# hyperplane-lab/RGBManip

Hardware: AMD Instinct MI355X
Metric: adapose_poses_per_sec_batch256 (higher is better)
Workload: dtype bf16

## Files before the change

include/rgbm.h:

```cpp
#ifndef RGBM_H_
#define RGBM_H_
#include <stddef.h>
#include <stdint.h>

#ifdef __cplusplus
extern "C" {
#endif

#define RGBM_VERSION 100
#define RGBM_F32 0
#define RGBM_BF16 1
#define RGBM_F16 2
#define RGBM_BF16X3 3

int rgbm_version(void);
const char* rgbm_last_error(void);

typedef struct rgbm_weight_desc {
  const char* name;
  const float* data;
  int ndim;
  const int64_t* shape;
} rgbm_weight_desc;

// ... 72 lines not shown
int rgbm_cloud_gather_views(const float* maps, const int32_t* index, int n, int V, int S2, int C, int cap, float* out, void* stream);

int rgbm_adapose_postprocess(int B, int P, int img_size, const float* nocs1, const float* depth1, const float* r1,
                             const int32_t* choose1, const double* Kcrop, const double* E1, double* bbox_world, double* ts,
                             int32_t* valid, void* stream);
int rgbm_adapose_postprocess_scratch_bytes(int B, size_t* bytes);
int rgbm_adapose_postprocess_ws(int B, int P, int img_size, const float* nocs1, const float* depth1, const float* r1,
                                const int32_t* choose1, const double* Kcrop, const double* E1, double* bbox_world, double* ts,
                                int32_t* valid, void* scratch, size_t scratch_bytes, void* stream);

int rgbm_adapose_postprocess_regressed(int B, int P, const float* nocs1, const float* r1, const float* t1, const float* s1,
                                       const double* E1, double* bbox_world, double* ts, int32_t* valid, void* stream);

int rgbm_adapose_postprocess_ransac(int B, int P, int img_size, uint32_t seed, const float* nocs1, const float* depth1,
                                    const int32_t* choose1, const double* Kcrop, const double* E1, double* bbox_world, double* srt,
                                    int32_t* valid, void* stream);
int rgbm_adapose_postprocess_pnp(int B, int P, uint32_t seed, const float* nocs1, const float* pts2d1, const float* nocs2,
                                 const float* pts2d2, const double* K, const double* E1, const double* E2, double* bbox_out,
                                 double* srt_out, int32_t* info_out, int32_t* valid_out, void* stream);

int rgbm_prepare_inputs(const float* rgb_dev, const uint8_t* mask_dev, const double* K_dev, int N, int H, int W, int S, int P,
                        uint32_t seed, float* img_out, int32_t* choose_out, float* pts2d_out, double* Kcrop_out,
                        int32_t* window_out, int32_t* valid_out, uint8_t* scratch, void* stream);

int rgbm_prepare_inputs_indexed(const float* rgb_dev, const uint8_t* mask_dev, const double* K_dev, const int32_t* frame_map_dev,
                                int N, int H, int W, int S, int P, uint32_t seed, float* img_out, int32_t* choose_out,
                                float* pts2d_out, double* Kcrop_out, int32_t* window_out, int32_t* valid_out, uint8_t* scratch,
                                void* stream);
int rgbm_prepare_inputs_ex(const float* rgb_dev, const uint8_t* mask_dev, const double* K_dev, const int32_t* frame_map_dev,
                           int frame0, int N, int H, int W, int S, int P, uint32_t seed, float* img_out, int32_t* choose_out,
                           float* pts2d_out, double* Kcrop_out, int32_t* window_out, int32_t* valid_out, uint8_t* scratch,
                           void* stream);
int rgbm_prepare_inputs_u8(const uint8_t* rgb_dev, const uint8_t* mask_dev, const double* K_dev, const int32_t* frame_map_dev,
                           int frame0, int N, int H, int W, int S, int P, uint32_t seed, float* img_out, int32_t* choose_out,
                           float* pts2d_out, double* Kcrop_out, int32_t* window_out, int32_t* valid_out, uint8_t* scratch,
                           void* stream);
int rgbm_prepare_inputs_opt(const void* rgb_dev, int pixel_type, int normalize, const uint8_t* mask_dev, const double* K_dev,
                            const int32_t* frame_map_dev, int frame0, int N, int H, int W, int S, int P, uint32_t seed, float* img_out,
                            int32_t* choose_out, float* pts2d_out, double* Kcrop_out, int32_t* window_out, int32_t* valid_out,
                            uint8_t* scratch, void* stream);
int rgbm_prepare_inputs_windows(const void* pix_dev, int pixel_type, int normalize, const uint8_t* mask_pix_dev, const int64_t* offset_dev,
                                const int32_t* window_dev, const int32_t* valid_in_dev, const double* K_dev, int frame0, int N, int H, int W,
                                int S, int P, uint32_t seed, float* img_out, int32_t* choose_out, float* pts2d_out, double* Kcrop_out,
                                int32_t* valid_out, uint8_t* scratch, void* stream);
int rgbm_quantize_frames(const float* src_dev, uint8_t* dst_dev, size_t n, void* stream);

int rgbm_projection(const double* Kcrop_dev, const double* E_dev, float* P_dev, int N, void* stream);
int rgbm_mask_extent(const uint8_t* mask_dev, int N, int H, int W, int32_t* ext_out, int32_t* count_out, void* stream);

int rgbm_lookat_quat(const double* dir_dev, int N, int batch_zero, double* quat_dev, void* stream);
int rgbm_control_action_to_pose(const float* action_dev, int lda, const double* pose_mid, const double* pose_min,
                                const double* pose_max, int N, double* pose_dev, void* stream);
typedef struct rgbm_control_reward_args {
  const float* action;
  const double* cam_pose;
  const double* target;
  const float* move_success;
  const double* bbox;
  const double* avail;
  const double* gt_bbox;
  const double* pred_bbox;
  const double* pose_cur;
  const double* pose_prev;
  const double* robot_pose;
  const double* success;
  double* reward;
  double* terms;
  double coef[14];
  double proper_pos[3];
  double precision2;
  int N, T, lda, pots, first;
  int pad_;
} rgbm_control_reward_args;
int rgbm_control_reward(const rgbm_control_reward_args* args, void* stream);
int rgbm_control_grasp_frame(const double* est_dev, int N, double* center_dev, double* direction_dev, void* stream);

typedef struct rgbm_synth_scene {
  const double* cam_pose;
  const double* robot_pose;
  const double* box;
  double fx, fy, cx, cy;
  int N, H, W, env0;
} rgbm_synth_scene;
int rgbm_synth_camera(const rgbm_synth_scene* scene, double* K_dev, double* E_dev, double* rays_dev, void* stream);
int rgbm_synth_render(const rgbm_synth_scene* scene, const double* rays_dev, float* color_dev, uint8_t* mask_dev, void* stream);
int rgbm_synth_render_u8(const rgbm_synth_scene* scene, const double* rays_dev, uint8_t* color_dev, uint8_t* mask_dev,
                         int32_t* extent_dev, int32_t* count_dev, void* stream);

int rgbm_gae(int T, int N, const float* rewards, const uint8_t* dones, const float* values, const float* last_values,
             float gamma, float lam, float* returns, float* adv, double* sums, void* stream);
int rgbm_adv_normalise(int64_t n_local, float* adv, const double* sums, double count_total, void* stream);

typedef struct rgbm_policy_layout {
  int dims[5];
  int log_std;
  int w[2][4];
  int b[2][4];
  int total;
} rgbm_policy_layout;
int rgbm_policy_forward(const float* params, const rgbm_policy_layout* L, int n, int mode, const float* obs, const float* noise,
                        float* actions, float* logp, float* value, float* mu, void* stream);
int rgbm_ppo_partial_floats(const rgbm_policy_layout* L, int n, size_t* count);
int rgbm_ppo_minibatch_fwd_bwd(const float* params, const rgbm_policy_layout* L, int n, const float* obs, const float* actions,
                               const float* old_logp, const float* adv, const float* returns, const float* old_values,
                               const float* old_mu, const float* old_log_std, float clip, float vcoef, float ecoef,
                               float* partial_scratch, float* grads_flat, void* stream);
int rgbm_ppo_clip_adam(float* params, const float* grads_flat, float* exp_avg, float* exp_avg_sq, void* opt_state,
                       const rgbm_policy_layout* L, float inv_world, float max_norm, float desired_kl, float lr_min,
                       float lr_max, int adaptive, void* stream);

#define RGBM_POLICY_MAX_HIDDEN 6
#define RGBM_POLICY_MAX_WIDTH 512
#define RGBM_POLICY_MAX_ACT 32
#define RGBM_ACT_ELU 0
#define RGBM_ACT_SELU 1
#define RGBM_ACT_RELU 2
#define RGBM_ACT_LRELU 3
#define RGBM_ACT_TANH 4
#define RGBM_ACT_SIGMOID 5
typedef struct rgbm_policy_desc {
  int obs_dim, state_dim, act_dim;
  int activation;
  int asymmetric;
  int n_hidden[2];
  int hidden[2][RGBM_POLICY_MAX_HIDDEN];
  int w[2][RGBM_POLICY_MAX_HIDDEN + 1];
  int b[2][RGBM_POLICY_MAX_HIDDEN + 1];
  int log_std;
  int total;
} rgbm_policy_desc;
int rgbm_policy_forward_ex(const float* params, const rgbm_policy_desc* D, int n, int mode, const float* obs, const float* states,
                           const float* noise, float* actions, float* logp, float* value, float* mu, void* stream);
int rgbm_ppo_scratch_floats_ex(const rgbm_policy_desc* D, int n, int clipped_value_loss, size_t* count);
int rgbm_ppo_minibatch_fwd_bwd_ex(const float* params, const rgbm_policy_desc* D, int n, const float* obs, const float* states,
                                  const float* actions, const float* old_logp, const float* adv, const float* returns,
                                  const float* old_values, const float* old_mu, const float* old_log_std, float clip, float vcoef,
                                  float ecoef, int clipped_value_loss, float* scratch, float* grads_flat, void* stream);
int rgbm_ppo_clip_adam_ex(float* params, const float* grads_flat, float* exp_avg, float* exp_avg_sq, void* opt_state, int total,
                          float inv_world, float max_norm, float desired_kl, float lr_min, float lr_max, int adaptive, void* stream);

int rgbm_conv_nd(int dtype, const void* in_dev, int N, int D, int H, int W, int Cin, int Cin_pad, const float* w_host,
                 int Cout, int Cout_pad, int KD, int KH, int KW, int stride_d, int stride_hw, int pad_d, int pad_hw,
                 int dil_hw, int transposed, const float* bias_host, const float* bn_scale_host, const float* bn_shift_host,
                 const void* res_dev, int res_mode, int act, float slope, void* out_dev, void* stream);
#define RGBM_CONV_PLAN_INTS 9
int rgbm_conv_plan(int dtype, int N, int D, int H, int W, int Cin, int Cin_pad, int Cout, int Cout_pad, int KD, int KH, int KW,
                   int stride_d, int stride_hw, int pad_d, int pad_hw, int dil_hw, int transposed, int has_bias, int res_mode, int act,
                   int cls, int n_cu, int32_t* plan);
#define RGBM_BORDER_HEAD_INTS 10
int rgbm_conv_border_plan(int dtype, int N, int H, int W, int Cin, int Cout, int K, int stride, int pad, int dil, int res_mode, int n_cu,
                          int32_t* head, int32_t* classes, int cap_classes, int32_t* tiles, int32_t* order, int cap_tiles, int32_t* wg_off,
                          int cap_wg, int32_t* rows, int64_t cap_rows);
int rgbm_conv_border_launches(int64_t* count);
int rgbm_bn_per_sample_scratch_bytes(int V, size_t* bytes);
int rgbm_bn_per_sample(int dtype, void* y_dev, const void* res_dev, const float* gamma_dev, const float* beta_dev, void* scratch_dev,
                       int V, int64_t nvox, int C, int relu, void* stream);
int rgbm_conv3d_tile(int layer, int dtype, const void* in_dev, int N, int D, int H, int W, const float* w_host,
                     const float* bn_scale_host, const float* bn_shift_host, const void* res_dev, void* out_dev, void* stream);
int rgbm_upsample_conv3x3(int dtype, const void* in_dev, int V, int h, int w, int Cin, const float* w_host, int Cout,
                          const float* bias_host, int act, float slope, void* z_scratch_dev, void* out_dev, void* stream);
int rgbm_upsample_conv3x3_final(int dtype, const void* in_dev, int V, int h, int w, const float* w3_host, const float* b3_host,
                                float slope, const float* wf_host, const float* bf_host, void* out_dev, int out_f32, void* stream);
int rgbm_stem(int dtype, const float* img1_dev, const float* img2_dev, const float* w_host, void* out_dev, int B, int S, void* stream);
int rgbm_maxpool3x3s2(int dtype, const void* in_dev, void* out_dev, int V, int H, int W, int C, void* stream);
int rgbm_resize_bilinear_ac(int dtype, const void* in_dev, void* out_dev, int V, int Hs, int Ws, int C, int Ho, int Wo,
                            void* stream);
int rgbm_adaptive_avgpool(int dtype, const void* in_dev, void* out_dev, int V, int H, int W, int C, int S, void* stream);
int rgbm_build_volume(int dtype, const void* feat_dev, const float* P_views_dev, const float* depths_dev, float* homog_scratch,
                      void* vol_dev, int V, int B, int D, int H, int W, void* stream);
int rgbm_conv0_sweep(const void* feat_dev, const float* P_views_dev, const float* depths_dev, float* homog_scratch,
                     const float* w_host, const float* bn_scale_host, const float* bn_shift_host, void* out_dev,
                     int V, int B, int D, int H, int W, void* stream);
int rgbm_conv0_sweep_dt(int dtype, const void* feat_dev, const float* P_views_dev, const float* depths_dev, float* homog_scratch,
                        const float* w_host, const float* bn_scale_host, const float* bn_shift_host, void* out_dev,
                        int V, int B, int D, int H, int W, void* stream);
int rgbm_conv0_sweep_f16feat(const void* feat_f16_dev, const float* P_views_dev, const float* depths_dev, float* homog_scratch,
                             const float* w_host, const float* bn_scale_host, const float* bn_shift_host, void* out_bf16_dev,
                             int V, int B, int D, int H, int W, void* stream);
int rgbm_adapose_forward_ex(rgbm_adapose_t* h, int B, const float* img1, const float* img2, const int32_t* choose1,
                            const int32_t* choose2, const float* P1, const float* P2, const float* depths, void* workspace,
                            size_t workspace_bytes, const rgbm_adapose_out* out, int stop_after, void* stream);
int rgbm_adapose_forward_graph(rgbm_adapose_t* h, int B, const float* img1, const float* img2, const int32_t* choose1,
                               const int32_t* choose2, const float* P1, const float* P2, const float* depths, void* workspace,
                               size_t workspace_bytes, const rgbm_adapose_out* out, void* stream, int32_t* n_nodes, int32_t* captured);
int rgbm_adapose_graph_clear(rgbm_adapose_t* h);
int rgbm_adapose_feature_bytes(rgbm_adapose_t* h, size_t* bytes);
int rgbm_adapose_features_workspace_bytes(rgbm_adapose_t* h, int V, size_t* bytes);
int rgbm_adapose_features(rgbm_adapose_t* h, int V, const float* img, const int32_t* slots_dev, void* pool, int pool_records,
                          void* workspace, size_t workspace_bytes, void* stream);
int rgbm_adapose_forward_cached(rgbm_adapose_t* h, int B, const void* pool, int pool_records, const int32_t* slot1_dev,
                                const int32_t* slot2_dev, const int32_t* choose1, const int32_t* choose2, const float* P1, const float* P2,
                                const float* depths, void* workspace, size_t workspace_bytes, const rgbm_adapose_out* out, void* stream);
int rgbm_adapose_fetch(rgbm_adapose_t* h, int B, void* workspace, const char* name, float* out_dev, size_t capacity,
                       size_t* n_elems, void* stream);
int rgbm_crop_fingerprint(const float* img, int V, int n_words, uint64_t* keys_out, void* stream);

#define RGBM_PROF_ROWS 42
int rgbm_debug_flags(int flags);
int rgbm_set_tuning(const char* key, long long value);
int rgbm_microbench_mfma_scratch_floats(int* n);
int rgbm_microbench_mfma(float* scratch, int iters, int random_operands, double* flops, void* stream);
int rgbm_microbench_copy(const void* src, void* dst, size_t bytes, void* stream);
int rgbm_prof_rows(void);
int rgbm_prof_start(void);
int rgbm_prof_stop(double* stats);
int rgbm_prof_select(int row);

#ifdef __cplusplus
}
#endif
#endif
```

rgbmanip_amd/_lib.py:

```python
from __future__ import annotations

import ctypes as C
import os

_HERE = os.path.dirname(os.path.abspath(__file__))
LIB_PATH = os.environ.get("RGBM_HIP_LIB") or os.path.join(_HERE, "librgbm_hip.so")

F32, BF16, F16, BF16X3 = 0, 1, 2, 3
ACT_NONE, ACT_RELU, ACT_PRELU, ACT_TANH = 0, 1, 2, 3
RES_NONE, RES_PRE_ACT, RES_POST_ACT = 0, 1, 2


PROF_ROWS = 42
PROF_KERNELS = [
    ("conv_igemm_glds_kernel<float, 16, 256>", "fp32"), ("conv_igemm_glds_kernel<float, 32, 256>", "fp32"),
    ("conv_igemm_glds_kernel<float, 64, 256>", "fp32"), ("conv_igemm_glds_kernel<float, 128, 128>", "fp32"),
    ("conv_igemm_glds_kernel<unsigned short, 16, 256>", "bf16"), ("conv_igemm_glds_kernel<unsigned short, 32, 256>", "bf16"),
    ("conv_igemm_glds_kernel<unsigned short, 64, 256>", "bf16"), ("conv_igemm_glds_kernel<unsigned short, 128, 128>", "bf16"),
    ("conv3d_tile_kernel<float, ...> (conv1..conv11)", "fp32"), ("conv3d_tile_kernel<unsigned short, ...> (conv1..conv11)", "bf16"),
    ("conv3d_tile_kernel<float, 32, 16, 4, 8, 8, 1, false, true> (conv0 + fused plane sweep)", "fp32"),
    ("conv3d_tile_kernel<unsigned short, 32, 16, 4, 8, 8, 1, false, true> (conv0 + fused plane sweep)", "bf16"),
    ("conv_igemm_ws_kernel<float, ...>", "fp32"), ("conv_igemm_ws_kernel<unsigned short, false, false> (128 channels x 256 pixels)", "bf16"),
    ("conv0_sweep_persistent_kernel<unsigned short> (conv0 + fused plane sweep of bf16 nets; sweep_f16 = 0 / fp16 nets: conv0_sweep_kernel)", "bf16"), ("conv_igemm_ws64_kernel", "bf16"),
    ("conv3d_tile_kernel<unsigned short, 32, 16, 6, 8, 8, 1, false, false> (conv0 on a materialised volume)", "bf16"),
    ("conv3d_tile_kernel<unsigned short, 8, 16, 2, 8, 8, 2, false, false> (conv1)", "bf16"),
    ("conv3d_tile_kernel<unsigned short, 16, 16, 4, 8, 8, 1, false, false> (conv2)", "bf16"),
    ("conv3d_tile_kernel<unsigned short, 16, 32, 2, 8, 8, 2, false, false> (conv3)", "bf16"),
    ("conv3d_tile_kernel<unsigned short, 32, 32, 2, 8, 8, 1, false, false> (conv4)", "bf16"),
    ("conv3d_tile_kernel<unsigned short, 32, 64, 1, 8, 8, 2, false, false> (conv5)", "bf16"),
    ("conv3d_tile_kernel<unsigned short, 64, 64, 1, 8, 8, 1, false, false> (conv6)", "bf16"),
    ("conv3d_tile_kernel<unsigned short, 64, 32, 1, 8, 8, 1, true, false> (conv7)", "bf16"),
    ("conv3d_tile_kernel<unsigned short, 32, 16, 2, 8, 8, 1, true, false> (conv9)", "bf16"),
    ("conv3d_tile_kernel<unsigned short, 16, 16, 4, 8, 8, 1, true, false> (conv11)", "bf16"),
] + [("conv_igemm_glds_kernel<bx3_t, ...> (all channel tiles)", "bf16x3"), ("conv3d_tile_kernel<bx3_t, ...> (conv1..conv11)", "bf16x3"),
     ("conv0 + fused plane sweep <bx3_t>", "bf16x3"), ("conv_igemm_ws_kernel<rgbm::bx3_t, false, false> (128 channels x 256 pixels)", "bf16x3"),
     ("pose_mlp1_kernel (pose_mlp1.0 + pose_mlp1.2 of a bf16 net in one launch)", "bf16"),
     ("conv_igemm_m32_kernel<unsigned short, 256, 256> (256 channels x 256 pixels, 32x32x16 MFMAs; gemm_kernel = 0: conv_igemm_ws_kernel<unsigned short, true, false>, 256 x 128)", "bf16"),
     ("pose_mlp2_kernel (pose_mlp2.0 + pose_mlp2.2 + the sum over points of a bf16 net in one launch)", "bf16"),
     ("conv_igemm_m32_kernel<rgbm::bx3_t, 256, 256> (256 channels x 256 pixels, 32x32x16 MFMAs; gemm_kernel = 0: conv_igemm_ws_kernel<rgbm::bx3_t, true, false>, 256 x 128)", "bf16x3"),
     ("conv_igemm_ws_kernel<rgbm::bx3_t, false, false, true> (64 channels x 256 pixels, four multiply waves)", "bf16x3"),
     ("conv_igemm_ws_kernel<unsigned short, false, false, true> (64 channels x 256 pixels, four multiply waves)", "bf16"),
     ("conv_igemm_ws_kernel<float, false, false, true> (64 channels x 256 pixels, four multiply waves)", "fp32"),
     ("upconv_combine_kernel<16-bit> (PSPUpsample tap combination)", "bf16"), ("upconv_combine_kernel<4-byte> (PSPUpsample tap combination)", "bf16x3"),
     ("upconv_final_kernel (up_3 + final in one kernel; either storage width)", "bf16"),
     ("conv_igemm_m32_kernel<unsigned short, 128, 64 / 128 / 256> (128-pixel tiles: tail and small-batch launches of the 256-channel GEMM)", "bf16"),
     ("conv_igemm_m32_kernel<rgbm::bx3_t, 128, 64 / 128 / 256> (128-pixel tiles: tail and small-batch launches of the 256-channel GEMM)", "bf16x3")]
assert len(PROF_KERNELS) == PROF_ROWS


class RgbmError(RuntimeError):
    pass


class WeightDesc(C.Structure):
    _fields_ = [("name", C.c_char_p), ("data", C.c_void_p), ("ndim", C.c_int), ("shape", C.POINTER(C.c_int64))]


class PolicyLayout(C.Structure):
    _fields_ = [("dims", C.c_int * 5), ("log_std", C.c_int), ("w", (C.c_int * 4) * 2), ("b", (C.c_int * 4) * 2), ("total", C.c_int)]


POLICY_MAX_HIDDEN, POLICY_MAX_WIDTH, POLICY_MAX_ACT = 6, 512, 32
POLICY_ACTIVATIONS = {"elu": 0, "selu": 1, "relu": 2, "crelu": 2, "lrelu": 3, "tanh": 4, "sigmoid": 5}


class PolicyDesc(C.Structure):
    _fields_ = [("obs_dim", C.c_int), ("state_dim", C.c_int), ("act_dim", C.c_int), ("activation", C.c_int), ("asymmetric", C.c_int),
                ("n_hidden", C.c_int * 2), ("hidden", (C.c_int * POLICY_MAX_HIDDEN) * 2),
                ("w", (C.c_int * (POLICY_MAX_HIDDEN + 1)) * 2), ("b", (C.c_int * (POLICY_MAX_HIDDEN + 1)) * 2),
                ("log_std", C.c_int), ("total", C.c_int)]


class AdaposeOut(C.Structure):
    _fields_ = [(n, C.c_void_p) for n in ("view1_nocs", "view2_nocs", "view1_depth", "view2_depth", "view1_r", "view2_r",
                                           "view1_t", "view2_t", "view1_s", "view2_s")]


class ControlRewardArgs(C.Structure):
    _fields_ = [(n, C.c_void_p) for n in ("action", "cam_pose", "target", "move_success", "bbox", "avail", "gt_bbox", "pred_bbox",
                                           "pose_cur", "pose_prev", "robot_pose", "success", "reward", "terms")] + [
        ("coef", C.c_double * 14), ("proper_pos", C.c_double * 3), ("precision2", C.c_double),
        ("N", C.c_int), ("T", C.c_int), ("lda", C.c_int), ("pots", C.c_int), ("first", C.c_int), ("pad_", C.c_int)]


class SynthScene(C.Structure):
    _fields_ = [("cam_pose", C.c_void_p), ("robot_pose", C.c_void_p), ("box", C.c_void_p),
                ("fx", C.c_double), ("fy", C.c_double), ("cx", C.c_double), ("cy", C.c_double),
                ("N", C.c_int), ("H", C.c_int), ("W", C.c_int), ("env0", C.c_int)]


_vp, _i, _f, _d, _sz, _i64 = C.c_void_p, C.c_int, C.c_float, C.c_double, C.c_size_t, C.c_int64

SIGNATURES = {
    "rgbm_version": (_i, []),
    "rgbm_last_error": (C.c_char_p, []),
    "rgbm_adapose_create": (_i, [C.POINTER(_vp), _i, C.POINTER(WeightDesc), _i, _i, _i]),
    "rgbm_adapose_create_baseline": (_i, [C.POINTER(_vp), _i, C.POINTER(WeightDesc), _i, _i, _i]),
    "rgbm_view_fusion": (_i, [_vp, _vp, _vp, _i, _i, _vp, _vp, _vp, _sz, _vp]),
    "rgbm_view_fusion_scratch_bytes": (_i, [_i, _i, C.POINTER(_sz)]),
    "rgbm_depth_head": (_i, [_vp, _vp, _i64, _vp, _vp]),
    "rgbm_adapose_destroy": (_i, [_vp]),
    "rgbm_adapose_set_chunk": (_i, [_vp, _i]),
    "rgbm_adapose_set_option": (_i, [_vp, C.c_char_p, _i]),
    "rgbm_adapose_workspace_bytes": (_i, [_vp, _i, C.POINTER(_sz)]),
    "rgbm_adapose_set_dropout": (_i, [_vp, _f, C.c_uint64]),
    "rgbm_adapose_dropout_masks": (_i, [_vp, _i, _vp]),
    "rgbm_adapose_set_dropout_masks": (_i, [_vp, _i, _vp]),
    "rgbm_adapose_forward": (_i, [_vp, _i, _vp, _vp, _vp, _vp, _vp, _vp, _vp, _vp, _sz, C.POINTER(AdaposeOut), _vp]),
    "rgbm_adapose_forward_ex": (_i, [_vp, _i, _vp, _vp, _vp, _vp, _vp, _vp, _vp, _vp, _sz, C.POINTER(AdaposeOut), _i, _vp]),
    "rgbm_adapose_forward_graph": (_i, [_vp, _i, _vp, _vp, _vp, _vp, _vp, _vp, _vp, _vp, _sz, C.POINTER(AdaposeOut), _vp, C.POINTER(C.c_int32),
                                        C.POINTER(C.c_int32)]),
    "rgbm_adapose_samples_workspace_bytes": (_i, [_vp, _i, _i, C.POINTER(_sz)]),
    "rgbm_adapose_forward_samples": (_i, [_vp, _i, _i, _vp, _vp, _vp, _vp, _vp, _vp, _vp, _vp, _sz, C.POINTER(AdaposeOut), _vp]),
    "rgbm_sample_box_stats": (_i, [_vp, _vp, _i, _i, _vp, _vp, _vp, _vp, _vp, _vp, _vp, _vp, _vp]),
    "rgbm_sample_point_stats": (_i, [_vp, _i, _i, _i64, _vp, _vp, _vp]),
    "rgbm_box_agreement": (_i, [_vp, _vp, _vp, _vp, _i] + [_vp] * 14),
    "rgbm_box_iou_matrix": (_i, [_vp, _vp, _vp, _vp, _i, _i, _i, _vp, _vp]),
    "rgbm_adapose_dense_workspace_bytes": (_i, [_vp, _i, C.POINTER(_sz)]),
    "rgbm_adapose_forward_dense": (_i, [_vp, _i, _vp, _vp, _vp, _vp, _vp, _vp, _vp, _vp, _sz, C.POINTER(AdaposeOut), _vp, _vp, _vp]),
    "rgbm_adapose_forward_maps": (_i, [_vp, _i, _vp, _vp, _vp, _vp, _vp, _vp, _vp, _vp, _sz, C.POINTER(AdaposeOut), _vp, _vp, _vp, _vp]),
    "rgbm_nocs_map": (_i, [_vp, _vp, _i, _i, _vp, _vp]),
    "rgbm_cloud_gather": (_i, [_vp, _vp, _vp, _i, _i, _i, _i, _vp, _vp]),
    "rgbm_cloud_similarity_scratch_bytes": (_i, [_i, _i, C.POINTER(_sz)]),
    "rgbm_cloud_similarity": (_i, [_vp, _vp, _vp, _i, _i, C.c_uint32, _vp, _vp, _vp, _vp, _vp, _sz, _vp]),
    "rgbm_depth_to_points": (_i, [_vp, _vp, _vp, _i, _i, _vp, _vp]),
    "rgbm_depth_consistency": (_i, [_vp, _vp, _vp, _vp, _vp, _vp, _vp, _vp, _i, _i, _d, _d, _f, _vp, _vp, _vp, _vp, _vp]),
    "rgbm_cloud_pack": (_i, [_vp, _vp, _vp, _vp, _vp, _vp, _vp, _vp, _i, _i, _i, _vp, _vp, _vp, _vp]),
    "rgbm_depth_fusion": (_i, [_vp, _vp, _vp, _vp, _vp, _i, _i, _i, _d, _d, _f, _i, _vp, _vp, _vp, _vp, _vp]),
    "rgbm_cloud_pack_views": (_i, [_vp, _vp, _vp, _vp, _i, _i, _i, _i, _vp, _vp, _vp, _vp]),
    "rgbm_cloud_gather_views": (_i, [_vp, _vp, _i, _i, _i, _i, _i, _vp, _vp]),
    "rgbm_adapose_graph_clear": (_i, [_vp]),
    "rgbm_adapose_feature_bytes": (_i, [_vp, C.POINTER(_sz)]),
    "rgbm_adapose_features_workspace_bytes": (_i, [_vp, _i, C.POINTER(_sz)]),
    "rgbm_adapose_features": (_i, [_vp, _i, _vp, _vp, _vp, _i, _vp, _sz, _vp]),
    "rgbm_adapose_forward_cached": (_i, [_vp, _i, _vp, _i, _vp, _vp, _vp, _vp, _vp, _vp, _vp, _vp, _sz, C.POINTER(AdaposeOut), _vp]),
    "rgbm_crop_fingerprint": (_i, [_vp, _i, _i, _vp, _vp]),
    "rgbm_adapose_fetch": (_i, [_vp, _i, _vp, C.c_char_p, _vp, _sz, C.POINTER(_sz), _vp]),
    "rgbm_adapose_postprocess": (_i, [_i, _i, _i, _vp, _vp, _vp, _vp, _vp, _vp, _vp, _vp, _vp, _vp]),
    "rgbm_adapose_postprocess_scratch_bytes": (_i, [_i, C.POINTER(_sz)]),
    "rgbm_adapose_postprocess_ws": (_i, [_i, _i, _i, _vp, _vp, _vp, _vp, _vp, _vp, _vp, _vp, _vp, _vp, _sz, _vp]),
    "rgbm_adapose_postprocess_regressed": (_i, [_i, _i, _vp, _vp, _vp, _vp, _vp, _vp, _vp, _vp, _vp]),
    "rgbm_adapose_postprocess_ransac": (_i, [_i, _i, _i, C.c_uint32, _vp, _vp, _vp, _vp, _vp, _vp, _vp, _vp, _vp]),
    "rgbm_adapose_postprocess_pnp": (_i, [_i, _i, C.c_uint32, _vp, _vp, _vp, _vp, _vp, _vp, _vp, _vp, _vp, _vp, _vp, _vp]),
    "rgbm_gae": (_i, [_i, _i, _vp, _vp, _vp, _vp, _f, _f, _vp, _vp, _vp, _vp]),
    "rgbm_adv_normalise": (_i, [_i64, _vp, _vp, _d, _vp]),
    "rgbm_policy_forward": (_i, [_vp, _vp, _i, _i, _vp, _vp, _vp, _vp, _vp, _vp, _vp]),
    "rgbm_ppo_partial_floats": (_i, [_vp, _i, C.POINTER(_sz)]),
    "rgbm_ppo_minibatch_fwd_bwd": (_i, [_vp, _vp, _i, _vp, _vp, _vp, _vp, _vp, _vp, _vp, _vp, _f, _f, _f, _vp, _vp, _vp]),
    "rgbm_ppo_clip_adam": (_i, [_vp, _vp, _vp, _vp, _vp, _vp, _f, _f, _f, _f, _f, _i, _vp]),
    "rgbm_policy_forward_ex": (_i, [_vp, _vp, _i, _i, _vp, _vp, _vp, _vp, _vp, _vp, _vp, _vp]),
    "rgbm_ppo_scratch_floats_ex": (_i, [_vp, _i, _i, C.POINTER(_sz)]),
    "rgbm_ppo_minibatch_fwd_bwd_ex": (_i, [_vp, _vp, _i, _vp, _vp, _vp, _vp, _vp, _vp, _vp, _vp, _vp, _f, _f, _f, _i, _vp, _vp, _vp]),
    "rgbm_ppo_clip_adam_ex": (_i, [_vp, _vp, _vp, _vp, _vp, _i, _f, _f, _f, _f, _f, _i, _vp]),
    "rgbm_conv_nd": (_i, [_i, _vp, _i, _i, _i, _i, _i, _i, _vp, _i, _i, _i, _i, _i, _i, _i, _i, _i, _i, _i, _vp, _vp, _vp,
                          _vp, _i, _i, _f, _vp, _vp]),
    "rgbm_conv_plan": (_i, [_i] * 23 + [C.POINTER(C.c_int32)]),
    "rgbm_conv_border_plan": (_i, [_i] * 12 + [C.POINTER(C.c_int32)] * 2 + [_i] + [C.POINTER(C.c_int32)] * 2 + [_i, C.POINTER(C.c_int32), _i,
                                   C.POINTER(C.c_int32), _i64]),
    "rgbm_conv_border_launches": (_i, [C.POINTER(C.c_int64)]),
    "rgbm_bn_per_sample_scratch_bytes": (_i, [_i, C.POINTER(_sz)]),
    "rgbm_bn_per_sample": (_i, [_i, _vp, _vp, _vp, _vp, _vp, _i, _i64, _i, _i, _vp]),
    "rgbm_conv3d_tile": (_i, [_i, _i, _vp, _i, _i, _i, _i, _vp, _vp, _vp, _vp, _vp, _vp]),
    "rgbm_upsample_conv3x3": (_i, [_i, _vp, _i, _i, _i, _i, _vp, _i, _vp, _i, _f, _vp, _vp, _vp]),
    "rgbm_upsample_conv3x3_final": (_i, [_i, _vp, _i, _i, _i, _vp, _vp, _f, _vp, _vp, _vp, _i, _vp]),
    "rgbm_stem": (_i, [_i, _vp, _vp, _vp, _vp, _i, _i, _vp]),
    "rgbm_maxpool3x3s2": (_i, [_i, _vp, _vp, _i, _i, _i, _i, _vp]),
    "rgbm_resize_bilinear_ac": (_i, [_i, _vp, _vp, _i, _i, _i, _i, _i, _i, _vp]),
    "rgbm_adaptive_avgpool": (_i, [_i, _vp, _vp, _i, _i, _i, _i, _i, _vp]),
    "rgbm_build_volume": (_i, [_i, _vp, _vp, _vp, _vp, _vp, _i, _i, _i, _i, _i, _vp]),
    "rgbm_conv0_sweep": (_i, [_vp, _vp, _vp, _vp, _vp, _vp, _vp, _vp, _i, _i, _i, _i, _i, _vp]),
    "rgbm_conv0_sweep_dt": (_i, [_i, _vp, _vp, _vp, _vp, _vp, _vp, _vp, _vp, _i, _i, _i, _i, _i, _vp]),
    "rgbm_conv0_sweep_f16feat": (_i, [_vp, _vp, _vp, _vp, _vp, _vp, _vp, _vp, _i, _i, _i, _i, _i, _vp]),
    "rgbm_prepare_inputs": (_i, [_vp, _vp, _vp, _i, _i, _i, _i, _i, C.c_uint32, _vp, _vp, _vp, _vp, _vp, _vp, _vp, _vp]),
    "rgbm_prepare_inputs_indexed": (_i, [_vp, _vp, _vp, _vp, _i, _i, _i, _i, _i, C.c_uint32, _vp, _vp, _vp, _vp, _vp, _vp, _vp, _vp]),
    "rgbm_prepare_inputs_ex": (_i, [_vp, _vp, _vp, _vp, _i, _i, _i, _i, _i, _i, C.c_uint32, _vp, _vp, _vp, _vp, _vp, _vp, _vp, _vp]),
    "rgbm_prepare_inputs_u8": (_i, [_vp, _vp, _vp, _vp, _i, _i, _i, _i, _i, _i, C.c_uint32, _vp, _vp, _vp, _vp, _vp, _vp, _vp, _vp]),
    "rgbm_prepare_inputs_opt": (_i, [_vp, _i, _i, _vp, _vp, _vp, _i, _i, _i, _i, _i, _i, C.c_uint32, _vp, _vp, _vp, _vp, _vp, _vp, _vp, _vp]),
    "rgbm_prepare_inputs_windows": (_i, [_vp, _i, _i, _vp, _vp, _vp, _vp, _vp, _i, _i, _i, _i, _i, _i, C.c_uint32, _vp, _vp, _vp, _vp, _vp, _vp, _vp]),
    "rgbm_quantize_frames": (_i, [_vp, _vp, C.c_size_t, _vp]),
    "rgbm_projection": (_i, [_vp, _vp, _vp, _i, _vp]),
    "rgbm_mask_extent": (_i, [_vp, _i, _i, _i, _vp, _vp, _vp]),
    "rgbm_lookat_quat": (_i, [_vp, _i, _i, _vp, _vp]),
    "rgbm_control_action_to_pose": (_i, [_vp, _i, C.POINTER(C.c_double), C.POINTER(C.c_double), C.POINTER(C.c_double), _i, _vp, _vp]),
    "rgbm_control_reward": (_i, [C.POINTER(ControlRewardArgs), _vp]),
    "rgbm_control_grasp_frame": (_i, [_vp, _i, _vp, _vp, _vp]),
    "rgbm_synth_camera": (_i, [C.POINTER(SynthScene), _vp, _vp, _vp, _vp]),
    "rgbm_synth_render": (_i, [C.POINTER(SynthScene), _vp, _vp, _vp, _vp]),
    "rgbm_synth_render_u8": (_i, [C.POINTER(SynthScene), _vp, _vp, _vp, _vp, _vp, _vp]),
    "rgbm_debug_flags": (_i, [_i]),
    "rgbm_set_tuning": (_i, [C.c_char_p, _i64]),
    "rgbm_prof_rows": (_i, []),
    "rgbm_microbench_mfma_scratch_floats": (_i, [C.POINTER(C.c_int)]),
    "rgbm_microbench_mfma": (_i, [_vp, _i, _i, C.POINTER(C.c_double), _vp]),
    "rgbm_microbench_copy": (_i, [_vp, _vp, C.c_size_t, _vp]),
    "rgbm_prof_start": (_i, []),
    "rgbm_prof_select": (_i, [_i]),
    "rgbm_prof_stop": (_i, [C.POINTER(C.c_double)]),
}

_lib = None


def load():
    global _lib
    if _lib is not None:
        return _lib
    if not os.path.exists(LIB_PATH):
        raise RgbmError(f"{LIB_PATH} not found: build it with rgbmanip_amd/csrc/build.sh "
                        f"(or `python -c 'import __graft_entry__ as g; g.build()'`). There is no CPU fallback.")
    lib = C.CDLL(LIB_PATH)
    for name, (res, args) in SIGNATURES.items():
        fn = getattr(lib, name)
        fn.restype = res
        fn.argtypes = args
    if lib.rgbm_prof_rows() != PROF_ROWS:
        raise RgbmError(f"{LIB_PATH}: rgbm_prof_rows() = {lib.rgbm_prof_rows()}, this binding expects {PROF_ROWS} (stale build?)")
    _lib = lib
    return lib


def check(rc: int, what: str = ""):
    if rc != 0:
        msg = load().rgbm_last_error()
        raise RgbmError(f"{what} failed (code {rc}): {msg.decode() if msg else ''}")


def stream_ptr(stream=None):
    import torch
    s = stream if stream is not None else torch.cuda.current_stream()
    return C.c_void_p(s.cuda_stream)


def ptr(t):
    return C.c_void_p(t.data_ptr()) if t is not None else C.c_void_p(0)
```

rgbmanip_amd/csrc/capi.cpp:

```cpp
#include "../../include/rgbm.h"

#include <string.h>

#include <algorithm>
#include <initializer_list>
#include <memory>
#include <string>
#include <utility>
#include <vector>

#include "adapose.h"
#include "box_overlap.h"
#include "control.h"
#include "cost3d.h"
#include "conv_plan.h"
#include "prof.h"
#include "sample_stats.h"
#include "view_fusion.h"

using namespace rgbm;

struct ForwardGraph {
  int B = 0;
  hipStream_t stream = nullptr;
// ... 490 lines not shown
  else if (nm == "pf96") { src = bf.PF96; cnt = V * P * 96; dt = n.pose_dtype() == BF16X3 ? BF16X3 : F32; }
  else if (nm == "pf2") { src = bf.pf2; cnt = V * 256; dt = F32; }
  else if (nm == "r6") { src = bf.r6; cnt = V * 6; dt = F32; }
  else if (nm == "fused1" && bf.fused) { src = bf.fused; cnt = (size_t)B * P * 32; dt = F32; }
  else if (nm == "fused2" && bf.fused) { src = bf.fused + (size_t)B * P * 32; cnt = (size_t)B * P * 32; dt = F32; }
  static const struct { const char* name; int row; } taps3d[] = {{"c0", 0}, {"c2", 2}, {"c4", 4}, {"c6", 6}, {"u7", 7}, {"u9", 8}, {"u11", 9}};
  int row3d = -1;
  for (const auto& t : taps3d)
    if (nm == t.name) { row3d = t.row; src = bf.c3[row3d]; cnt = cost3d_out_elems(row3d, (int)Vc, (int)D, (int)S); }
  if (is_baseline(h))
    RGBM_REQUIRE(nm == "feat" || nm == "fused1" || nm == "fused2" || nm == "pf96" || nm == "pf2" || nm == "r6" || nm == "layer4" || nm == "cat" ||
                 nm == "u1" || nm == "u2", "tap '" + nm + "' does not exist in the baseline network");
  RGBM_REQUIRE(src != nullptr, "unknown intermediate name: " + nm);
  const bool tap3d = row3d >= 0 && row3d < 9;
  RGBM_REQUIRE(!(tap3d && n.sparse_active()), "tap '" + nm + "' needs a dense cost regularisation: set option sparse_dec = 0 before the forward "
               "(the default computes it only inside the chosen pixels' dependency cones)");
  *n_elems = cnt;
  RGBM_REQUIRE(cnt <= capacity, "fetch capacity too small");
  return launch_to_f32(dt, src, out_dev, (long long)cnt, (hipStream_t)stream);
}

int rgbm_adapose_postprocess(int B, int P, int img_size, const float* nocs1, const float* depth1, const float* r1,
                             const int32_t* choose1, const double* Kcrop, const double* E1, double* bbox_world, double* ts,
                             int32_t* valid, void* stream) {
  RGBM_REQUIRE(B > 0 && nocs1 && depth1 && r1 && choose1 && Kcrop && E1 && bbox_world && ts && valid, "postprocess arguments");
  return launch_postprocess(nocs1, depth1, r1, choose1, Kcrop, E1, bbox_world, ts, valid, B, P, img_size, (hipStream_t)stream);
}

int rgbm_adapose_postprocess_scratch_bytes(int B, size_t* bytes) {
  RGBM_REQUIRE(B > 0 && bytes, "postprocess_scratch_bytes arguments");
  *bytes = postprocess_slices(B) > 1 ? postprocess_scratch_bytes(B) : 0;
  return 0;
}

int rgbm_adapose_postprocess_ws(int B, int P, int img_size, const float* nocs1, const float* depth1, const float* r1,
                                const int32_t* choose1, const double* Kcrop, const double* E1, double* bbox_world, double* ts,
                                int32_t* valid, void* scratch, size_t scratch_bytes, void* stream) {
  RGBM_REQUIRE(B > 0 && nocs1 && depth1 && r1 && choose1 && Kcrop && E1 && bbox_world && ts && valid, "postprocess arguments");
  return launch_postprocess(nocs1, depth1, r1, choose1, Kcrop, E1, bbox_world, ts, valid, B, P, img_size, (hipStream_t)stream,
                            scratch, scratch_bytes);
}

int rgbm_adapose_postprocess_ransac(int B, int P, int img_size, uint32_t seed, const float* nocs1, const float* depth1,
                                    const int32_t* choose1, const double* Kcrop, const double* E1, double* bbox_world, double* srt,
                                    int32_t* valid, void* stream) {
  return launch_umeyama_ransac(nocs1, depth1, choose1, Kcrop, E1, bbox_world, srt, valid, B, P, img_size, seed, (hipStream_t)stream);
}

int rgbm_gae(int T, int N, const float* rewards, const uint8_t* dones, const float* values, const float* last_values,
             float gamma, float lam, float* returns, float* adv, double* sums, void* stream) {
  RGBM_REQUIRE(rewards && dones && values && last_values && returns && adv && sums, "gae arguments");
  return launch_gae(T, N, rewards, dones, values, last_values, gamma, lam, returns, adv, sums, (hipStream_t)stream);
}

int rgbm_adv_normalise(int64_t n_local, float* adv, const double* sums, double count_total, void* stream) {
  RGBM_REQUIRE(adv && sums && n_local > 0 && count_total > 1.0, "adv_normalise arguments");
  return launch_adv_normalise(n_local, adv, sums, count_total, (hipStream_t)stream);
}

static ConvGeom conv_nd_geom(int Cin, int Cout, int KD, int KH, int KW, int stride_d, int stride_hw, int pad_d, int pad_hw, int dil_hw,
                             int transposed, int act, float slope) {
  ConvGeom g;
  g.Cin = Cin; g.Cout = Cout; g.KD = KD; g.KH = KH; g.KW = KW;
  g.sd = stride_d; g.sh = g.sw = stride_hw; g.pd = pad_d; g.ph = g.pw = pad_hw;
  g.dild = 1; g.dilh = g.dilw = dil_hw; g.transposed = transposed != 0; g.act = act; g.slope = slope;
  return g;
}

int rgbm_conv_nd(int dtype, const void* in_dev, int N, int D, int H, int W, int Cin, int Cin_pad, const float* w_host,
                 int Cout, int Cout_pad, int KD, int KH, int KW, int stride_d, int stride_hw, int pad_d, int pad_hw,
                 int dil_hw, int transposed, const float* bias_host, const float* bn_scale_host, const float* bn_shift_host,
                 const void* res_dev, int res_mode, int act, float slope, void* out_dev, void* stream) {
  RGBM_REQUIRE(in_dev && w_host && out_dev, "conv arguments");
  const ConvGeom g = conv_nd_geom(Cin, Cout, KD, KH, KW, stride_d, stride_hw, pad_d, pad_hw, dil_hw, transposed, act, slope);
  ConvLayer L;
  if (int rc = L.init(dtype, g, w_host, bias_host, bn_scale_host, bn_shift_host, Cin_pad, Cout_pad)) return rc;
  return finish_one_shot(L.run(in_dev, out_dev, N, D, H, W, Cout_pad, res_dev, res_mode, nullptr, 0, (hipStream_t)stream), stream);
}

int rgbm_conv_plan(int dtype, int N, int D, int H, int W, int Cin, int Cin_pad, int Cout, int Cout_pad, int KD, int KH, int KW,
                   int stride_d, int stride_hw, int pad_d, int pad_hw, int dil_hw, int transposed, int has_bias, int res_mode, int act,
                   int cls, int n_cu, int32_t* plan) {
  RGBM_REQUIRE(plan && n_cu >= 0 && dtype >= F32 && dtype <= BF16X3 && N > 0 && D > 0 && H > 0 && W > 0, "conv_plan arguments");
  const ConvGeom g = conv_nd_geom(Cin, Cout, KD, KH, KW, stride_d, stride_hw, pad_d, pad_hw, dil_hw, transposed, act, 0.f);
  PackedConv pc;
  if (int rc = conv_pack_geom(g, dtype, Cin_pad, Cout_pad, cls, &pc)) return rc;
  ConvDesc d;
  conv_desc_geom(d, g, pc, Cin_pad, Cout_pad, N, D, H, W, Cout_pad, cls);
  alignas(16) static const float buffer[4] = {};
  d.in = d.wgt = buffer; d.out = const_cast<float*>(buffer);
  d.bias = has_bias ? buffer : nullptr;
  d.res = res_mode != RES_NONE ? buffer : nullptr;
  d.res_mode = res_mode;
  ConvTuning t;
  ConvPlan p;
  if (int rc = conv_tuning(n_cu, &t)) return rc;
  if (int rc = plan_conv(d, dtype, t, &p)) return rc;
  const int32_t v[RGBM_CONV_PLAN_INTS] = {p.kernel, p.bch, p.bpix, p.ksplit, (int32_t)p.main_rows, p.tail_bch, p.identity_residual, (int32_t)d.M, d.KT};
  memcpy(plan, v, sizeof(v));
  return 0;
}

int rgbm_conv_border_plan(int dtype, int N, int H, int W, int Cin, int Cout, int K, int stride, int pad, int dil, int res_mode, int n_cu,
                          int32_t* head, int32_t* classes, int cap_classes, int32_t* tiles, int32_t* order, int cap_tiles, int32_t* wg_off,
                          int cap_wg, int32_t* rows, int64_t cap_rows) {
  RGBM_REQUIRE(head && n_cu >= 0 && dtype >= F32 && dtype <= BF16X3 && N > 0 && H > 0 && W > 0 && K > 0, "conv_border_plan arguments");
  const ConvGeom g = conv_nd_geom(Cin, Cout, 1, K, K, 1, stride, 0, pad, dil, 0, ACT_RELU, 0.f);
  PackedConv pc;
  const int E = dtype_chunk(dtype);
  const int Cin_pad = (Cin + E - 1) / E * E, Cout_pad = (Cout + 3) / 4 * 4;
  if (int rc = conv_pack_geom(g, dtype, Cin_pad, Cout_pad, 0, &pc)) return rc;
  ConvDesc d;
  conv_desc_geom(d, g, pc, Cin_pad, Cout_pad, N, 1, H, W, Cout_pad, 0);
  alignas(16) static const float buffer[4] = {};
  d.in = d.wgt = buffer; d.out = const_cast<float*>(buffer);
  d.res = res_mode != RES_NONE ? buffer : nullptr;
  d.res_mode = res_mode;
  d.w_finite = 1;
  ConvTuning t;
  ConvPlan p;
  if (int rc = conv_tuning(n_cu, &t)) return rc;
  if (int rc = plan_conv(d, dtype, t, &p)) return rc;
  memset(head, 0, RGBM_BORDER_HEAD_INTS * sizeof(int32_t));
  BorderPlan bp;
  if (p.kernel != CONV_M32 || !p.border || !plan_border(d, dtype, t.flags, p.main_rows, t.n_cu, &bp)) return 0;
  const int32_t h[RGBM_BORDER_HEAD_INTS] = {1, (int32_t)bp.classes.size(), (int32_t)bp.tiles.size(), bp.n_wg, (int32_t)bp.rows.size(),
                                             (int32_t)bp.max_wg_steps, (int32_t)bp.total_steps, (int32_t)bp.parent_steps, bp.steps_per_tap, bp.kr};
  memcpy(head, h, sizeof(h));
  if (classes) {
    RGBM_REQUIRE((int)bp.classes.size() <= cap_classes, "conv_border_plan: cap_classes too small");
    for (size_t c = 0; c < bp.classes.size(); ++c) {
      classes[3 * c] = bp.classes[c].n_pix; classes[3 * c + 1] = bp.classes[c].mask; classes[3 * c + 2] = (int32_t)bp.classes[c].row0;
    }
  }
  if (tiles || order) RGBM_REQUIRE((int)bp.tiles.size() <= cap_tiles, "conv_border_plan: cap_tiles too small");
  if (tiles)
    for (size_t i = 0; i < bp.tiles.size(); ++i) {
      const BorderTile& bt = bp.tiles[i];
      const int32_t v[5] = {bt.cls, bt.ch, bt.mask, bt.steps, (int32_t)bt.row0};
      memcpy(tiles + 5 * i, v, sizeof(v));
    }
  if (order) memcpy(order, bp.order.data(), bp.order.size() * sizeof(int32_t));
  if (wg_off) {
    RGBM_REQUIRE(bp.n_wg + 1 <= cap_wg, "conv_border_plan: cap_wg too small");
    memcpy(wg_off, bp.wg_off.data(), bp.wg_off.size() * sizeof(int32_t));
  }
  if (rows) {
    RGBM_REQUIRE((int64_t)bp.rows.size() <= cap_rows, "conv_border_plan: cap_rows too small");
    memcpy(rows, bp.rows.data(), bp.rows.size() * sizeof(int32_t));
  }
  return 0;
}

int rgbm_conv_border_launches(int64_t* count) {
  RGBM_REQUIRE(count, "conv_border_launches arguments");
  *count = border_launch_count();
  return 0;
}

int rgbm_upsample_conv3x3(int dtype, const void* in_dev, int V, int h, int w, int Cin, const float* w_host, int Cout,
                          const float* bias_host, int act, float slope, void* z_scratch_dev, void* out_dev, void* stream) {
  RGBM_REQUIRE(in_dev && w_host && z_scratch_dev && out_dev, "upsample_conv3x3 arguments");
  UpConvLayer L;
  if (int rc = L.init(dtype, Cin, Cout, w_host, bias_host, act, slope)) return rc;
  return finish_one_shot(L.run(in_dev, z_scratch_dev, out_dev, V, h, w, Cout, (hipStream_t)stream), stream);
}

int rgbm_upsample_conv3x3_final(int dtype, const void* in_dev, int V, int h, int w, const float* w3_host, const float* b3_host,
                                float slope, const float* wf_host, const float* bf_host, void* out_dev, int out_f32, void* stream) {
  RGBM_REQUIRE(in_dev && w3_host && b3_host && wf_host && bf_host && out_dev, "upsample_conv3x3_final arguments");
  UpConvFinal L;
  if (int rc = L.init(dtype, w3_host, b3_host, slope, wf_host, bf_host)) return rc;
  return finish_one_shot(L.run(in_dev, out_dev, out_f32, V, h, w, (hipStream_t)stream), stream);
}

int rgbm_stem(int dtype, const float* img1_dev, const float* img2_dev, const float* w_host, void* out_dev, int B, int S, void* stream) {
  RGBM_REQUIRE(img1_dev && img2_dev && w_host && out_dev && B > 0, "stem arguments");
  std::vector<float> pk;
  stem_pack(w_host, pk);
  DevBuf wd;
  if (int rc = upload_packed(pk, dtype, wd)) return rc;
  return finish_one_shot(launch_stem(dtype, img1_dev, img2_dev, wd.get(), out_dev, B, 2 * B, S, (hipStream_t)stream), stream);
}

int rgbm_bn_per_sample_scratch_bytes(int V, size_t* bytes) {
  RGBM_REQUIRE(V > 0 && bytes, "bn_per_sample_scratch_bytes arguments");
  *bytes = bn_scratch_bytes(V);
  return 0;
}
int rgbm_bn_per_sample(int dtype, void* y_dev, const void* res_dev, const float* gamma_dev, const float* beta_dev, void* scratch_dev,
                       int V, int64_t nvox, int C, int relu, void* stream) {
  RGBM_REQUIRE(y_dev && gamma_dev && beta_dev && scratch_dev, "bn_per_sample arguments");
  return launch_bn_per_sample(dtype, y_dev, res_dev, gamma_dev, beta_dev, scratch_dev, V, (long long)nvox, C, relu, (hipStream_t)stream);
}
int rgbm_maxpool3x3s2(int dtype, const void* in_dev, void* out_dev, int V, int H, int W, int C, void* stream) {
  return launch_maxpool3x3s2(dtype, in_dev, out_dev, V, H, W, C, (hipStream_t)stream);
}
int rgbm_resize_bilinear_ac(int dtype, const void* in_dev, void* out_dev, int V, int Hs, int Ws, int C, int Ho, int Wo,
                            void* stream) {
  return launch_resize_bilinear_ac(dtype, in_dev, out_dev, V, Hs, Ws, C, Ho, Wo, C, 0, (hipStream_t)stream);
}
int rgbm_adaptive_avgpool(int dtype, const void* in_dev, void* out_dev, int V, int H, int W, int C, int S, void* stream) {
  return launch_adaptive_avgpool(dtype, in_dev, out_dev, V, H, W, C, S, (hipStream_t)stream);
}
int rgbm_build_volume(int dtype, const void* feat_dev, const float* P_views_dev, const float* depths_dev, float* homog_scratch,
                      void* vol_dev, int V, int B, int D, int H, int W, void* stream) {
  if (int rc = launch_homography(P_views_dev, homog_scratch, V, B, (hipStream_t)stream)) return rc;
  return launch_build_volume(dtype, feat_dev, homog_scratch, depths_dev, vol_dev, 0, V, V, B, D, H, W, (hipStream_t)stream);
}

}

#include "prof.h"
extern "C" {
int rgbm_prof_rows(void) { return rgbm::kProfVariants; }
int rgbm_microbench_mfma_scratch_floats(int* n) {
  RGBM_REQUIRE(n, "microbench_mfma_scratch_floats arguments");
  return rgbm::microbench_mfma_scratch_floats(n);
}
int rgbm_microbench_mfma(float* scratch, int iters, int random_operands, double* flops, void* stream) {
  return rgbm::launch_microbench_mfma(scratch, iters, random_operands, flops, (hipStream_t)stream);
}
int rgbm_microbench_copy(const void* src, void* dst, size_t bytes, void* stream) {
  return rgbm::launch_microbench_copy(src, dst, bytes, (hipStream_t)stream);
}
int rgbm_prof_start(void) { return rgbm::prof_start(); }
int rgbm_prof_select(int row) {
  RGBM_REQUIRE(row >= -1 && row < rgbm::kProfVariants, "prof_select: row out of range");
  return rgbm::prof_select(row);
}
int rgbm_prof_stop(double* stats) {
  RGBM_REQUIRE(stats != nullptr, "prof_stop arguments");
  return rgbm::prof_stop(stats, rgbm::kProfVariants);
}
}

extern "C" int rgbm_conv3d_tile(int layer, int dtype, const void* in_dev, int N, int D, int H, int W, const float* w_host,
                                const float* bn_scale_host, const float* bn_shift_host, const void* res_dev, void* out_dev,
                                void* stream) {
  RGBM_REQUIRE(layer >= 0 && layer < kCost3dLayers && in_dev && w_host && bn_scale_host && bn_shift_host && out_dev, "conv3d_tile arguments");
  const Cost3dLayer& L = kCost3d[layer];
  const int coutp = cost3d_coutp(layer);
  std::vector<float> packed;
  conv3d_tile_pack(w_host, bn_scale_host, L.cin, L.cout, coutp, L.transposed, dtype, packed);
  DevBuf wdev, bdev;
  if (upload_packed(packed, dtype, wdev)) return -2;
  std::vector<float> bpad(coutp, 0.f);
  for (int o = 0; o < L.cout; ++o) bpad[o] = bn_shift_host[o];
  if (upload_f32(bpad.data(), bpad.size(), bdev)) return -2;
  Conv3dTileDesc d;
  memset(&d, 0, sizeof(d));
  d.in = in_dev; d.wgt = wdev.get(); d.out = out_dev; d.bias = bdev.get<float>(); d.res = res_dev;
  d.N = N; d.Di = D; d.Hi = H; d.Wi = W;
  if (L.transposed) { d.Do = 2 * D; d.Ho = 2 * H; d.Wo = 2 * W; d.Dq = D; d.Hq = H; d.Wq = W; }
  else {
    const int s = L.stride;
    d.Do = (D + 2 - 3) / s + 1; d.Ho = (H + 2 - 3) / s + 1; d.Wo = (W + 2 - 3) / s + 1;
    d.Dq = d.Do; d.Hq = d.Ho; d.Wq = d.Wo;
  }
  d.Cout = L.cout; d.relu = 1; d.prof_variant = -1;
  return finish_one_shot(launch_conv3d_tile(layer, dtype, d, (hipStream_t)stream), stream);
}

static int conv0_sweep_entry(int dtype, int feat_f16, const void* feat_dev, const float* P_views_dev, const float* depths_dev,
                             float* homog_scratch, const float* w_host, const float* bn_scale_host, const float* bn_shift_host,
                             void* out_dev, int V, int B, int D, int H, int W, void* stream) {
  RGBM_REQUIRE(feat_dev && P_views_dev && depths_dev && homog_scratch && w_host && bn_scale_host && bn_shift_host && out_dev,
               "conv0_sweep arguments");
  RGBM_REQUIRE(dtype == BF16 || dtype == F16 || dtype == BF16X3, "conv0_sweep: 16-bit storage types or bf16x3 (fp32 features in, split-pair c0 out)");
  if (int rc = launch_homography(P_views_dev, homog_scratch, V, B, (hipStream_t)stream)) return rc;
  std::vector<float> packed;
  conv0_sweep_pack(w_host, bn_scale_host, packed);
  DevBuf wdev, bdev;
  if (dtype == BF16X3) { if (conv0_sweep_x3_upload(packed, wdev.out())) return -2; }
  else if (upload_packed(packed, feat_f16 ? (int)F16 : dtype, wdev)) return -2;
  std::vector<float> bpad(cost3d_coutp(0), 0.f);
  for (int o = 0; o < kCost3d[0].cout; ++o) bpad[o] = bn_shift_host[o];
  if (upload_f32(bpad.data(), bpad.size(), bdev)) return -2;
  Conv3dTileDesc d;
  memset(&d, 0, sizeof(d));
  d.wgt = wdev.get(); d.out = out_dev; d.bias = bdev.get<float>();
  d.N = V; d.Di = D; d.Hi = H; d.Wi = W; d.Do = D; d.Ho = H; d.Wo = W; d.Dq = D; d.Hq = H; d.Wq = W;
  d.Cout = kCost3d[0].cout; d.relu = 1; d.prof_variant = -1;
  d.feat = feat_dev; d.homog = homog_scratch; d.depths = depths_dev; d.v0 = 0; d.V = V; d.B = B;
  d.feat_f16 = feat_f16;
  return finish_one_shot(dtype == BF16X3 ? launch_conv0_sweep_x3(d, (hipStream_t)stream) : launch_conv0_sweep(d, dtype, (hipStream_t)stream), stream);
}

extern "C" int rgbm_conv0_sweep_dt(int dtype, const void* feat_dev, const float* P_views_dev, const float* depths_dev,
                                   float* homog_scratch, const float* w_host, const float* bn_scale_host, const float* bn_shift_host,
                                   void* out_dev, int V, int B, int D, int H, int W, void* stream) {
  return conv0_sweep_entry(dtype, 0, feat_dev, P_views_dev, depths_dev, homog_scratch, w_host, bn_scale_host, bn_shift_host, out_dev, V, B, D,
                           H, W, stream);
}

extern "C" int rgbm_conv0_sweep_f16feat(const void* feat_f16_dev, const float* P_views_dev, const float* depths_dev,
                                        float* homog_scratch, const float* w_host, const float* bn_scale_host,
                                        const float* bn_shift_host, void* out_bf16_dev, int V, int B, int D, int H, int W, void* stream) {
  return conv0_sweep_entry(BF16, 1, feat_f16_dev, P_views_dev, depths_dev, homog_scratch, w_host, bn_scale_host, bn_shift_host, out_bf16_dev,
                           V, B, D, H, W, stream);
}

extern "C" int rgbm_conv0_sweep(const void* feat_dev, const float* P_views_dev, const float* depths_dev, float* homog_scratch,
                                const float* w_host, const float* bn_scale_host, const float* bn_shift_host, void* out_dev,
                                int V, int B, int D, int H, int W, void* stream) {
  return rgbm_conv0_sweep_dt(BF16, feat_dev, P_views_dev, depths_dev, homog_scratch, w_host, bn_scale_host, bn_shift_host, out_dev,
// ... 191 lines not shown
```

rgbmanip_amd/csrc/common.h:

```cpp
#pragma once
#include <hip/hip_runtime.h>
#include <stdint.h>
#include <stdio.h>
#include <string>

namespace rgbm {

enum DType { F32 = 0, BF16 = 1, F16 = 2, BF16X3 = 3 };
enum Act { ACT_NONE = 0, ACT_RELU = 1, ACT_PRELU = 2, ACT_TANH = 3 };
enum ResMode { RES_NONE = 0, RES_PRE_ACT = 1, RES_POST_ACT = 2 };

typedef __attribute__((ext_vector_type(8))) __bf16 bf16x8;
typedef _Float16 f16_t;
typedef __attribute__((ext_vector_type(8))) _Float16 f16x8;
typedef __attribute__((ext_vector_type(4))) _Float16 f16x4;
typedef __attribute__((ext_vector_type(8))) float f32x8;
typedef __attribute__((ext_vector_type(4))) float f32x4;

void set_error(const std::string& s);
int fail(const char* what, const char* file, int line);

#define RGBM_CHECK_HIP(expr)                                                             \
  do {                                                                                   \
    hipError_t _e = (expr);                                                              \
// ... 63 lines not shown
  return o;
}
__device__ __forceinline__ void bx3_join4(const uint4& c, float* v) {
  v[0] = __uint_as_float(c.x << 16) + __uint_as_float(c.z << 16);
  v[1] = __uint_as_float(c.x & 0xffff0000u) + __uint_as_float(c.z & 0xffff0000u);
  v[2] = __uint_as_float(c.y << 16) + __uint_as_float(c.w << 16);
  v[3] = __uint_as_float(c.y & 0xffff0000u) + __uint_as_float(c.w & 0xffff0000u);
}
template <> struct Elem<bx3_t> {
  static constexpr int kPerChunk = 4;
  __device__ static __forceinline__ float ld(const bx3_t* p) {
    const unsigned long long a = (unsigned long long)p;
    const unsigned short* ch = reinterpret_cast<const unsigned short*>(a & ~15ull);
    const int e = (int)((a >> 2) & 3);
    return bf16_to_f32(ch[e]) + bf16_to_f32(ch[4 + e]);
  }
  __device__ static __forceinline__ void st(bx3_t* p, float v) {
    const unsigned long long a = (unsigned long long)p;
    unsigned short* ch = reinterpret_cast<unsigned short*>(a & ~15ull);
    const int e = (int)((a >> 2) & 3);
    const unsigned short h = f32_to_bf16(v);
    ch[e] = h;
    ch[4 + e] = f32_to_bf16(v - bf16_to_f32(h));
  }
};

__device__ __forceinline__ float sat_f16(float v) { return v != v ? v : fminf(fmaxf(v, -65504.f), 65504.f); }

__device__ __forceinline__ void load4(const float* p, float v[4]) {
  float4 t = *reinterpret_cast<const float4*>(p);
  v[0] = t.x; v[1] = t.y; v[2] = t.z; v[3] = t.w;
}
__device__ __forceinline__ void load4(const unsigned short* p, float v[4]) {
  uint2 t = *reinterpret_cast<const uint2*>(p);
  v[0] = __uint_as_float(t.x << 16); v[1] = __uint_as_float(t.x & 0xffff0000u);
  v[2] = __uint_as_float(t.y << 16); v[3] = __uint_as_float(t.y & 0xffff0000u);
}
__device__ __forceinline__ void load4(const f16_t* p, float v[4]) {
  const f16x4 t = *reinterpret_cast<const f16x4*>(p);
  v[0] = (float)t[0]; v[1] = (float)t[1]; v[2] = (float)t[2]; v[3] = (float)t[3];
}
__device__ __forceinline__ void store4(f16_t* p, const float v[4]) {
  f16x4 t;
  t[0] = (f16_t)sat_f16(v[0]); t[1] = (f16_t)sat_f16(v[1]); t[2] = (f16_t)sat_f16(v[2]); t[3] = (f16_t)sat_f16(v[3]);
  *reinterpret_cast<f16x4*>(p) = t;
}
__device__ __forceinline__ void store4(float* p, const float v[4]) {
  *reinterpret_cast<float4*>(p) = make_float4(v[0], v[1], v[2], v[3]);
}
__device__ __forceinline__ void store4(unsigned short* p, const float v[4]) {
  uint2 t;
  t.x = pack2_bf16(v[0], v[1]);
  t.y = pack2_bf16(v[2], v[3]);
  *reinterpret_cast<uint2*>(p) = t;
}
__device__ __forceinline__ void load4(const bx3_t* p, float v[4]) { bx3_join4(*reinterpret_cast<const uint4*>(p), v); }
__device__ __forceinline__ void store4(bx3_t* p, const float v[4]) { *reinterpret_cast<uint4*>(p) = bx3_split4(v[0], v[1], v[2], v[3]); }
__device__ __forceinline__ void unpack_chunk(const uint4& c, float* v, bx3_t ) { bx3_join4(c, v); }
__device__ __forceinline__ uint4 pack_chunk(const float* v, bx3_t ) { return bx3_split4(v[0], v[1], v[2], v[3]); }
__device__ __forceinline__ void unpack_chunk(const uint4& c, float* v, float ) {
  v[0] = __uint_as_float(c.x); v[1] = __uint_as_float(c.y); v[2] = __uint_as_float(c.z); v[3] = __uint_as_float(c.w);
}
__device__ __forceinline__ void unpack_chunk(const uint4& c, float* v, unsigned short ) {
  v[0] = __uint_as_float(c.x << 16); v[1] = __uint_as_float(c.x & 0xffff0000u);
  v[2] = __uint_as_float(c.y << 16); v[3] = __uint_as_float(c.y & 0xffff0000u);
  v[4] = __uint_as_float(c.z << 16); v[5] = __uint_as_float(c.z & 0xffff0000u);
  v[6] = __uint_as_float(c.w << 16); v[7] = __uint_as_float(c.w & 0xffff0000u);
}
__device__ __forceinline__ void unpack_chunk(const uint4& c, float* v, f16_t ) {
  const f16x8 h = __builtin_bit_cast(f16x8, c);
#pragma unroll
  for (int e = 0; e < 8; ++e) v[e] = (float)h[e];
}
__device__ __forceinline__ uint4 pack_chunk(const float* v, f16_t ) {
  f16x8 h;
#pragma unroll
  for (int e = 0; e < 8; ++e) h[e] = (f16_t)sat_f16(v[e]);
  return __builtin_bit_cast(uint4, h);
}
__device__ __forceinline__ uint4 pack_chunk(const float* v, float ) {
  return make_uint4(__float_as_uint(v[0]), __float_as_uint(v[1]), __float_as_uint(v[2]), __float_as_uint(v[3]));
}
__device__ __forceinline__ uint4 pack_chunk(const float* v, unsigned short ) {
  uint4 c;
  c.x = pack2_bf16(v[0], v[1]);
  c.y = pack2_bf16(v[2], v[3]);
  c.z = pack2_bf16(v[4], v[5]);
  c.w = pack2_bf16(v[6], v[7]);
  return c;
}

typedef __attribute__((ext_vector_type(4))) short rgbm_s16x4;
__device__ __forceinline__ f32x4 mma_bx3_k16(const uint4& a, const uint4& b, f32x4 c) {
  const rgbm_s16x4 ah = __builtin_bit_cast(rgbm_s16x4, make_uint2(a.x, a.y)), al = __builtin_bit_cast(rgbm_s16x4, make_uint2(a.z, a.w));
  const rgbm_s16x4 bh = __builtin_bit_cast(rgbm_s16x4, make_uint2(b.x, b.y)), bl = __builtin_bit_cast(rgbm_s16x4, make_uint2(b.z, b.w));
  c = __builtin_amdgcn_mfma_f32_16x16x16bf16_1k(al, bh, c, 0, 0, 0);
  c = __builtin_amdgcn_mfma_f32_16x16x16bf16_1k(ah, bl, c, 0, 0, 0);
  c = __builtin_amdgcn_mfma_f32_16x16x16bf16_1k(ah, bh, c, 0, 0, 0);
  return c;
}
__device__ __forceinline__ void bx3_pair(const uint4& c0, const uint4& c1, uint4& hi, uint4& lo) {
  hi = make_uint4(c0.x, c0.y, c1.x, c1.y);
  lo = make_uint4(c0.z, c0.w, c1.z, c1.w);
}

__host__ __device__ inline unsigned mix32(unsigned seed, unsigned frame, unsigned idx) {
  unsigned h = seed ^ (frame * 0x9E3779B9u) ^ (idx * 0x85EBCA6Bu);
  h ^= h >> 16; h *= 0x85EBCA6Bu; h ^= h >> 13; h *= 0xC2B2AE35u; h ^= h >> 16;
  return h;
}

template <int THREADS, class Op> __device__ inline double block_reduce(double v, double* red, Op op) {
  const int t = threadIdx.x;
  red[t] = v;
  __syncthreads();
  for (int s = THREADS / 2; s > 0; s >>= 1) {
    if (t < s) red[t] = op(red[t], red[t + s]);
    __syncthreads();
  }
  const double r = red[0];
  __syncthreads();
  return r;
}
template <int THREADS> __device__ inline double block_sum(double v, double* red) {
  return block_reduce<THREADS>(v, red, [](double a, double b) { return a + b; });
}
template <int THREADS> __device__ inline double block_max(double v, double* red) {
  return block_reduce<THREADS>(v, red, [](double a, double b) { return fmax(a, b); });
}

struct ConvDesc {
  const void* in; const void* wgt; void* out; const float* bias; const void* res;
  int N, Di, Hi, Wi, Cin, lcin;
  int Dq, Hq, Wq;
  int sd, sh, sw, pd, ph, pw;
  int KD, KH, KW, dild, dilh, dilw;
  int ntaps, KT, Kpad;
  int Cout, ldo;
  int Do, Ho, Wo;
  int osd, osh, osw, opd, oph, opw;
  int act; float slope; int res_mode; int bias_stride;
  long long M;
  int n_pix_tiles, n_ch_tiles;
  int n_tiles; unsigned fd_m[3]; int fd_s[3];
  int korder;
  int buf_ok;
  const void* ident;
  long long m0;
  const void* w2; const float* bias2; void* out2; int ldo2, cout2, kpad2, act2; float slope2;
  double algo_flops, algo_bytes;
  int out_f32;
  int ksplit; float* kscratch; unsigned* kcount;
  int w_finite; const int* btab; int b_nwg, b_ent, b_rows;
};

int launch_conv(const ConvDesc& d, int dtype, hipStream_t s);
bool conv_ws64_eligible(const ConvDesc& d, int dtype);
int conv_ch_tile(int Cout);
int conv_bk(int dtype);

}
```

rgbmanip_amd/csrc/conv_igemm_m32.inc:

```
#ifndef M32_SHIFT
#define M32_SHIFT 1
#endif
#ifndef M32_RACE_PROBE
#define M32_RACE_PROBE 0
#endif
typedef __attribute__((ext_vector_type(16))) float f32x16;

template <typename T> struct Mma32;
template <> struct Mma32<unsigned short> {
  __device__ static __forceinline__ void run(const uint4& a, const uint4& b, f32x16& c) {
    c = __builtin_amdgcn_mfma_f32_32x32x16_bf16(__builtin_bit_cast(bf16x8, a), __builtin_bit_cast(bf16x8, b), c, 0, 0, 0);
  }
};
template <> struct Mma32<f16_t> {
  __device__ static __forceinline__ void run(const uint4& a, const uint4& b, f32x16& c) {
    c = __builtin_amdgcn_mfma_f32_32x32x16_f16(__builtin_bit_cast(f16x8, a), __builtin_bit_cast(f16x8, b), c, 0, 0, 0);
  }
};

template <> struct Mma32<bx3_t> {
  __device__ static __forceinline__ void run(const uint4&, const uint4&, f32x16&) {}
};

__device__ __forceinline__ int m32_row_channel(int i) { return ((i >> 2) & 1) * 16 + (i & 3) + 4 * (i >> 3); }

template <typename T, int BPIX, int BCH = 256>
__global__ __launch_bounds__(BPIX == 256 ? 768 : 512) void conv_igemm_m32_kernel(const ConvDesc d) {
  constexpr bool BIG = BPIX == 256;
  constexpr bool STAGED = BIG && BCH == 256;
  constexpr bool X3 = std::is_same<T, bx3_t>::value;
  constexpr int NMW = BIG ? 8 : 4;
  constexpr int NTH = (NMW + 4) * 64;
  constexpr int NST = BIG ? 2 : 3;
  static_assert(BCH == 256 || BCH == 128 || BCH == 64, "channel tiles of 256 / 128 / 64");
  constexpr int E = 16 / sizeof(T);
  constexpr int BK = 8 * E;
  constexpr int XR = BPIX / 32;
  constexpr int WL = BCH / 32;
  constexpr int NP = XR + WL;
  constexpr int FA = BCH / 64, FB = 2;
  constexpr int WCHW = FA * 32;
  constexpr int STAGE = (BCH + BPIX) * 8;
  extern __shared__ __attribute__((aligned(16))) uint4 lds3[];

  const int tid = threadIdx.x;
  const int lane = tid & 63;
  const int wave = __builtin_amdgcn_readfirstlane(tid >> 6);
  constexpr bool KSPLIT = !BIG && BCH <= 128;
  int KT = d.KT, kt0 = 0, part = 0, nsp = 1, vtile = -1;
  if constexpr (KSPLIT) {
    if (d.ksplit > 1) {
      nsp = d.ksplit;
      part = (int)blockIdx.x % nsp;
      vtile = (int)blockIdx.x / nsp;
      kt0 = (int)((long long)part * d.KT / nsp);
      KT = (int)((long long)(part + 1) * d.KT / nsp) - kt0;
    }
  }
  const bool res_in_acc = d.ident != nullptr && d.res_mode == RES_PRE_ACT;
  const int KR = (res_in_acc && part == nsp - 1) ? BCH / BK : 0;
  const int KTT = KT + KR;
  const bool bm = STAGED && !X3 && d.btab != nullptr;
  const int* __restrict__ bent = d.btab;
  int n_my = vtile >= 0 ? 1 : ((int)d.n_tiles - (int)blockIdx.x + (int)gridDim.x - 1) / (int)gridDim.x;
  int total = n_my * KTT;
  if (bm) {
    const int be0 = d.btab[blockIdx.x];
    n_my = d.btab[blockIdx.x + 1] - be0;
    bent = d.btab + d.b_ent + 4 * be0;
    total = 0;
    for (int k = 0; k < n_my; ++k) total += bent[4 * k + 1] + KR;
  }
  auto bsteps = [&](int k) { return bm ? __builtin_amdgcn_readfirstlane(bent[4 * k + 1]) : KT; };
  auto tile_of = [&](int k, int& pix_tile, int& ch_tile) {
    if (bm) { pix_tile = 0; ch_tile = __builtin_amdgcn_readfirstlane(bent[4 * k + 2]) >> 16; return; }
    const int v = vtile >= 0 ? vtile : (int)blockIdx.x + k * (int)gridDim.x;
    const int nblk = d.n_tiles, bq = nblk >> 3, br = nblk & 7, xcd = v & 7, bidx = v >> 3;
    const int lid = (xcd < br ? xcd * (bq + 1) : br * (bq + 1) + (xcd - br) * bq) + bidx;
    pix_tile = lid / d.n_ch_tiles;
    ch_tile = lid - pix_tile * d.n_ch_tiles;
  };

  float* lbias = reinterpret_cast<float*>(lds3 + NST * STAGE);
  const bool bias_lds = d.bias != nullptr && d.bias_stride == 0 && d.Cout <= 2560;
  if (bias_lds)
    for (int i = tid; i < d.Cout; i += NTH) lbias[i] = d.bias[i];
  __syncthreads();

  if (wave >= NMW) {
    const int pw = wave - NMW;
    const int tp = tid - NMW * 64;
    const int j = tp & 7;
    const int r0 = tp >> 3;
    const int js = j ^ ((r0 >> 1) & 7);
    unsigned rmask[XR], xoff[XR], woff[WL], roff[XR];
    int tkd = 0, tkh = 0, tkw = 0, tc = 0;
    unsigned wko = 0;
    const unsigned lds0 = __builtin_amdgcn_readfirstlane(lds_addr(lds3 + pw * 64));
    const long long xbias = ((long long)(d.pd * d.Hi + d.ph) * d.Wi + d.pw) * d.Cin * (long long)sizeof(T);
    const __amdgpu_buffer_rsrc_t rsrc_x = __builtin_amdgcn_make_buffer_rsrc(
        const_cast<char*>(reinterpret_cast<const char*>(d.in)) - xbias, 0,
        (int)(unsigned)((long long)d.N * d.Di * d.Hi * d.Wi * d.Cin * (long long)sizeof(T) + xbias), 0x00020000);
    const __amdgpu_buffer_rsrc_t rsrc_w = __builtin_amdgcn_make_buffer_rsrc(
        const_cast<char*>(reinterpret_cast<const char*>(d.wgt)), 0, (int)(unsigned)((long long)d.n_ch_tiles * BCH * d.Kpad * (long long)sizeof(T)), 0x00020000);

    const __amdgpu_buffer_rsrc_t rsrc_r = __builtin_amdgcn_make_buffer_rsrc(
        const_cast<char*>(reinterpret_cast<const char*>(d.res)), 0, (int)(unsigned)(d.M * d.ldo * (long long)sizeof(T)), 0x00020000);
    const __amdgpu_buffer_rsrc_t rsrc_i = __builtin_amdgcn_make_buffer_rsrc(
        const_cast<char*>(reinterpret_cast<const char*>(d.ident)), 0, (int)(unsigned)(256 * 256 * sizeof(T)), 0x00020000);
    long long mybase = 0;
    unsigned mymask = 0;
    int my_ch_tile = 0, my_pix_tile = 0;
    int ikt = 0, itile = 0;
    int KTc = KT, KTTc = KTT, bkh0 = 0, bkh1 = 0, bkw0 = 0, bkw1 = 0, mym = -1;
    int* lrow = reinterpret_cast<int*>(lbias + 2560);
    auto decode_my = [&](long long m) {
      mybase = 0;
      mymask = 0;
      if (j < XR) {
        int xn = 0, xd0 = -(1 << 20), xh0 = 0, xw0 = 0;
        if (m >= 0 && m < d.M) {
          unsigned n, qd, qh, qw;
          decode_row(d, (unsigned)m, n, qd, qh, qw);
          xn = (int)n * d.Di;
          xd0 = (int)qd * d.sd - d.pd;
          xh0 = (int)qh * d.sh - d.ph;
          xw0 = (int)qw * d.sw - d.pw;
        }
        for (int kk = 0; kk < d.KD; ++kk) mymask |= (unsigned)((unsigned)(xd0 + kk * d.dild) < (unsigned)d.Di) << kk;
        for (int kk = 0; kk < d.KH; ++kk) mymask |= (unsigned)((unsigned)(xh0 + kk * d.dilh) < (unsigned)d.Hi) << (8 + kk);
        for (int kk = 0; kk < d.KW; ++kk) mymask |= (unsigned)((unsigned)(xw0 + kk * d.dilw) < (unsigned)d.Wi) << (16 + kk);
        if (bm) mymask = m >= 0 ? 0x00ffffffu : 0u;
        const long long pix0 = ((long long)(xn + xd0) * d.Hi + xh0) * d.Wi + xw0;
        mybase = pix0 * d.Cin * (long long)sizeof(T);
      }
    };
    auto prepare_tile = [&](int k) {
      int pix_tile, ch_tile;
      tile_of(k, pix_tile, ch_tile);
      my_ch_tile = ch_tile;
      my_pix_tile = pix_tile;
      if (bm) {
        const int tr = __builtin_amdgcn_readfirstlane(bent[4 * k + 2]);
        KTc = bsteps(k);
        KTTc = KTc + KR;
        bkh0 = tr & 15; bkh1 = (tr >> 4) & 15; bkw0 = (tr >> 8) & 15; bkw1 = (tr >> 12) & 15;
        mym = j < XR ? d.btab[d.b_rows + __builtin_amdgcn_readfirstlane(bent[4 * k]) + r0 + 32 * j] : -1;
        return;
      }
      decode_my(d.m0 + (long long)pix_tile * BPIX + r0 + 32 * j);
    };
    auto enter_tile = [&]() {
      const int grp = (tp & 63) & 56;
      if (bm) {
        decode_my(mym);
        if (j < XR) lrow[(itile & 1) * 256 + r0 + 32 * j] = mym;
        asm volatile("s_waitcnt lgkmcnt(0)" ::: "memory");
      }
#pragma unroll
      for (int i = 0; i < XR; ++i) {
        const long long b = __shfl(mybase, grp | i, 64);
        rmask[i] = (unsigned)__shfl((int)mymask, grp | i, 64);
        xoff[i] = (unsigned)(b + xbias + (long long)(js * E) * (long long)sizeof(T));
        if (KR) {
          long long m = d.m0 + (long long)my_pix_tile * BPIX + r0 + 32 * i;
          if (bm) { m = __shfl(mym, grp | i, 64); if (m < 0) m = d.M; }
          roff[i] = m < d.M ? (unsigned)((m * d.ldo + my_ch_tile * BCH + js * E) * (long long)sizeof(T)) : 0xffffffffu;
        }
      }
#pragma unroll
      for (int i = 0; i < WL; ++i) {
        const int row = r0 + 32 * i;
        woff[i] = (unsigned)(((long long)(my_ch_tile * BCH + row) * d.Kpad + js * E) * (long long)sizeof(T));
      }
      tkd = tkh = tkw = tc = 0;
      wko = 0;
      if (bm) {
        tkh = bkh0; tkw = bkw0;
        wko = (unsigned)((tkh * d.KW + tkw) * d.Cin) * (unsigned)sizeof(T);
      }
      if (kt0 > 0) {
        if (d.korder && d.lcin >= 0) {
          const int tap = kt0 % d.ntaps, cb = kt0 / d.ntaps;
          tkw = tap % d.KW; tkh = (tap / d.KW) % d.KH; tkd = tap / (d.KW * d.KH);
          tc = cb * BK;
          wko = (unsigned)(((long long)tap * d.Cin + tc) * (long long)sizeof(T));
        } else {
          wko = (unsigned)kt0 * (unsigned)(BK * sizeof(T));
          if (d.lcin >= 0) {
            const int cpt = d.Cin / BK, tap = kt0 / cpt;
            tc = (kt0 - tap * cpt) * BK;
            tkw = tap % d.KW; tkh = (tap / d.KW) % d.KH; tkd = tap / (d.KW * d.KH);
          } else {
            tc = kt0 * BK;
          }
        }
      }
    };

    auto issue = [&](int stage) {
      if (ikt == 0) enter_tile();
      const unsigned sbase = lds0 + (unsigned)stage * (STAGE * 16);
      const unsigned sel = (1u << tkd) | (256u << tkh) | (65536u << tkw);
      const unsigned soff = (unsigned)(((long long)((tkd * d.dild * d.Hi + tkh * d.dilh) * d.Wi + tkw * d.dilw) * d.Cin + tc) * (long long)sizeof(T));
      const bool cok = tkd < d.KD && tc + js * E < d.Cin;
      if (ikt >= KTc) {
        const unsigned ro = (unsigned)(ikt - KTc) * (unsigned)(BK * sizeof(T));
#pragma unroll
        for (int i = 0; i < XR; ++i) blds16(roff[i], rsrc_r, ro, sbase + (BCH * 8 + i * 256) * 16);
        if (!BIG) {
#pragma unroll
          for (int i = 0; i < WL; ++i) blds16((unsigned)(((r0 + 32 * i) * 256 + js * E) * (int)sizeof(T)), rsrc_i, ro, sbase + (i * 256) * 16);
        }
      } else {
#pragma unroll
        for (int i = 0; i < XR; ++i) {
          const bool ok = cok && (rmask[i] & sel) == sel;
          blds16(ok ? xoff[i] : 0xffffffffu, rsrc_x, soff, sbase + (BCH * 8 + i * 256) * 16);
        }
#pragma unroll
        for (int i = 0; i < WL; ++i) blds16(woff[i], rsrc_w, wko, sbase + (i * 256) * 16);
      }
      if (ikt >= KTc) {
      } else if (bm) {
        if (++tkw == bkw1) { tkw = bkw0; if (++tkh == bkh1) { tkh = bkh0; tc += BK; } }
        wko = (unsigned)((tkh * d.KW + tkw) * d.Cin + tc) * (unsigned)sizeof(T);
      } else if (d.korder && d.lcin >= 0) {
        wko += (unsigned)d.Cin * (unsigned)sizeof(T);
        if (++tkw == d.KW) { tkw = 0; if (++tkh == d.KH) { tkh = 0; if (++tkd == d.KD) { tkd = 0; tc += BK; wko = (unsigned)tc * (unsigned)sizeof(T); } } }
      } else {
        wko += BK * (unsigned)sizeof(T);
        tc += BK;
        if (d.lcin >= 0 && tc >= d.Cin) {
          tc = 0;
          if (++tkw == d.KW) { tkw = 0; if (++tkh == d.KH) { tkh = 0; ++tkd; } }
        }
      }
      if (++ikt == KTTc) { ikt = 0; ++itile; if (itile < n_my) prepare_tile(itile); }
    };

    if (total > 0) prepare_tile(0);
    if (total > 0) issue(0);
    if (NST == 3 && total > 1) issue(1);
    int st = 0, gk = 0, gtile = 0;
    int gKTT = total > 0 ? bsteps(0) + KR : KTT;
    for (int g = 0; g < total; ++g) {
      if (NST == 2 || g + 1 >= total) asm volatile("s_waitcnt vmcnt(0)" ::: "memory");
      else asm volatile("s_waitcnt vmcnt(%0)" :: "n"(NP) : "memory");
      RGBM_BARRIER();
      if (NST == 3) { if (g + 2 < total) issue(st == 0 ? 2 : st - 1); }
      else { if (g + 1 < total) issue(st ^ 1); }
      st = st == NST - 1 ? 0 : st + 1;
      if (STAGED) { if (++gk == gKTT) { gk = 0; RGBM_BARRIER(); if (++gtile < n_my) gKTT = bsteps(gtile) + KR; } }
    }
    return;
  }

  const int wch = BIG ? (wave >> 2) * WCHW : (wave >> 1) * WCHW;
  const int wpix = BIG ? (wave & 3) * 64 : (wave & 1) * 64;
  const int li = lane & 31, lh = lane >> 5;
  const int rowA = wch + m32_row_channel(li), rowB = wpix + li;
  const unsigned offA = (unsigned)(rowA * 8 + (lh ^ ((rowA >> 1) & 7))) * 16u;
  const unsigned offB = (unsigned)(BCH * 8 + rowB * 8 + (lh ^ ((rowB >> 1) & 7))) * 16u;
  const char* ldsc = reinterpret_cast<const char*>(lds3);
  f32x16 acc[FA][FB];
  auto ident_frag = [&](int sub) {
    int lq = lane;
    asm volatile("" : "+v"(lq));
    const int qi = lq & 31, qh = lq >> 5;
    const int id_s = (qi >> 2) & 1, id_c = (qi & 3) + 4 * (qi >> 3);
    const int lh = qh;
    const unsigned one = std::is_same<T, f16_t>::value ? 0x3c00u : 0x3f80u;
    const bool mine = sub == id_s && lh == (id_c >> 3);
    const unsigned w = mine ? one << (16 * (id_c & 1)) : 0u;
    const int q = (id_c & 7) >> 1;
    return make_uint4(q == 0 ? w : 0u, q == 1 ? w : 0u, q == 2 ? w : 0u, q == 3 ? w : 0u);
  };
  auto load_step = [&](int st, int s, uint4 (&af)[FA], uint4 (&bf)[FB]) {
    const char* base = ldsc + st * (STAGE * 16);
    const unsigned oa = offA ^ ((unsigned)s << 5), ob = offB ^ ((unsigned)s << 5);
#pragma unroll
    for (int b = 0; b < FB; ++b) bf[b] = *reinterpret_cast<const uint4*>(base + ob + b * 4096);
#pragma unroll
    for (int a = 0; a < FA; ++a) af[a] = *reinterpret_cast<const uint4*>(base + oa + a * 4096);
  };
  auto mma_step = [&](const uint4 (&af)[FA], const uint4 (&bf)[FB]) {
#pragma unroll
    for (int a = 0; a < FA; ++a)
#pragma unroll
      for (int b = 0; b < FB; ++b) {
        Mma32<T>::run(af[a], bf[b], acc[a][b]);
      }
  };
  T* __restrict__ out = reinterpret_cast<T*>(d.out);
  const T* __restrict__ res = reinterpret_cast<const T*>(d.res);
  auto tile_interior = [&](int pix_tile, int ch_tile) {
    if (bm) return true;
    return (d.bias == nullptr || bias_lds) && d.m0 + (long long)(pix_tile + 1) * BPIX <= d.M && (ch_tile + 1) * BCH <= d.Cout && d.act != ACT_TANH;
  };
  int st = 0;
  for (int k = 0; k < n_my; ++k) {
    const int KTk = BIG ? bsteps(k) : KT;
    {
      int pt, ct;
      tile_of(k, pt, ct);
      if (tile_interior(pt, ct) && d.bias && part == 0) {
        const float* bp = lbias + ct * BCH + wch + lh * 16;
#pragma unroll
        for (int a = 0; a < FA; ++a) {
          f32x16 b16;
#pragma unroll
          for (int q = 0; q < 4; ++q) {
            const f32x4 b4 = *reinterpret_cast<const f32x4*>(bp + a * 32 + q * 4);
            b16[q * 4 + 0] = b4[0]; b16[q * 4 + 1] = b4[1]; b16[q * 4 + 2] = b4[2]; b16[q * 4 + 3] = b4[3];
          }
#pragma unroll
          for (int b = 0; b < FB; ++b) acc[a][b] = b16;
        }
      } else {
#pragma unroll
        for (int a = 0; a < FA; ++a)
#pragma unroll
          for (int b = 0; b < FB; ++b)
#pragma unroll
            for (int e = 0; e < 16; ++e) acc[a][b][e] = 0.f;
      }
    }
    if constexpr (X3) {
      const int zA = (rowA >> 1) & 7, zB = (rowB >> 1) & 7;
      unsigned oA3 = (unsigned)(rowA * 128) + (unsigned)(((2 * lh) ^ zA) << 4);
      unsigned oB3 = (unsigned)(BCH * 128 + rowB * 128) + (unsigned)(((2 * lh) ^ zB) << 4);
      const char* sb = ldsc;
      auto rdp = [&](unsigned off, uint4& hi, uint4& lo) {
        const uint4 c0 = *reinterpret_cast<const uint4*>(sb + off), c1 = *reinterpret_cast<const uint4*>(sb + (off ^ 16u));
        hi = make_uint4(c0.x, c0.y, c1.x, c1.y);
        lo = make_uint4(c0.z, c0.w, c1.z, c1.w);
      };
      const int KTM = BIG ? KTk : KTT;
      for (int kt = 0; kt < KTM; ++kt) {
        asm volatile("s_waitcnt lgkmcnt(0)" ::: "memory");
        RGBM_BARRIER();
        asm volatile("" : "+v"(oA3), "+v"(oB3));
        sb = ldsc + st * (STAGE * 16);
#pragma unroll
        for (int s = 0; s < 2; ++s) {
          uint4 Bh[FB], Bl[FB], Al, Ah, Aln, Ahn;
          const unsigned ob = oB3 ^ ((unsigned)s << 6), oa = oA3 ^ ((unsigned)s << 6);
#pragma unroll
          for (int b = 0; b < FB; ++b) rdp(ob + b * 4096, Bh[b], Bl[b]);
          rdp(oa, Ah, Al);
          __builtin_amdgcn_sched_barrier(0);
#pragma unroll
          for (int a = 0; a < FA; ++a) {
            if (a + 1 < FA) rdp(oa + (a + 1) * 4096, Ahn, Aln);
            __builtin_amdgcn_sched_barrier(0);
#pragma unroll
            for (int b = 0; b < FB; ++b) Mma32<unsigned short>::run(Al, Bh[b], acc[a][b]);
#pragma unroll
            for (int b = 0; b < FB; ++b) Mma32<unsigned short>::run(Ah, Bl[b], acc[a][b]);
#pragma unroll
            for (int b = 0; b < FB; ++b) Mma32<unsigned short>::run(Ah, Bh[b], acc[a][b]);
            __builtin_amdgcn_sched_barrier(0);
            if (a + 1 < FA) { Al = Aln; Ah = Ahn; }
          }
        }
        st = st == NST - 1 ? 0 : st + 1;
      }
      if constexpr (BIG) {
        if (KR) {
#pragma unroll
          for (int r = 0; r < BCH / BK; ++r) {
            asm volatile("s_waitcnt lgkmcnt(0)" ::: "memory");
            RGBM_BARRIER();
            if (wch == ((32 * r) / WCHW) * WCHW) {
              asm volatile("" : "+v"(oB3));
              sb = ldsc + st * (STAGE * 16);
#pragma unroll
              for (int s2 = 0; s2 < 2; ++s2) {
                uint4 Bh[FB], Bl[FB];
                const unsigned ob = oB3 ^ ((unsigned)s2 << 6);
#pragma unroll
                for (int b = 0; b < FB; ++b) rdp(ob + b * 4096, Bh[b], Bl[b]);
                const uint4 Aid = ident_frag(s2);
#pragma unroll
                for (int b = 0; b < FB; ++b) Mma32<unsigned short>::run(Aid, Bl[b], acc[((32 * r) % WCHW) / 32][b]);
#pragma unroll
                for (int b = 0; b < FB; ++b) Mma32<unsigned short>::run(Aid, Bh[b], acc[((32 * r) % WCHW) / 32][b]);
              }
            }
            st ^= 1;
          }
        }
      }
    } else if constexpr (BIG) {
      uint4 A[FA], B[FB], Bn[FB];
      unsigned oA = offA, oB = offB;
      auto ldA = [&](int s, int a) { A[a] = *reinterpret_cast<const uint4*>(ldsc + st * (STAGE * 16) + (oA ^ ((unsigned)s << 5)) + a * 4096); };
      auto ldB = [&](int s, uint4 (&bf)[FB]) {
#pragma unroll
        for (int b = 0; b < FB; ++b) bf[b] = *reinterpret_cast<const uint4*>(ldsc + st * (STAGE * 16) + (oB ^ ((unsigned)s << 5)) + b * 4096);
      };
      auto ldAs = [&](int stg, int s, int a) { A[a] = *reinterpret_cast<const uint4*>(ldsc + stg * (STAGE * 16) + (oA ^ ((unsigned)s << 5)) + a * 4096); };
      auto ldBs = [&](int stg, int s, uint4 (&bf)[FB]) {
#pragma unroll
        for (int b = 0; b < FB; ++b) bf[b] = *reinterpret_cast<const uint4*>(ldsc + stg * (STAGE * 16) + (oB ^ ((unsigned)s << 5)) + b * 4096);
      };
// ... 176 lines not shown
      pok[b] = m < d.M;
      if (dense_out && (interior || d.bias_stride == 0)) {
        nn[b] = 0;
        obase[b] = (pok[b] ? m : 0ll) * d.ldo;
        continue;
      }
      unsigned n, qd, qh, qw;
      decode_row(d, pok[b] ? (unsigned)m : 0u, n, qd, qh, qw);
      nn[b] = (int)n;
      obase[b] = ((((long long)n * d.Do + (qd * d.osd + d.opd)) * d.Ho + (qh * d.osh + d.oph)) * d.Wo + (qw * d.osw + d.opw)) * d.ldo;
    }
    constexpr int CHK = 16 / (int)sizeof(T);
    constexpr int NQ = 16 / CHK;
    if (interior) {
      const float nslope = d.act == ACT_RELU ? 0.f : d.act == ACT_PRELU ? d.slope : 1.f;
      auto fast = [&](auto resc) {
        constexpr int RES = decltype(resc)::value;
        constexpr int NF = FA * FB;
        constexpr int AR = FA < (X3 ? 2 : 4) ? FA : (X3 ? 2 : 4);
        static_assert(FA % AR == 0, "whole store rounds");
        uint4 pk[AR][NQ];
        uint4 rr[4][NQ];
        const long long mrow = d.m0 + (long long)pix_tile * BPIX + wpix;
        const int ch0 = ch_tile * BCH + wch;
        unsigned lofs_c = (unsigned)((li * d.ldo + lh * 16) * (int)sizeof(T));
        asm volatile("" : "+v"(lofs_c));
        auto rd = [&](int i) {
          const int b = i / FA, a = i % FA;
          const char* ub = reinterpret_cast<const char*>(res + (mrow + b * 32) * d.ldo + ch0 + a * 32);
#pragma unroll
          for (int q = 0; q < NQ; ++q) rr[i & 3][q] = *reinterpret_cast<const uint4*>(ub + lofs_c + q * 16);
        };
        auto make = [&](int i) {
          const int b = i / FA, a = i % FA;
#pragma unroll
          for (int q = 0; q < NQ; ++q) {
            float v[CHK], rv[CHK];
#pragma unroll
            for (int e = 0; e < CHK; ++e) v[e] = acc[a][b][q * CHK + e];
            if (RES != RES_NONE) unpack_chunk(rr[i & 3][q], rv, T());
            if (RES == RES_PRE_ACT) {
#pragma unroll
              for (int e = 0; e < CHK; ++e) v[e] += rv[e];
            }
#pragma unroll
            for (int e = 0; e < CHK; ++e) v[e] = v[e] < 0.f ? __builtin_fmaxf(v[e], -3.402823466e38f) * nslope : v[e];
            if (RES == RES_POST_ACT) {
#pragma unroll
              for (int e = 0; e < CHK; ++e) v[e] += rv[e];
            }
            pk[a % AR][q] = pack_chunk(v, T());
          }
        };
        auto store_round = [&](int b, int ar) {
          if constexpr (STAGED) {
            char* stg = const_cast<char*>(ldsc) + (st ^ 1) * (STAGE * 16) + wave * 8192;
            unsigned wofs = (unsigned)(li * 256 + (((lh * NQ) ^ (li & 15)) << 4));
            unsigned rofs = (unsigned)((lane >> 4) * 256 + (((lane & 15) ^ (lane >> 4)) << 4));
            unsigned gofs = (unsigned)(((lane >> 4) * d.ldo + (lane & 15) * CHK) * (int)sizeof(T));
            asm volatile("" : "+v"(wofs), "+v"(rofs), "+v"(gofs));
#pragma unroll
            for (int a = 0; a < AR; ++a)
#pragma unroll
              for (int q = 0; q < NQ; ++q)
                *reinterpret_cast<uint4*>(stg + (wofs ^ (unsigned)((a * 2 * NQ + q) << 4))) = pk[a][q];
            if (bm) {
              const int* lrow = reinterpret_cast<const int*>(lbias + 2560) + (k & 1) * 256 + wpix + b * 32 + (lane >> 4);
              char* oc = reinterpret_cast<char*>(out + ch0 + ar * AR * 32) + (lane & 15) * 16;
#pragma unroll
              for (int t = 0; t < 8; ++t) {
                const int m = lrow[4 * t];
                const uint4 v = *reinterpret_cast<const uint4*>(stg + t * 1024 + (rofs ^ (unsigned)(((4 * t) & 15) << 4)));
                if (m >= 0) *reinterpret_cast<uint4*>(oc + (long long)m * d.ldo * (long long)sizeof(T)) = v;
              }
              return;
            }
            char* ob = reinterpret_cast<char*>(out + (mrow + b * 32) * d.ldo + ch0 + ar * AR * 32);
#pragma unroll
            for (int t = 0; t < 8; ++t) {
              const uint4 v = *reinterpret_cast<const uint4*>(stg + t * 1024 + (rofs ^ (unsigned)(((4 * t) & 15) << 4)));
              *reinterpret_cast<uint4*>(ob + (long long)(4 * t) * d.ldo * (long long)sizeof(T) + gofs) = v;
            }
          } else {
#pragma unroll
            for (int a = 0; a < AR; ++a)
#pragma unroll
              for (int q = 0; q < NQ; ++q)
                *reinterpret_cast<uint4*>(reinterpret_cast<char*>(out + (mrow + b * 32) * d.ldo + ch0 + (ar * AR + a) * 32) + lofs_c + q * 16) = pk[a][q];
          }
        };
        if (RES != RES_NONE) { rd(0); rd(1); __builtin_amdgcn_sched_barrier(0); }
#pragma unroll
        for (int i = 0; i < NF; ++i) {
          make(i);
          __builtin_amdgcn_sched_barrier(0);
          if (RES != RES_NONE) {
            if (i < FA - 1) rd(i + 2);
            else if (i == FA - 1) {
#pragma unroll
              for (int k = FA + 1; k < NF; ++k) rd(k);
            }
            __builtin_amdgcn_sched_barrier(0);
          }
          if (i % AR == AR - 1) { store_round(i / FA, (i % FA) / AR); __builtin_amdgcn_sched_barrier(0); }
        }
      };
      if (BIG || res_in_acc) fast(IC<RES_NONE>{});
      else if (d.res_mode == RES_NONE) fast(IC<RES_NONE>{});
      else if (d.res_mode == RES_PRE_ACT) fast(IC<RES_PRE_ACT>{});
      else fast(IC<RES_POST_ACT>{});
      continue;
    }
    if constexpr (BIG) continue;
#pragma unroll
    for (int a = 0; a < FA; ++a) {
      const int chL = ch_tile * BCH + wch + a * 32 + lh * 16;
#pragma unroll
      for (int b = 0; b < FB; ++b) {
#pragma unroll
        for (int q = 0; q < NQ; ++q) {
          const int c = chL + q * CHK;
          if (!pok[b] || c >= d.Cout) continue;
          const bool whole = c + CHK <= d.Cout;
          float v[CHK], rv[CHK];
#pragma unroll
          for (int e = 0; e < CHK; ++e) v[e] = acc[a][b][q * CHK + e];
          if (d.bias) {
            const float* bp = d.bias + (long long)nn[b] * d.bias_stride + c;
#pragma unroll
            for (int e = 0; e < CHK; ++e) if (e < 4 || whole) v[e] += bp[e];
          }
#pragma unroll
          for (int e = 0; e < CHK; ++e) rv[e] = 0.f;
          if (d.res_mode != RES_NONE && !res_in_acc) {
            if (whole) unpack_chunk(*reinterpret_cast<const uint4*>(res + obase[b] + c), rv, T());
            else load4(res + obase[b] + c, rv);
          }
          if (d.res_mode == RES_PRE_ACT && !res_in_acc) {
#pragma unroll
            for (int e = 0; e < CHK; ++e) v[e] += rv[e];
          }
#pragma unroll
          for (int e = 0; e < CHK; ++e) v[e] = apply_act_g(v[e], d.act, d.slope);
          if (d.res_mode == RES_POST_ACT) {
#pragma unroll
            for (int e = 0; e < CHK; ++e) v[e] += rv[e];
          }
          if (whole) *reinterpret_cast<uint4*>(out + obase[b] + c) = pack_chunk(v, T());
          else store4(out + obase[b] + c, v);
        }
      }
    }
  }
}

static std::atomic<long long> g_border_launches{0};
long long border_launch_count() { return g_border_launches.load(std::memory_order_relaxed); }

template <typename T, int BPIX, int BCH = 256>
static int launch_m32_range(ConvDesc d, hipStream_t s) {
  constexpr int NST = BPIX == 256 ? 2 : 3;
  constexpr size_t LDS = ((size_t)NST * (BCH + BPIX) * 8) * sizeof(uint4) + 2560 * sizeof(float) + (BPIX == 256 && BCH == 256 ? 2 * 256 * sizeof(int) : 0);
  d.n_pix_tiles = (int)((d.M - d.m0 + BPIX - 1) / BPIX);
  d.n_ch_tiles = (d.Cout + BCH - 1) / BCH;
  const long long ntiles = (long long)d.n_pix_tiles * d.n_ch_tiles;
  RGBM_REQUIRE(ntiles > 0 && ntiles < (1ll << 31) && d.M < (1ll << 31), "conv grid out of range");
  d.n_tiles = (int)ntiles;
  make_fastdiv(d.Wq, d.fd_m[0], d.fd_s[0]);
  make_fastdiv(d.Hq, d.fd_m[1], d.fd_s[1]);
  make_fastdiv(d.Dq, d.fd_m[2], d.fd_s[2]);
  if (int rc = ensure_dynamic_lds(reinterpret_cast<const void*>(conv_igemm_m32_kernel<T, BPIX, BCH>), (int)LDS)) return rc;
  int n_cu = 0;
  if (int rc = persistent_grid_cus(&n_cu)) return rc;
  RGBM_REQUIRE(d.ksplit <= 1 || (BPIX == 128 && BCH <= 128 && ntiles * d.ksplit <= 4096 && d.kscratch && d.kcount), "K split: 64 / 128-channel x 128-pixel tiles, one workgroup per (tile, part)");
  const int grid = d.ksplit > 1 ? (int)(ntiles * d.ksplit) : ntiles < n_cu ? (int)ntiles : n_cu;
  RGBM_REQUIRE(d.btab == nullptr || (BPIX == 256 && BCH == 256 && d.m0 == 0 && grid == d.b_nwg), "border-class table: made for another grid");
  if (d.btab) g_border_launches.fetch_add(1, std::memory_order_relaxed);
  prof_begin_launch(s, BPIX == 256 && BCH == 256 ? (std::is_same<T, bx3_t>::value ? 33 : 31) : (std::is_same<T, bx3_t>::value ? 41 : 40), d.algo_flops, d.algo_bytes);
  hipLaunchKernelGGL((conv_igemm_m32_kernel<T, BPIX, BCH>), dim3((unsigned)grid), dim3(BPIX == 256 ? 768 : 512), LDS, s, d);
  prof_end_launch(s);
  RGBM_CHECK_HIP(hipGetLastError());
  return 0;
}

template <typename T>
static int m32_identity(const void** out) {
  static std::mutex mu;
  static std::map<int, void*> per_dev;
  int dev = 0;
  RGBM_CHECK_HIP(hipGetDevice(&dev));
  std::lock_guard<std::mutex> lock(mu);
  void*& p = per_dev[dev];
  if (!p) {
    if (std::is_same<T, bx3_t>::value) {
      std::vector<unsigned short> h(256 * 256 * 2, 0);
      for (int i = 0; i < 256; ++i) h[(i * 256 + (i & ~3)) * 2 + (i & 3)] = 0x3f80;
      RGBM_CHECK_HIP(hipMalloc(&p, h.size() * 2));
      RGBM_CHECK_HIP(hipMemcpy(p, h.data(), h.size() * 2, hipMemcpyHostToDevice));
    } else {
      std::vector<unsigned short> h(256 * 256, 0);
      const unsigned short one = std::is_same<T, f16_t>::value ? 0x3c00 : 0x3f80;
      for (int i = 0; i < 256; ++i) h[i * 256 + i] = one;
      RGBM_CHECK_HIP(hipMalloc(&p, h.size() * 2));
      RGBM_CHECK_HIP(hipMemcpy(p, h.data(), h.size() * 2, hipMemcpyHostToDevice));
    }
  }
  *out = p;
  return 0;
}

static int m32_ksplit_buffers(hipStream_t s, float** scratch, unsigned** count) {
  static std::mutex mu;
  static std::map<std::pair<int, hipStream_t>, std::pair<float*, unsigned*>> per_stream;
  int dev = 0;
  RGBM_CHECK_HIP(hipGetDevice(&dev));
  std::lock_guard<std::mutex> lock(mu);
  auto& e = per_stream[std::make_pair(dev, s)];
  if (!e.first) {
    hipStreamCaptureStatus cs = hipStreamCaptureStatusNone;
    if (hipStreamIsCapturing(s, &cs) == hipSuccess && cs != hipStreamCaptureStatusNone) { *scratch = nullptr; *count = nullptr; return 0; }
    float* sc = nullptr; unsigned* cn = nullptr;
    RGBM_CHECK_HIP(hipMalloc(&sc, kM32SplitFloats * sizeof(float)));
    RGBM_CHECK_HIP(hipMalloc(&cn, kM32SplitCounters * sizeof(unsigned)));
    RGBM_CHECK_HIP(hipMemsetAsync(cn, 0, kM32SplitCounters * sizeof(unsigned), s));
    e.first = sc; e.second = cn;
  }
  *scratch = e.first; *count = e.second;
  return 0;
}

template <typename T>
static int m32_setup(ConvDesc& d, const ConvPlan& p, hipStream_t s) {
  d.m0 = 0;
  d.ident = nullptr;
  d.korder = p.korder;
  d.ksplit = 1; d.kscratch = nullptr; d.kcount = nullptr;
  if (p.ksplit > 1) {
    if (int rc = m32_ksplit_buffers(s, &d.kscratch, &d.kcount)) return rc;
    if (d.kscratch) d.ksplit = p.ksplit;
  }
  return p.identity_residual ? m32_identity<T>(&d.ident) : 0;
}

template <typename T>
static int launch_m32_tiles128(const ConvDesc& d, int bch, hipStream_t s) {
  return bch == 64 ? launch_m32_range<T, 128, 64>(d, s) : bch == 128 ? launch_m32_range<T, 128, 128>(d, s) : launch_m32_range<T, 128, 256>(d, s);
}

template <typename T>
static int launch_m32_small(ConvDesc d, const ConvPlan& p, hipStream_t s) {
  if (int rc = m32_setup<T>(d, p, s)) return rc;
  d.btab = nullptr;
  return launch_m32_tiles128<T>(d, p.bch, s);
}

template <typename T>
static int launch_m32(ConvDesc d, const ConvPlan& p, hipStream_t s) {
  if (int rc = m32_setup<T>(d, p, s)) return rc;
  if (!p.border) d.btab = nullptr;
  if (p.main_rows > 0) {
    ConvDesc m = d;
    m.M = p.main_rows;
    const double frac = (double)m.M / (double)d.M;
    m.algo_flops = d.algo_flops * frac; m.algo_bytes = d.algo_bytes * frac;
    if (int rc = launch_m32_range<T, 256, 256>(m, s)) return rc;
    d.m0 = m.M;
    d.btab = nullptr;
    d.algo_flops *= 1.0 - frac; d.algo_bytes *= 1.0 - frac;
  }
  return p.tail_bch ? launch_m32_tiles128<T>(d, p.tail_bch, s) : 0;
}
```

rgbmanip_amd/csrc/conv_plan.cpp:

```cpp
#include "conv_plan.h"

#include <algorithm>
#include <functional>
#include <queue>
#include <utility>

#include "kernels.h"

namespace rgbm {

#ifndef M32_KSPLIT_MAX
#define M32_KSPLIT_MAX 4
#endif
#ifndef M32_KSPLIT_MINSTEPS
#define M32_KSPLIT_MINSTEPS 8
#endif

namespace {

bool uniform_taps(const ConvDesc& d, int bk) {
  if (d.KD > 8 || d.KH > 8 || d.KW > 8) return false;
  if (d.lcin < 0) return d.ntaps == 1;
  return d.Cin % bk == 0;
}
// ... 37 lines not shown
void tap_range(int q, int pad, int dil, int K, int n, int& k0, int& k1) {
  k0 = K; k1 = 0;
  for (int k = 0; k < K; ++k) {
    const int x = q - pad + k * dil;
    if (x >= 0 && x < n) { if (k < k0) k0 = k; k1 = k + 1; }
  }
  if (k0 > k1) k0 = k1 = 0;
}

struct AxisClasses {
  std::vector<int> k0, k1, count, cls;
};
bool axis_classes(int nq, int pad, int dil, int K, int n, AxisClasses* a) {
  a->cls.resize(nq);
  for (int q = 0; q < nq; ++q) {
    int k0, k1;
    tap_range(q, pad, dil, K, n, k0, k1);
    if (k1 == k0) return false;
    for (int k = k0; k < k1; ++k) {
      const int x = q - pad + k * dil;
      if (x < 0 || x >= n) return false;
    }
    size_t c = 0;
    while (c < a->k0.size() && !(a->k0[c] == k0 && a->k1[c] == k1)) ++c;
    if (c == a->k0.size()) { a->k0.push_back(k0); a->k1.push_back(k1); a->count.push_back(0); }
    a->count[c] += 1;
    a->cls[q] = (int)c;
  }
  return true;
}

bool border_shape_ok(const ConvDesc& d, int dtype) {
  return (dtype == BF16 || dtype == F16) && d.w_finite && d.KD == 1 && d.Di == 1 && d.Dq == 1 && d.pd == 0 && d.sd == 1 && d.sh == 1 && d.sw == 1 &&
         d.KH * d.KW > 1 && d.KH <= 4 && d.KW <= 4 && d.lcin >= 0 && d.Cin % conv_bk(dtype) == 0 && d.Cout % 256 == 0 && d.ph >= 0 && d.pw >= 0 &&
         d.dilh >= 1 && d.dilw >= 1 && d.N > 0 && d.M == (long long)d.N * d.Hq * d.Wq;
}

int popcount_int(int v) { int n = 0; for (; v; v &= v - 1) ++n; return n; }

}

static long long class_live_rows(const ConvDesc& d, const AxisClasses& ah, const AxisClasses& aw, long long main_rows, int i, int j) {
  const long long hw = (long long)d.Hq * d.Wq, whole = main_rows / hw, rem = main_rows % hw;
  const int hr = (int)(rem / d.Wq), wr = (int)(rem % d.Wq);
  long long h_below = 0, w_below = 0;
  for (int h = 0; h < hr; ++h) h_below += ah.cls[h] == i;
  for (int w = 0; w < wr; ++w) w_below += aw.cls[w] == j;
  return whole * ah.count[i] * aw.count[j] + h_below * aw.count[j] + (ah.cls[hr < d.Hq ? hr : 0] == i && hr < d.Hq ? w_below : 0);
}

bool border_applies(const ConvDesc& d, int dtype, int flags, long long main_rows) {
  if ((flags & (DBG_NO_BORDER_TILES | DBG_KORDER_TAPS_OUTER)) || !border_shape_ok(d, dtype)) return false;
  if (main_rows <= 0 || main_rows > d.M || main_rows % 256) return false;
  AxisClasses ah, aw;
  if (!axis_classes(d.Hq, d.ph, d.dilh, d.KH, d.Hi, &ah) || !axis_classes(d.Wq, d.pw, d.dilw, d.KW, d.Wi, &aw)) return false;
  long long tiles = 0, taps = 0;
  for (size_t i = 0; i < ah.k0.size(); ++i)
    for (size_t j = 0; j < aw.k0.size(); ++j) {
      const long long t = (class_live_rows(d, ah, aw, main_rows, (int)i, (int)j) + 255) / 256;
      tiles += t;
      taps += t * (ah.k1[i] - ah.k0[i]) * (aw.k1[j] - aw.k0[j]);
    }
  return taps < (main_rows / 256) * (long long)d.ntaps && tiles < (1ll << 20);
}

bool plan_border(const ConvDesc& d, int dtype, int flags, long long main_rows, int n_wg, BorderPlan* out) {
  if (n_wg <= 0 || !border_applies(d, dtype, flags, main_rows)) return false;
  AxisClasses ah, aw;
  axis_classes(d.Hq, d.ph, d.dilh, d.KH, d.Hi, &ah);
  axis_classes(d.Wq, d.pw, d.dilw, d.KW, d.Wi, &aw);
  BorderPlan p;
  p.n_wg = n_wg;
  p.n_ch = d.Cout / 256;
  p.steps_per_tap = d.Cin / conv_bk(dtype);
  const bool dense_out = d.osd == 1 && d.osh == 1 && d.osw == 1 && d.opd == 0 && d.oph == 0 && d.opw == 0 && d.Dq == d.Do && d.Hq == d.Ho && d.Wq == d.Wo;
  p.kr = (dense_out && d.res_mode == RES_PRE_ACT && d.res != nullptr) ? 256 / conv_bk(dtype) : 0;
  const int nw = (int)aw.k0.size();
  std::vector<int> of_class(ah.k0.size() * nw, -1);
  for (int h = 0; h < d.Hq; ++h)
    for (int w = 0; w < d.Wq; ++w) {
      int& c = of_class[ah.cls[h] * nw + aw.cls[w]];
      if (c < 0) {
        c = (int)p.classes.size();
        BorderClass bc = {};
        bc.kh0 = ah.k0[ah.cls[h]]; bc.kh1 = ah.k1[ah.cls[h]]; bc.kw0 = aw.k0[aw.cls[w]]; bc.kw1 = aw.k1[aw.cls[w]];
        for (int kh = bc.kh0; kh < bc.kh1; ++kh)
          for (int kw = bc.kw0; kw < bc.kw1; ++kw) bc.mask |= 1 << (kh * d.KW + kw);
        bc.n_pix = ah.count[ah.cls[h]] * aw.count[aw.cls[w]];
        p.classes.push_back(bc);
      }
    }
  int pix0 = 0;
  for (BorderClass& bc : p.classes) { bc.pix0 = pix0; pix0 += bc.n_pix; }
  p.pix.assign((size_t)d.Hq * d.Wq, 0);
  {
    std::vector<int> fill(p.classes.size(), 0);
    for (int h = 0; h < d.Hq; ++h)
      for (int w = 0; w < d.Wq; ++w) {
        const int c = of_class[ah.cls[h] * nw + aw.cls[w]];
        p.pix[p.classes[c].pix0 + fill[c]++] = h * d.Wq + w;
      }
  }
  const long long hw = (long long)d.Hq * d.Wq;
  p.total_steps = 0;
  for (size_t c = 0; c < p.classes.size(); ++c) {
    BorderClass& bc = p.classes[c];
    bc.row0 = (long long)p.rows.size();
    for (long long v = 0; v * hw < main_rows; ++v)
      for (int i = 0; i < bc.n_pix; ++i) {
        const long long m = v * hw + p.pix[bc.pix0 + i];
        if (m < main_rows) p.rows.push_back((int)m);
      }
    const long long live = (long long)p.rows.size() - bc.row0;
    p.rows.resize((size_t)(bc.row0 + (live + 255) / 256 * 256), -1);
    if (p.rows.size() >= (1u << 30)) return false;
    const int steps = popcount_int(bc.mask) * p.steps_per_tap + p.kr;
    for (long long t = 0; t < (live + 255) / 256; ++t)
      for (int ch = 0; ch < p.n_ch; ++ch) {
        p.tiles.push_back(BorderTile{(int)c, ch, bc.mask, steps, bc.row0 + t * 256});
        p.total_steps += steps;
      }
  }
  p.parent_steps = (main_rows / 256) * p.n_ch * (long long)(d.ntaps * p.steps_per_tap + p.kr);
  std::vector<int> by_steps(p.tiles.size());
  for (size_t i = 0; i < by_steps.size(); ++i) by_steps[i] = (int)i;
  auto mid_view = [&](int i) { const BorderClass& bc = p.classes[p.tiles[i].cls]; return (double)(p.tiles[i].row0 - bc.row0 + 128) / bc.n_pix; };
  std::stable_sort(by_steps.begin(), by_steps.end(), [&](int a, int b) { return mid_view(a) < mid_view(b); });
  if ((int)by_steps.size() > n_wg)
    std::stable_sort(by_steps.end() - n_wg, by_steps.end(), [&](int a, int b) { return p.tiles[a].steps > p.tiles[b].steps; });
  typedef std::pair<long long, std::pair<int, int>> Load;
  std::priority_queue<Load, std::vector<Load>, std::greater<Load>> q;
  const int per_xcd = (n_wg + 7) / 8;
  for (int b = 0; b < n_wg; ++b) q.push(Load(0, std::make_pair((b & 7) * per_xcd + (b >> 3), b)));
  std::vector<std::vector<int>> mine(n_wg);
  for (int i : by_steps) {
    Load l = q.top();
    q.pop();
    mine[l.second.second].push_back(i);
    l.first += p.tiles[i].steps;
    q.push(l);
  }
  p.max_wg_steps = 0;
  p.wg_off.assign(1, 0);
  for (int b = 0; b < n_wg; ++b) {
    long long s = 0;
    for (int i : mine[b]) { p.order.push_back(i); s += p.tiles[i].steps; }
    p.wg_off.push_back((int)p.order.size());
    if (s > p.max_wg_steps) p.max_wg_steps = s;
  }
  *out = std::move(p);
  return true;
}

int plan_conv(const ConvDesc& d, int dtype, const ConvTuning& t, ConvPlan* out) {
  RGBM_REQUIRE(d.M > 0 && d.M < (1ll << 31), "conv M out of range");
  RGBM_REQUIRE(d.Cout % 4 == 0 && d.ldo % 4 == 0, "conv Cout/ldo must be multiples of 4");
  RGBM_REQUIRE(d.KT > 0 && d.Kpad == d.KT * conv_bk(dtype), "conv K padding mismatch");
  RGBM_REQUIRE(d.Cin % dtype_chunk(dtype) == 0, "conv Cin must be a multiple of the 16-byte chunk");
  if (d.lcin >= 0) {
    RGBM_REQUIRE((1 << d.lcin) == d.Cin, "conv lcin mismatch");
  } else {
    RGBM_REQUIRE(d.ntaps == 1, "linear-K mode needs a single tap");
  }
  const int f = t.flags, n_cu = t.n_cu;
  const long long esz = (long long)dtype_size(dtype);
  const bool bits16 = esz == 2, mfma32 = dtype != F32;
  const int ch_tile = conv_ch_tile(d.Cout);
  const bool uni = uniform_taps(d, conv_bk(dtype)) && !(f & DBG_NONUNIFORM_TAPS);
  const bool out16 = (((unsigned long long)d.out | (unsigned long long)(d.ldo * esz)) & 15ull) == 0ull;
  const bool rows16 = out16 && ((unsigned long long)d.res & 15ull) == 0ull;
  const bool dense_out = d.osd == 1 && d.osh == 1 && d.osw == 1 && d.opd == 0 && d.oph == 0 && d.opw == 0 && d.Dq == d.Do && d.Hq == d.Ho && d.Wq == d.Wo;
  const bool ident_ok = dense_out && d.res_mode == RES_PRE_ACT && d.res != nullptr && d.M * d.ldo * esz < (1ll << 32) - 65536;
  const bool ws_rows = d.M >= (t.ws_min_rows > 0 ? t.ws_min_rows : 1024);

  ConvPlan p = {};
  p.uniform_taps = uni;
  p.ksplit = 1;
  p.korder = (f & DBG_KORDER_TAPS_OUTER) ? 0 : 1;
  auto pick = [&](int kernel, int bch, int bpix) {
    p.kernel = kernel; p.bch = bch; p.bpix = bpix;
    p.buf_ok = buffer_offsets_ok(d, bch, esz) && !(f & DBG_GLOBAL_ADDR);
    *out = p;
    return 0;
  };
  auto generic = [&]() { return pick(CONV_GENERIC, ch_tile, ch_tile == 128 ? 128 : 256); };
  auto small = [&](int bch) {
    p.ksplit = m32_ksplit_choice(d, f, ((d.M + 127) / 128) * ((d.Cout + bch - 1) / bch), n_cu, bch, 4);
    p.identity_residual = ident_ok && d.Cout % 256 == 0;
    return pick(CONV_M32_SMALL, bch, 128);
  };

  if (d.out_f32) {
    RGBM_REQUIRE(dtype == BF16X3 && d.w2 == nullptr, "out_f32 is a bf16x3 option of the generic kernel");
    return generic();
  }
  if (ch_tile == 128 && !(f & DBG_NO_WS) && ws_rows) {
    if (!uni || (f & DBG_V3_FOR_WS) || !rows16) return pick(CONV_V3, 128, 256);
    if (!(f & DBG_NO_SLIM_SMALL) && d.Cout % 64 == 0) {
      const long long slim_tiles = ((d.M + 255) / 256) * (d.Cout / 64);
      if (mfma32) {
        if (d.Cout % 256 == 0 && ((d.M + 255) / 256) * (d.Cout / 256) < n_cu && t.gemm_kernel >= 1 && !(f & (DBG_M32_TAILS_R5 | DBG_WS_128x256)) &&
            buffer_offsets_ok(d, 256, esz)) {
          const int bch = t.gemm_kernel == 1 ? 256 : m32_small_choice(d, n_cu, slim_tiles <= n_cu);
          if (bch) return small(bch);
        }
        if (d.Cout == 128 && ((d.M + 127) / 128) * 2 * 2 <= n_cu && t.gemm_kernel == 2 &&
            !(f & (DBG_M32_TAILS_R5 | DBG_WS_128x256 | DBG_NO_KSPLIT | DBG_L2_SLIM_TILE)) && d.w2 == nullptr && buffer_offsets_ok(d, 64, esz))
          return small(64);
      }
      if (slim_tiles <= n_cu) return pick(CONV_WS_SLIM, 64, 256);
    }
    if (d.Cout % 256 == 0 && !(f & DBG_WS_128x256)) {
      if (!(mfma32 && buffer_offsets_ok(d, 256, esz) && t.gemm_kernel >= 1)) return pick(CONV_WS_WIDE, 256, 128);
      const bool big_ok = dense_out && (d.bias == nullptr || (d.bias_stride == 0 && d.Cout <= 2560)) && d.act != ACT_TANH &&
                          (d.res_mode == RES_NONE || (d.res_mode == RES_PRE_ACT && d.res != nullptr)) && d.M * d.ldo * esz < (1ll << 32) - 65536;
      const long long P = d.M / 256, n_ch = d.Cout / 256, tiles = P * n_ch;
      long long Pm = 0;
      if (t.gemm_kernel != 1 && big_ok && tiles >= n_cu) {
        const long long rem = tiles % n_cu;
        Pm = (rem == 0 || rem * 10 >= (long long)n_cu * 6) ? P : (tiles - rem) / n_ch;
      }
      p.main_rows = Pm * 256;
      p.identity_residual = ident_ok;
      p.border = p.main_rows > 0 && p.korder == 1 && uni && border_applies(d, dtype, f, p.main_rows);
      p.tail_bch = p.main_rows == d.M ? 0 : 256;
      const long long pt = (d.M - p.main_rows + 127) / 128;
      if (p.tail_bch && t.gemm_kernel != 1 && !(f & DBG_M32_TAILS_R5)) {
        if (pt * (d.Cout / 64) <= n_cu) p.tail_bch = 64;
        else if (pt * (d.Cout / 128) <= n_cu) p.tail_bch = 128;
      }
      return pick(CONV_M32, 256, 256);
    }
    return pick(CONV_WS, 128, 256);
  }
  if (bits16 && uni && !(f & DBG_NO_WS64) && ch_tile == 64 && d.res_mode == RES_NONE && d.KT >= 2 && ws_rows &&
      (d.w2 ? d.Cout == 64 && d.kpad2 == 64 && (d.cout2 == 16 || d.cout2 == 32) && d.ldo2 % 4 == 0 : out16))
    return rowhalo_ok(d) && !(f & DBG_NO_ROWHALO) ? pick(CONV_WS64_ROWHALO, 64, 256) : pick(CONV_WS64, 64, 256);
  RGBM_REQUIRE(d.w2 == nullptr, "a fused 1x1 needs the ws64 kernel (check conv_ws64_eligible first)");
  if (ch_tile == 64 && uni && ws_rows && !(f & (DBG_NO_WS | DBG_V3_FOR_WS | DBG_NO_SLIM64)) && rows16) return pick(CONV_WS_SLIM, 64, 256);
  return generic();
}

}
```

rgbmanip_amd/csrc/conv_plan.h:

```cpp
#pragma once
#include <vector>

#include "common.h"

namespace rgbm {

struct ConvTuning {
  int flags;
  int gemm_kernel;
  long long ws_min_rows;
  int n_cu;
};

enum ConvKernel {
  CONV_GENERIC = 0,
  CONV_V3 = 1,
  CONV_WS = 2,
  CONV_WS_WIDE = 3,
  CONV_WS_SLIM = 4,
  CONV_WS64 = 5,
  CONV_WS64_ROWHALO = 6,
  CONV_M32 = 7,
  CONV_M32_SMALL = 8,
};

struct ConvPlan {
  int kernel;
  int bch, bpix;
  bool uniform_taps;
  long long main_rows;
  int tail_bch;
  int ksplit;
  bool identity_residual;
  int korder, buf_ok;
  bool border;
};

struct BorderClass {
  int kh0, kh1, kw0, kw1;
  int mask;
  int n_pix;
  int pix0;
  long long row0;
};
struct BorderTile {
  int cls, ch;
  int mask;
  int steps;
  long long row0;
};
struct BorderPlan {
  int n_wg, n_ch, kr, steps_per_tap;
  std::vector<BorderClass> classes;
  std::vector<int> pix;
  std::vector<BorderTile> tiles;
  std::vector<int> order;
  std::vector<int> wg_off;
  std::vector<int> rows;
  long long total_steps, parent_steps, max_wg_steps;
};
bool border_applies(const ConvDesc& d, int dtype, int flags, long long main_rows);
bool plan_border(const ConvDesc& d, int dtype, int flags, long long main_rows, int n_wg, BorderPlan* out);

constexpr size_t kM32SplitFloats = 8u << 20, kM32SplitCounters = 16384;

int plan_conv(const ConvDesc& d, int dtype, const ConvTuning& t, ConvPlan* out);
int conv_tuning(int n_cu, ConvTuning* t);

}
```

rgbmanip_amd/csrc/kernels.h:

```cpp
#pragma once
#include <vector>

#include "common.h"

namespace rgbm {

int launch_nchw_to_nhwc_pad(int dtype, const float* in, void* out, int V, int C, int H, int W, int Cp, hipStream_t s);
int launch_maxpool3x3s2(int dtype, const void* in, void* out, int V, int H, int W, int C, hipStream_t s);
int launch_resize_bilinear_ac(int dtype, const void* in, void* out, int V, int Hs, int Ws, int C, int Ho, int Wo, int ldo,
                              int ch_off, hipStream_t s);
int launch_copy_channels(int dtype, const void* in, void* out, long long npix, int C, int ldo, int ch_off, hipStream_t s);
int launch_adaptive_avgpool(int dtype, const void* in, void* out, int V, int H, int W, int C, int S, hipStream_t s);
int launch_adaptive_avgpool_multi(int dtype, const void* in, void* const* outs, const int* bins, int nb, int V, int H, int W, int C,
                                  hipStream_t s);
int launch_psp_pool_conv(int dtype, const void* in, int ldi, const void* const* w, void* const* outs, const int* bins, int V, int H, int W,
                         int act, float slope, hipStream_t s);
int launch_psp_resize_cat(int dtype, const void* f, const void* const* stages, const int* bins, void* out, int V, int Ho, int Wo, hipStream_t s);
int launch_homography(const float* P_views, float* out, int V, int B, hipStream_t s);
int launch_build_volume(int dtype, const void* feat, const float* homog, const float* depths, void* vol, int v0, int Vc, int V,
                        int B, int D, int H, int W, hipStream_t s);

int launch_upconv_combine(int dtype, const void* z, const float* bias, void* out, int V, int h, int w, int Co, int ldo, int act,
                          float slope, hipStream_t s, const float* drop = nullptr);
int launch_upconv_final(int dtype, const void* x, const void* wz, const float* bias, float slope, const void* wf, const float* biasf,
                        void* out, int out_f32, int V, int h, int w, hipStream_t s, const void* wf_f16 = nullptr);

constexpr int kDropoutPerView = 256 + 64;
unsigned dropout_threshold(float p);
float dropout_scale(float p);
int launch_dropout_masks(float* masks, unsigned long long* state, int B, float p, unsigned long long seed, int advance, hipStream_t s);

size_t bn_scratch_bytes(int V);
int launch_bn_per_sample(int dtype, void* y, const void* res, const float* gamma, const float* beta, void* scratch, int V,
                         long long nvox, int C, int relu, hipStream_t s);

int launch_to_f32(int dtype, const void* in, float* out, long long n, hipStream_t s);

int launch_gather_points(int dtype, const void* feat, const int* choose, float* out, int V, int P, int HW, int C, hipStream_t s);
int launch_prob_softmax_depth(int dtype, const void* u11, const float* wprob, const int* choose, const float* depths,
                              float* prob, float* depth_out, int v0, int Vc, int B, int P, int D, int H, int W, int classmajor,
                              hipStream_t s);
int launch_dense_depth(int dtype, const void* u11, const float* wprob, const float* depths, float* depth_map, float* conf_map,
                       int v0, int Vc, int B, int D, int H, int W, int classmajor, hipStream_t s);
int launch_depth_to_points(const float* depth, const double* Kc, const double* E, int n, int S, float* points, hipStream_t s);
int launch_depth_consistency(const float* depth_a, const float* conf_a, const unsigned char* mask_a, const double* Ka, const double* Ea,
                             const float* depth_b, const double* Kb, const double* Eb, int n, int S, double px_max, double rel_max,
                             float conf_min, float* fused, float* reproj, float* rel, unsigned char* keep, hipStream_t s);
int launch_cloud_pack(const float* fused1, const unsigned char* keep1, const double* K1, const double* E1, const float* fused2,
                      const unsigned char* keep2, const double* K2, const double* E2, int n, int S, int cap, float* cloud, int* index,
                      int* count, hipStream_t s);
int launch_depth_fusion(const float* depth, const float* conf, const unsigned char* mask, const double* Kc, const double* E, int n, int V,
                        int S, double px_max, double rel_max, float conf_min, int n_min, float* fused, unsigned char* keep,
                        unsigned char* nviews, unsigned short* agree, hipStream_t s);
int launch_cloud_pack_views(const float* fused, const unsigned char* keep, const double* Kc, const double* E, int n, int V, int S, int cap,
                            float* cloud, int* index, int* count, hipStream_t s);
int launch_cloud_gather_views(const float* maps, const int* index, int n, int V, int S2, int C, int cap, float* out, hipStream_t s);
int launch_fuse_points(int dtype, const void* feat, const float* homog, const float* depths, const int* choose,
                       const float* prob, float* out, int V, int B, int P, int D, int H, int W, int ldo, int ch_off,
                       hipStream_t s, int Vn = -1);
int launch_mean_points(int dtype, const void* in, float* out, float* scratch, int V, int P, int C, hipStream_t s);
int launch_f32_to_f16(const float* in, void* out, long long n, hipStream_t s);
void stem_pack(const float* w, std::vector<float>& packed);
int launch_stem(int dtype, const float* img1, const float* img2, const void* wpk, void* out, int B, int V, int S, hipStream_t s);
int launch_stem_views(int dtype, const float* img, const void* wpk, void* out, int V, int S, hipStream_t s);
int launch_feature_store(const void* src, void* pool, const int* slots, int V, int pool_records, size_t part_off, size_t part_bytes,
                         size_t record_bytes, hipStream_t s);
int launch_feature_gather(const void* pool, void* dst, const int* slot1, const int* slot2, int B, int pool_records, size_t part_off,
                          size_t part_bytes, size_t record_bytes, hipStream_t s);
int launch_feature_bad_slot_nan(const int* slot1, const int* slot2, int B, int pool_records, float* const out[10], const int per_pose[10],
                                hipStream_t s);
int launch_crop_fingerprint(const float* img, int V, int n_words, unsigned long long* keys_out, hipStream_t s);
int launch_f32_to_bx3(const float* in, void* out, long long n, hipStream_t s);
int launch_view_linear(const float* x, const float* W, const float* bias, float* out, int V, int I, int O, int ldw, int i0,
                       int relu, hipStream_t s);
struct PointMlpDesc {
  const float* table;
  const void* feat;
  const int* choose;
  float* nocs4;
  float* pf;
  int ldpf, P, HW;
  long long N;
};
int point_mlp_table_floats();
void point_mlp_pack(const float* const w[6], const float* const b[6], float* table);
int launch_point_mlp(int feat_dtype, const PointMlpDesc& d, hipStream_t s);
int launch_dense_nocs(int feat_dtype, const float* table, const void* feat, float* out, long long N, hipStream_t s);
int launch_ortho6d(const float* r6, float* R, int V, hipStream_t s);
int launch_mean_points_partial(int dtype, const void* in, float* scratch, int V, int P, int C, hipStream_t s);
int launch_view_linear_mean(const float* partial, int P, float* mean_out, const float* W, const float* bias, float* out, int V, int I, int O,
                            int ldw, int i0, int relu, hipStream_t s);
int launch_pose_heads_mean(const float* partial, int P, float* mean_out, float* R, float* const w[3][3], float* const b[3][3],
                           float* const out[3], const int odim[3], int V, hipStream_t s);
constexpr int kMeanSplit = 8;
constexpr int kPoseMlpSlab = 128;
struct PoseMlpDesc {
  const float* pf96;
  const void* w[4];
  int ldw[4];
  const float* bias[4];
  const float* vbias;
  void* q128;
  float* part128;
  float* part256;
  int V, P;
};
bool pose_mlp_fits(int P);
int launch_pose_mlp1(const PoseMlpDesc& d, hipStream_t s);
int launch_pose_mlp2(const PoseMlpDesc& d, hipStream_t s);
int launch_pose_heads(const float* pf2, float* const w[3][3], float* const b[3][3], float* const out[3], const int odim[3], int V,
                      hipStream_t s);
int launch_stage_in(const float* P1, const float* P2, const int* c1, const int* c2, float* Pviews, int* choose, int B, int P, hipStream_t s);
int launch_stage_out(const float* nocs4, const float* depth, const float* R, const float* tv, const float* sv, float* const nocs[2],
                     float* const dep[2], float* const r[2], float* const t[2], float* const sz[2], int B, int P, int view2, hipStream_t s);
int launch_copy_cols(const float* in, float* out, long long rows, int ldi, int ldo, int n, hipStream_t s);

struct Conv3dTileDesc {
  const void* in; const void* wgt; void* out; const float* bias; const void* res;
  int N, Di, Hi, Wi;
  int Do, Ho, Wo;
  int Dq, Hq, Wq;
  int ntd, nth, ntw;
  int Cout, relu;
  const void* feat; const float* homog; const float* depths; int v0, V, B;
  int prof_variant; double algo_flops, algo_bytes;
  int out_classmajor;
  int feat_f16;
  const int* tile_list; const int* tile_count;
  int tile_mask_stride;
  const unsigned char* tile_mask;
};
enum DebugFlag {
  DBG_NO_WS = 8, DBG_NONUNIFORM_TAPS = 16, DBG_V3_FOR_WS = 64, DBG_NO_WS64 = 128, DBG_NO_ROWHALO = 256, DBG_GENERIC_RESIZE = 512,
  DBG_PSP_STAGE_R5 = 1024, DBG_POINT_MLP_R5 = 2048, DBG_TILE_CONV0 = 4096, DBG_NO_KSPLIT = 16384, DBG_L2_SLIM_TILE = 32768,
  DBG_WS_128x256 = 65536, DBG_NO_SLIM64 = 262144, DBG_KORDER_TAPS_OUTER = 1 << 20, DBG_SWEEP_ALT_BLEND = 1 << 21, DBG_SWEEP_DOT2 = 1 << 22,
  DBG_PP_ONE_KERNEL = 1 << 23, DBG_NO_SLIM_SMALL = 1 << 24, DBG_PP_GENERIC_SELECT = 1 << 25, DBG_PP_GUARD = 1 << 26, DBG_GLOBAL_ADDR = 1 << 27,
  DBG_SWEEP_PER_TILE = 1 << 28, DBG_SPARSE_TAIL_R5 = 1 << 29, DBG_M32_TAILS_R5 = 1 << 30, DBG_POSE_MLP_R6 = 1 << 19, DBG_NO_BORDER_TILES = 32,
};
extern int g_debug_flags;
long long border_launch_count();
extern long long g_ws_min_rows;
extern int g_tuning_version;
extern int g_gemm_kernel;
void conv3d_tile_pack(const float* w, const float* scale, int Cin, int Cout, int coutp, bool transposed, int dtype,
                      std::vector<float>& packed);
int launch_conv3d_tile(int layer, int dtype, const Conv3dTileDesc& d, hipStream_t s);
int sparse_mask_bytes_per_view(int S);
int sparse_mask_offset(int S, int layer);
int launch_sparse_masks(const int* choose, int v0, int Vc, int P, int S, unsigned char* masks, int* sweep_list, int* sweep_count,
                        hipStream_t s);
int conv3d_tile_dims(int layer, int dtype, int* TD, int* TH, int* TW);

void conv0_sweep_pack(const float* w, const float* scale, std::vector<float>& packed);
int launch_conv0_sweep(const Conv3dTileDesc& d, int dtype, hipStream_t s);

int conv0_sweep_x3_upload(const std::vector<float>& packed, void** dev);
int launch_conv0_sweep_x3(const Conv3dTileDesc& d, hipStream_t s);
int launch_bx3_to_f32(const void* in, float* out, long long n, hipStream_t s);

int launch_prob_sparse(const void* u9, const void* c0, const void* w11_packed, const float* bias11, const float* wprob,
                       const int* choose, const float* depths, float* prob, float* depth_out, int v0, int Vc, int B, int P,
                       int D, int H, int W, int dtype, hipStream_t s, const void* w11_taps = nullptr);
void prob_sparse_pack(const float* w, const float* scale, std::vector<float>& packed);

int launch_prepare_inputs(const float* rgb, const unsigned char* mask, const double* K, const int* frame_map, int N, int H, int W, int S, int P,
                          unsigned seed, float* img, int* choose, float* pts2d, double* Kcrop, int* window, int* valid,
                          unsigned char* small_scratch, hipStream_t s, int frame0 = 0);
int launch_prepare_inputs_u8(const unsigned char* rgb, const unsigned char* mask, const double* K, const int* frame_map, int N, int H, int W,
                             int S, int P, unsigned seed, float* img, int* choose, float* pts2d, double* Kcrop, int* window, int* valid,
                             unsigned char* small_scratch, hipStream_t s, int frame0 = 0);
int launch_prepare_inputs_opt(const void* rgb, int pixel_type, int normalize, const unsigned char* mask, const double* K, const int* frame_map,
                              int N, int H, int W, int S, int P, unsigned seed, float* img, int* choose, float* pts2d, double* Kcrop,
                              int* window, int* valid, unsigned char* small_scratch, hipStream_t s, int frame0 = 0);
int launch_prepare_inputs_windows(const void* pix, int pixel_type, int normalize, const unsigned char* mask_pix, const long long* offset,
                                  const int* window, const int* valid_in, const double* K, int frame0, int N, int H, int W, int S, int P,
                                  unsigned seed, float* img, int* choose, float* pts2d, double* Kcrop, int* valid, unsigned char* small_scratch,
                                  hipStream_t s);
int launch_quantize_frames(const float* src, unsigned char* dst, size_t n, hipStream_t s);

int launch_umeyama_ransac(const float* nocs, const float* depth, const int* choose, const double* Kc, const double* E1,
                          double* bbox, double* srt, int* valid, int B, int P, int img, unsigned seed, hipStream_t s);

int launch_cloud_gather(const float* map1, const float* map2, const int* index, int n, int S2, int C, int cap, float* out, hipStream_t s);
size_t cloud_similarity_scratch_bytes(int n, int cap);
int launch_cloud_similarity(const float* nocs, const float* cloud, const int* count, int n, int cap, unsigned seed, double* bbox, double* srt,
                            int* info, int* valid, void* scratch, size_t scratch_bytes, hipStream_t s);

int launch_projection(const double* Kc, const double* E, float* P, int n, hipStream_t s);
int launch_pnp_ransac(const float* nocs1, const float* pts1, const float* nocs2, const float* pts2, const double* K, const double* E1,
                      const double* E2, double* bbox, double* srt, int* info, int* valid, int B, int P, unsigned seed, hipStream_t s);

int launch_mask_extent(const unsigned char* mask, int N, int H, int W, int* ext, int* count, hipStream_t s);

int launch_postprocess(const float* nocs, const float* depth, const float* rot, const int* choose, const double* Kc,
                       const double* E1, double* bbox, double* ts_out, int* valid, int B, int P, int img, hipStream_t s,
                       void* scratch = nullptr, size_t scratch_bytes = 0);
int launch_postprocess_regressed(const float* nocs, const float* rot, const float* tr, const float* sv, const double* E1, double* bbox,
                                 double* ts_out, int* valid, int B, int P, hipStream_t s);
int launch_microbench_mfma(float* scratch, int iters, int random_operands, double* flops, hipStream_t s);
int microbench_mfma_scratch_floats(int* n);
int launch_microbench_copy(const void* src, void* dst, size_t bytes, hipStream_t s);
size_t postprocess_scratch_bytes(int B);
int postprocess_slices(int B);

int launch_gae(int T, int N, const float* rewards, const unsigned char* dones, const float* values, const float* last_values,
               float gamma, float lam, float* returns, float* adv, double* sums, hipStream_t s);
int launch_adv_normalise(long long n_local, float* adv, const double* sums, double count_total, hipStream_t s);

struct PolicyLayout { int dims[5]; int log_std; int w[2][4]; int b[2][4]; int total; };
struct PolicyOptState { int t; int n_updates; float lr; float last_kl; float last_norm; float pad_; double sum_surr; double sum_vloss; };
int launch_policy_forward(const float* params, const PolicyLayout& L, int n, int mode, const float* obs, const float* noise,
                          float* actions, float* logp, float* value, float* mu, hipStream_t s);
int policy_partial_floats(const PolicyLayout& L, int n);
int launch_ppo_minibatch(const float* params, const PolicyLayout& L, int n, const float* obs, const float* actions,
                         const float* old_logp, const float* adv, const float* returns, const float* old_values,
                         const float* old_mu, const float* old_sigma, float clip, float vcoef, float ecoef, float* partial,
                         float* grads, hipStream_t s);
constexpr int POLICY_MAX_HIDDEN = 6, POLICY_MAX_WIDTH = 512, POLICY_MAX_ACT = 32;
enum { PACT_ELU = 0, PACT_SELU = 1, PACT_RELU = 2, PACT_LRELU = 3, PACT_TANH = 4, PACT_SIGMOID = 5 };
struct PolicyDesc {
  int obs_dim, state_dim, act_dim, activation, asymmetric;
  int n_hidden[2];
  int hidden[2][POLICY_MAX_HIDDEN];
  int w[2][POLICY_MAX_HIDDEN + 1];
  int b[2][POLICY_MAX_HIDDEN + 1];
  int log_std, total;
};
int launch_policy_forward_ex(const float* params, const PolicyDesc& D, int n, int mode, const float* obs, const float* states,
                             const float* noise, float* actions, float* logp, float* value, float* mu, hipStream_t s);
int ppo_scratch_floats_ex(const PolicyDesc& D, int n, int clipped_vloss, size_t* count);
int launch_ppo_minibatch_ex(const float* params, const PolicyDesc& D, int n, const float* obs, const float* states,
                            const float* actions, const float* old_logp, const float* adv, const float* returns,
                            const float* old_values, const float* old_mu, const float* old_sigma, float clip, float vcoef, float ecoef,
                            int clipped_vloss, float* scratch, float* grads, hipStream_t s);
int launch_ppo_adam(float* params, const float* grads, float* m, float* v, PolicyOptState* st, int total, float inv_world,
                    float max_norm, float desired_kl, float lr_min, float lr_max, int adaptive, hipStream_t s);

}
```

rgbmanip_amd/csrc/layers.cpp:

```cpp
#include "layers.h"
#include "conv_plan.h"
#include "kernels.h"

#include <string.h>

#include <array>
#include <map>
#include <mutex>
#include <utility>
#include <vector>

namespace rgbm {

static thread_local std::string g_err;
void set_error(const std::string& s) { g_err = s; }
const char* last_error_cstr() { return g_err.c_str(); }

static inline unsigned short host_f32_to_bf16(float f) {
  unsigned u;
  memcpy(&u, &f, 4);
  if ((u & 0x7fffffffu) > 0x7f800000u) return (unsigned short)((u >> 16) | 0x40);
  u += 0x7fffu + ((u >> 16) & 1u);
  return (unsigned short)(u >> 16);
}

int ensure_dynamic_lds(const void* fn, int bytes) {
  static std::mutex mu;
  static std::map<std::pair<int, const void*>, int> set_for;
  int dev = 0;
  RGBM_CHECK_HIP(hipGetDevice(&dev));
  std::lock_guard<std::mutex> lock(mu);
  int& have = set_for[std::make_pair(dev, fn)];
  if (bytes > have) {
    RGBM_CHECK_HIP(hipFuncSetAttribute(fn, hipFuncAttributeMaxDynamicSharedMemorySize, bytes));
    have = bytes;
  }
  return 0;
}

int persistent_grid_cus(int* n_cu) {
  static std::mutex mu;
  static std::map<int, int> per_dev;
  int dev = 0;
  RGBM_CHECK_HIP(hipGetDevice(&dev));
  std::lock_guard<std::mutex> lock(mu);
  int& n = per_dev[dev];
  if (n == 0) {
    RGBM_CHECK_HIP(hipDeviceGetAttribute(&n, hipDeviceAttributeMultiprocessorCount, dev));
    n = n / 8 * 8;
    if (n < 8) n = 8;
  }
  *n_cu = n;
  return 0;
}

static int upload_bytes(const void* host, size_t bytes, DevBuf& dev) {
  RGBM_CHECK_HIP(hipMalloc(dev.out(), bytes));
  RGBM_CHECK_HIP(hipMemcpy(dev.get(), host, bytes, hipMemcpyHostToDevice));
  return 0;
}

int upload_f32(const float* host, size_t n, DevBuf& dev) { return upload_bytes(host, n * sizeof(float), dev); }

static inline unsigned short host_f32_to_f16(float f) {
  const _Float16 h = (_Float16)(f > 65504.f ? 65504.f : (f < -65504.f ? -65504.f : f));
  unsigned short u;
  memcpy(&u, &h, 2);
  return u;
}

bool weights_fit_f16(const std::vector<float>& w) {
  double total = 0.0, small = 0.0;
  for (float v : w) {
    const float a = v < 0.f ? -v : v;
    if (!(a < 65504.f)) return false;
    total += a;
    if (a != 0.f && a < 6.103515625e-05f) small += a;
  }
  return small <= 1e-3 * total;
}

int upload_packed(const std::vector<float>& w, int dtype, DevBuf& dev) {
  if (dtype == BF16 || dtype == F16) {
    std::vector<unsigned short> h(w.size());
    for (size_t i = 0; i < w.size(); ++i) h[i] = dtype == BF16 ? host_f32_to_bf16(w[i]) : host_f32_to_f16(w[i]);
    return upload_bytes(h.data(), h.size() * 2, dev);
  }
  if (dtype == BF16X3) {
    RGBM_REQUIRE(w.size() % 4 == 0, "bf16x3 weights: element count must be a multiple of 4");
    std::vector<unsigned> h(w.size());
    for (size_t i = 0; i < w.size(); i += 4) {
      unsigned short hi[4], lo[4];
      for (int e = 0; e < 4; ++e) {
        hi[e] = host_f32_to_bf16(w[i + e]);
        unsigned u = (unsigned)hi[e] << 16;
        float hf;
        memcpy(&hf, &u, 4);
        lo[e] = host_f32_to_bf16(w[i + e] - hf);
      }
      h[i] = hi[0] | ((unsigned)hi[1] << 16); h[i + 1] = hi[2] | ((unsigned)hi[3] << 16);
      h[i + 2] = lo[0] | ((unsigned)lo[1] << 16); h[i + 3] = lo[2] | ((unsigned)lo[3] << 16);
    }
    return upload_bytes(h.data(), h.size() * 4, dev);
  }
  return upload_bytes(w.data(), w.size() * 4, dev);
}

int conv_pack_geom(const ConvGeom& g, int dtype, int Cin_pad, int Cout_pad, int cls, PackedConv* pc) {
  const int BK = conv_bk(dtype);
  RGBM_REQUIRE(Cin_pad % dtype_chunk(dtype) == 0 && Cin_pad >= g.Cin, "Cin_pad");
  RGBM_REQUIRE(Cout_pad % 4 == 0 && Cout_pad >= g.Cout, "Cout_pad");
  *pc = PackedConv();
  if (!g.transposed) {
    pc->KD = g.KD; pc->KH = g.KH; pc->KW = g.KW;
  } else {
    RGBM_REQUIRE(g.KD == 3 && g.KH == 3 && g.KW == 3 && g.sd == 2 && g.sh == 2 && g.sw == 2, "transposed conv geometry");
    RGBM_REQUIRE(cls >= 0 && cls < 8, "sub-pixel class");
    pc->KD = 1 + ((cls >> 2) & 1); pc->KH = 1 + ((cls >> 1) & 1); pc->KW = 1 + (cls & 1);
  }
  pc->ntaps = pc->KD * pc->KH * pc->KW;
  if (pc->ntaps > 1 || g.transposed) RGBM_REQUIRE(is_pow2(Cin_pad), "multi-tap / transposed conv needs power-of-two Cin_pad");
  const int K = pc->ntaps * Cin_pad;
  pc->Kpad = (K + BK - 1) / BK * BK;
  pc->KT = pc->Kpad / BK;
  return 0;
}

struct BorderTables {
  struct Entry { DevBuf buf; int n_wg = 0, b_ent = 0, b_rows = 0; };
  std::mutex mu;
  std::map<std::array<long long, 7>, Entry> per_shape;
};

int ConvLayer::init(int dtype_, const ConvGeom& g_, const float* w, const float* bias_h, const float* bn_scale,
                    const float* bn_shift, int Cin_pad_, int Cout_pad_) {
  g = g_;
  dtype = dtype_;
  Cin_pad = Cin_pad_;
  Cout_pad = Cout_pad_;
  PackedConv pc;
  if (int rc = conv_pack_geom(g, dtype, Cin_pad, Cout_pad, 0, &pc)) return rc;
  const int bch = conv_ch_tile(Cout_pad);
  const int rows = (Cout_pad + bch - 1) / bch * bch;

  if (bias_h || bn_shift) {
    std::vector<float> b(Cout_pad, 0.f);
    for (int o = 0; o < g.Cout; ++o) {
      float v = bias_h ? bias_h[o] : 0.f;
      if (bn_scale) v *= bn_scale[o];
      if (bn_shift) v += bn_shift[o];
      b[o] = v;
    }
    if (upload_f32(b.data(), b.size(), bias)) return -2;
  }

  auto finish = [&](PackedConv& pc, std::vector<float>& packed) -> int {
    if (upload_packed(packed, dtype, pc.w)) return -2;
    packs.push_back(std::move(pc));
    return 0;
  };

  if (!g.transposed) {
    std::vector<float> packed((size_t)rows * pc.Kpad, 0.f);
    const long long kvol = (long long)g.KD * g.KH * g.KW;
    for (int o = 0; o < g.Cout; ++o) {
      const float sc = bn_scale ? bn_scale[o] : 1.f;
      for (int c = 0; c < g.Cin; ++c)
        for (int t = 0; t < pc.ntaps; ++t)
          packed[(size_t)o * pc.Kpad + (size_t)t * Cin_pad + c] = w[((long long)o * g.Cin + c) * kvol + t] * sc;
    }
    w_finite = true;
    for (float v : packed)
      if (!((v < 0.f ? -v : v) <= 3.3895313892515355e38f)) { w_finite = false; break; }
    border = std::make_shared<BorderTables>();
    return finish(pc, packed);
  }

  for (int cls = 0; cls < 8; ++cls) {
    const int pd_ = (cls >> 2) & 1, ph_ = (cls >> 1) & 1, pw_ = cls & 1;
    if (int rc = conv_pack_geom(g, dtype, Cin_pad, Cout_pad, cls, &pc)) return rc;
    std::vector<float> packed((size_t)rows * pc.Kpad, 0.f);
    auto kidx = [](int p, int delta) { return p == 0 ? 1 : (delta == 0 ? 2 : 0); };
    for (int o = 0; o < g.Cout; ++o) {
      const float sc = bn_scale ? bn_scale[o] : 1.f;
      for (int c = 0; c < g.Cin; ++c)
        for (int dd = 0; dd < pc.KD; ++dd)
          for (int dh = 0; dh < pc.KH; ++dh)
            for (int dw = 0; dw < pc.KW; ++dw) {
              const int t = (dd * pc.KH + dh) * pc.KW + dw;
              const int kd = kidx(pd_, dd), kh = kidx(ph_, dh), kw = kidx(pw_, dw);
              packed[(size_t)o * pc.Kpad + (size_t)t * Cin_pad + c] =
                  w[(((long long)c * g.Cout + o) * 3 + kd) * 9 + kh * 3 + kw] * sc;
            }
    }
    if (finish(pc, packed)) return -2;
  }
  return 0;
}

void conv_out_dims(const ConvGeom& g, int Di, int Hi, int Wi, int& Do, int& Ho, int& Wo) {
  if (g.transposed) { Do = 2 * Di; Ho = 2 * Hi; Wo = 2 * Wi; return; }
  Do = (Di + 2 * g.pd - g.dild * (g.KD - 1) - 1) / g.sd + 1;
  Ho = (Hi + 2 * g.ph - g.dilh * (g.KH - 1) - 1) / g.sh + 1;
  Wo = (Wi + 2 * g.pw - g.dilw * (g.KW - 1) - 1) / g.sw + 1;
}

void ConvLayer::out_dims(int Di, int Hi, int Wi, int& Do, int& Ho, int& Wo) const { conv_out_dims(g, Di, Hi, Wi, Do, Ho, Wo); }

void conv_desc_geom(ConvDesc& d, const ConvGeom& g, const PackedConv& pc, int Cin_pad, int Cout_pad, int N, int Di, int Hi, int Wi,
                    int ldo, int cls) {
  memset(&d, 0, sizeof(d));
  conv_out_dims(g, Di, Hi, Wi, d.Do, d.Ho, d.Wo);
  d.N = N; d.Di = Di; d.Hi = Hi; d.Wi = Wi;
  d.Cin = Cin_pad;
  d.Cout = Cout_pad; d.ldo = ldo;
  d.act = g.act; d.slope = g.slope;
  d.KD = pc.KD; d.KH = pc.KH; d.KW = pc.KW;
  d.ntaps = pc.ntaps; d.KT = pc.KT; d.Kpad = pc.Kpad;
  d.lcin = (pc.ntaps > 1 || is_pow2(Cin_pad)) ? ilog2(Cin_pad) : -1;
  if (g.transposed) {
    d.Dq = Di; d.Hq = Hi; d.Wq = Wi;
    d.sd = d.sh = d.sw = 1; d.pd = d.ph = d.pw = 0;
    d.dild = d.dilh = d.dilw = 1;
    d.osd = d.osh = d.osw = 2;
    d.opd = (cls >> 2) & 1; d.oph = (cls >> 1) & 1; d.opw = cls & 1;
  } else {
    d.Dq = d.Do; d.Hq = d.Ho; d.Wq = d.Wo;
    d.sd = g.sd; d.sh = g.sh; d.sw = g.sw; d.pd = g.pd; d.ph = g.ph; d.pw = g.pw;
    d.dild = g.dild; d.dilh = g.dilh; d.dilw = g.dilw;
    d.osd = d.osh = d.osw = 1;
    d.opd = d.oph = d.opw = 0;
  }
  d.M = (long long)N * d.Dq * d.Hq * d.Wq;
}

int ConvLayer::build_desc(ConvDesc& d, const void* in, void* out, int N, int Di, int Hi, int Wi, int ldo, const void* res,
                          int res_mode, const float* bias_override, int bias_stride, int cls, bool out_plain_f32) const {
  RGBM_REQUIRE(!packs.empty(), "conv layer not initialised");
  const PackedConv& pc = packs[cls];
  conv_desc_geom(d, g, pc, Cin_pad, Cout_pad, N, Di, Hi, Wi, ldo, cls);
  d.in = in; d.out = out; d.res = res; d.wgt = pc.w.get();
  d.bias = bias_override ? bias_override : bias.get<float>();
  d.bias_stride = bias_override ? bias_stride : 0;
  d.res_mode = res ? res_mode : RES_NONE;
  d.out_f32 = (out_plain_f32 && dtype == BF16X3) ? 1 : 0;
  d.w_finite = w_finite ? 1 : 0;
  d.algo_flops = 2.0 * (double)d.M * g.Cout * (double)pc.ntaps * g.Cin;
  d.algo_bytes = ((double)d.M * g.Cout + (cls == 0 ? (double)N * Di * Hi * Wi * g.Cin : 0.0) +
                  (res ? (double)d.M * g.Cout : 0.0)) * (double)dtype_size(dtype) +
                 (double)g.Cout * pc.ntaps * g.Cin * (double)dtype_size(dtype);
  return 0;
}

int ConvLayer::attach_border(ConvDesc& d, hipStream_t s) const {
  if (!border || !w_finite || g.transposed || dtype == F32 || g.KH * g.KW == 1) return 0;
  ConvTuning t;
  ConvPlan p;
  if (int rc = conv_tuning(0, &t)) return rc;
  if (int rc = plan_conv(d, dtype, t, &p)) return rc;
  if (p.kernel != CONV_M32 || !p.border) return 0;
  int dev = 0;
  RGBM_CHECK_HIP(hipGetDevice(&dev));
  const std::array<long long, 7> key = {dev, d.N, d.Hi, d.Wi, t.n_cu, p.identity_residual ? 1 : 0, p.main_rows};
  std::lock_guard<std::mutex> lock(border->mu);
  auto it = border->per_shape.find(key);
  if (it == border->per_shape.end()) {
    hipStreamCaptureStatus cs = hipStreamCaptureStatusNone;
    if (hipStreamIsCapturing(s, &cs) == hipSuccess && cs != hipStreamCaptureStatusNone) return 0;
    BorderPlan bp;
    if (!plan_border(d, dtype, t.flags, p.main_rows, t.n_cu, &bp)) return 0;
    std::vector<int> tab(bp.wg_off);
    BorderTables::Entry e;
    e.n_wg = bp.n_wg;
    e.b_ent = (int)tab.size();
    for (int i : bp.order) {
      const BorderTile& bt = bp.tiles[i];
      const BorderClass& bc = bp.classes[bt.cls];
      tab.push_back((int)bt.row0);
      tab.push_back(bt.steps - bp.kr);
      tab.push_back(bc.kh0 | bc.kh1 << 4 | bc.kw0 << 8 | bc.kw1 << 12 | bt.ch << 16);
      tab.push_back(0);
    }
    e.b_rows = (int)tab.size();
    tab.insert(tab.end(), bp.rows.begin(), bp.rows.end());
    RGBM_CHECK_HIP(hipMalloc(e.buf.out(), tab.size() * sizeof(int)));
    RGBM_CHECK_HIP(hipMemcpy(e.buf.get(), tab.data(), tab.size() * sizeof(int), hipMemcpyHostToDevice));
    it = border->per_shape.emplace(key, std::move(e)).first;
  }
  d.btab = it->second.buf.get<int>();
  d.b_nwg = it->second.n_wg; d.b_ent = it->second.b_ent; d.b_rows = it->second.b_rows;
  return 0;
}

int ConvLayer::run(const void* in, void* out, int N, int Di, int Hi, int Wi, int ldo, const void* res, int res_mode,
                   const float* bias_override, int bias_stride, hipStream_t s, bool out_plain_f32) const {
  const int nclass = g.transposed ? 8 : 1;
  for (int cls = 0; cls < nclass; ++cls) {
    ConvDesc d;
    if (int rc = build_desc(d, in, out, N, Di, Hi, Wi, ldo, res, res_mode, bias_override, bias_stride, cls, out_plain_f32)) return rc;
    if (int rc = attach_border(d, s)) return rc;
    if (int rc = launch_conv(d, dtype, s)) return rc;
  }
  return 0;
}

int ConvLayer::run_then_1x1(const ConvLayer& next, const void* in, void* mid, int ldmid, void* out2, int ldo2, int N, int Di, int Hi,
                            int Wi, bool allow_fuse, bool* fused, hipStream_t s, bool out2_plain_f32) const {
  if (fused) *fused = false;
  const ConvGeom& ng = next.g;
  const bool is1x1 = !ng.transposed && ng.KD == 1 && ng.KH == 1 && ng.KW == 1 && ng.sd == 1 && ng.sh == 1 && ng.sw == 1 &&
                     ng.pd == 0 && ng.ph == 0 && ng.pw == 0 && next.packs.size() == 1;
  if (allow_fuse && is1x1 && !g.transposed && dtype_size(dtype) == 2 && next.dtype == dtype && next.Cin_pad == Cout_pad) {
    ConvDesc d;
    if (int rc = build_desc(d, in, mid, N, Di, Hi, Wi, ldmid, nullptr, RES_NONE, nullptr, 0, 0)) return rc;
    d.w2 = next.packs[0].w.get(); d.bias2 = next.bias.get<float>(); d.out2 = out2; d.ldo2 = ldo2; d.cout2 = next.Cout_pad;
    d.kpad2 = next.packs[0].Kpad; d.act2 = ng.act; d.slope2 = ng.slope;
    if (conv_ws64_eligible(d, dtype)) {
      d.algo_flops += 2.0 * (double)d.M * ng.Cout * ng.Cin;
      d.algo_bytes += ((double)d.M * ng.Cout - (double)d.M * g.Cout) * 2.0;
      if (int rc = launch_conv(d, dtype, s)) return rc;
      if (fused) *fused = true;
      return 0;
    }
  }
  if (int rc = run(in, mid, N, Di, Hi, Wi, ldmid, nullptr, RES_NONE, nullptr, 0, s)) return rc;
  int Do, Ho, Wo;
  out_dims(Di, Hi, Wi, Do, Ho, Wo);
  return next.run(mid, out2, N, Do, Ho, Wo, ldo2, nullptr, RES_NONE, nullptr, 0, s, out2_plain_f32);
}

int UpConvLayer::init(int dtype, int Cin, int Cout_, const float* w, const float* bias_h, int act_, float slope_) {
  Cout = Cout_; act = act_; slope = slope_;
  RGBM_REQUIRE(Cout % dtype_chunk(dtype) == 0, "upconv Cout must be a multiple of the 16-byte chunk");
  std::vector<float> wz((size_t)9 * Cout * Cin);
  for (int t = 0; t < 9; ++t)
    for (int o = 0; o < Cout; ++o)
      for (int c = 0; c < Cin; ++c) wz[((size_t)t * Cout + o) * Cin + c] = w[((size_t)o * Cin + c) * 9 + t];
  ConvGeom g;
  g.Cin = Cin; g.Cout = 9 * Cout; g.act = ACT_NONE;
  split = (dtype != F32 && 9 * Cout > 256 && (9 * Cout) % 256 != 0 && (9 * Cout) % 256 <= 64 && Cin % 64 == 0) ? (9 * Cout) / 256 * 256 : 0;
  if (split) {
    ConvGeom g1 = g, g2 = g;
    g1.Cout = split; g2.Cout = 9 * Cout - split;
    if (int rc = gemm.init(dtype, g1, wz.data(), nullptr, nullptr, nullptr, Cin, g1.Cout)) return rc;
    if (int rc = gemm2.init(dtype, g2, wz.data() + (size_t)split * Cin, nullptr, nullptr, nullptr, Cin, g2.Cout)) return rc;
  } else {
    if (int rc = gemm.init(dtype, g, wz.data(), nullptr, nullptr, nullptr, Cin, 9 * Cout)) return rc;
  }
  if (bias_h) { if (upload_f32(bias_h, Cout, bias)) return -2; }
  return 0;
}

int UpConvLayer::run_gemm(const void* in, void* z, int V, int h, int w, hipStream_t s) const {
  if (int rc = gemm.run(in, z, V, 1, h, w, 9 * Cout, nullptr, RES_NONE, nullptr, 0, s)) return rc;
  if (split)
    if (int rc = gemm2.run(in, reinterpret_cast<char*>(z) + (size_t)split * dtype_size(gemm.dtype), V, 1, h, w, 9 * Cout, nullptr, RES_NONE, nullptr, 0, s)) return rc;
  return 0;
}

int UpConvLayer::combine(const void* z, void* out, int V, int h, int w, int ldo, hipStream_t s, const float* drop) const {
  return launch_upconv_combine(gemm.dtype, z, bias.get<float>(), out, V, h, w, Cout, ldo, act, slope, s, drop);
}

int UpConvLayer::run(const void* in, void* z, void* out, int V, int h, int w, int ldo, hipStream_t s, const float* drop) const {
  if (int rc = run_gemm(in, z, V, h, w, s)) return rc;
  return combine(z, out, V, h, w, ldo, s, drop);
}

int UpConvFinal::init(int dtype_, const float* w3, const float* b3, float slope_, const float* wfin, const float* bfin) {
  RGBM_REQUIRE(dtype_ == BF16 || dtype_ == F16 || dtype_ == BF16X3, "upconv + final: 16-bit or split-pair storage");
  dtype = dtype_; slope = slope_;
  std::vector<float> z((size_t)9 * 64 * 64), f(wfin, wfin + 32 * 64);
  for (int t = 0; t < 9; ++t)
    for (int o = 0; o < 64; ++o)
      for (int c = 0; c < 64; ++c) z[((size_t)t * 64 + o) * 64 + c] = w3[((size_t)o * 64 + c) * 9 + t];
  if (int rc = upload_packed(z, dtype, wz)) return rc;
  if (int rc = upload_packed(f, dtype, wf)) return rc;
  if (dtype == BF16 && weights_fit_f16(f)) if (int rc = upload_packed(f, F16, wf_h)) return rc;
  if (upload_f32(b3, 64, bias) || upload_f32(bfin, 32, biasf)) return -2;
  return 0;
}

int UpConvFinal::run(const void* in, void* out, int out_kind, int V, int h, int w, hipStream_t s) const {
  return launch_upconv_final(dtype, in, wz.get(), bias.get<float>(), slope, wf.get(), biasf.get<float>(), out, out_kind, V, h, w, s, wf_h.get());
}

}
```

Before: 6030.

## Fold M32 conv tail tiles into the border-table main launch

Adds a 'fold' mode to the M32 implicit-GEMM conv kernel. The leftover pixel rows after the main range, normally run in a separate tail launch, are instead split into 128-pixel tiles and handed to the persistent workgroups of the main launch via a greedy least-loaded assignment stored in the border table. This removes a kernel launch and the tail's poor occupancy. In exchange it enlarges the LDS ring, adds a second producer/consumer pipeline inside the kernel, and relies on a heuristic cost model (step weight, tail launch cost) to decide when folding is used.

```diff
diff --git a/include/rgbm.h b/include/rgbm.h
--- a/include/rgbm.h
+++ b/include/rgbm.h
@@ -248,6 +248,11 @@
                           int32_t* head, int32_t* classes, int cap_classes, int32_t* tiles, int32_t* order, int cap_tiles, int32_t* wg_off,
                           int cap_wg, int32_t* rows, int64_t cap_rows);
 int rgbm_conv_border_launches(int64_t* count);
+#define RGBM_FOLD_HEAD_INTS 8
+int rgbm_conv_fold_plan(int dtype, int N, int H, int W, int Cin, int Cout, int K, int stride, int pad, int dil, int res_mode, int n_cu,
+                        int32_t* head, double* costs, int32_t* tiles, int32_t* order, int cap_tiles, int32_t* wg_off, int32_t* barriers,
+                        int cap_wg);
+int rgbm_conv_fold_launches(int64_t* count);
 int rgbm_bn_per_sample_scratch_bytes(int V, size_t* bytes);
 int rgbm_bn_per_sample(int dtype, void* y_dev, const void* res_dev, const float* gamma_dev, const float* beta_dev, void* scratch_dev,
                        int V, int64_t nvox, int C, int relu, void* stream);
diff --git a/rgbmanip_amd/_lib.py b/rgbmanip_amd/_lib.py
--- a/rgbmanip_amd/_lib.py
+++ b/rgbmanip_amd/_lib.py
@@ -158,6 +158,9 @@
     "rgbm_conv_border_plan": (_i, [_i] * 12 + [C.POINTER(C.c_int32)] * 2 + [_i] + [C.POINTER(C.c_int32)] * 2 + [_i, C.POINTER(C.c_int32), _i,
                                    C.POINTER(C.c_int32), _i64]),
     "rgbm_conv_border_launches": (_i, [C.POINTER(C.c_int64)]),
+    "rgbm_conv_fold_plan": (_i, [_i] * 12 + [C.POINTER(C.c_int32), C.POINTER(C.c_double)] + [C.POINTER(C.c_int32)] * 2 + [_i] +
+                                 [C.POINTER(C.c_int32)] * 2 + [_i]),
+    "rgbm_conv_fold_launches": (_i, [C.POINTER(C.c_int64)]),
     "rgbm_bn_per_sample_scratch_bytes": (_i, [_i, C.POINTER(_sz)]),
     "rgbm_bn_per_sample": (_i, [_i, _vp, _vp, _vp, _vp, _vp, _i, _i64, _i, _i, _vp]),
     "rgbm_conv3d_tile": (_i, [_i, _i, _vp, _i, _i, _i, _i, _vp, _vp, _vp, _vp, _vp, _vp]),
diff --git a/rgbmanip_amd/csrc/capi.cpp b/rgbmanip_amd/csrc/capi.cpp
--- a/rgbmanip_amd/csrc/capi.cpp
+++ b/rgbmanip_amd/csrc/capi.cpp
@@ -666,6 +666,69 @@
   return 0;
 }
 
+int rgbm_conv_fold_plan(int dtype, int N, int H, int W, int Cin, int Cout, int K, int stride, int pad, int dil, int res_mode, int n_cu,
+                        int32_t* head, double* costs, int32_t* tiles, int32_t* order, int cap_tiles, int32_t* wg_off, int32_t* barriers,
+                        int cap_wg) {
+  RGBM_REQUIRE(head && n_cu >= 0 && dtype >= F32 && dtype <= BF16X3 && N > 0 && H > 0 && W > 0 && K > 0, "conv_fold_plan arguments");
+  const ConvGeom g = conv_nd_geom(Cin, Cout, 1, K, K, 1, stride, 0, pad, dil, 0, ACT_RELU, 0.f);
+  PackedConv pc;
+  const int E = dtype_chunk(dtype);
+  const int Cin_pad = (Cin + E - 1) / E * E, Cout_pad = (Cout + 3) / 4 * 4;
+  if (int rc = conv_pack_geom(g, dtype, Cin_pad, Cout_pad, 0, &pc)) return rc;
+  ConvDesc d;
+  conv_desc_geom(d, g, pc, Cin_pad, Cout_pad, N, 1, H, W, Cout_pad, 0);
+  alignas(16) static const float buffer[4] = {};
+  d.in = d.wgt = buffer; d.out = const_cast<float*>(buffer);
+  d.res = res_mode != RES_NONE ? buffer : nullptr;
+  d.res_mode = res_mode;
+  d.w_finite = 1;
+  ConvTuning t;
+  ConvPlan p;
+  if (int rc = conv_tuning(n_cu, &t)) return rc;
+  if (int rc = plan_conv(d, dtype, t, &p)) return rc;
+  memset(head, 0, RGBM_FOLD_HEAD_INTS * sizeof(int32_t));
+  if (costs) costs[0] = costs[1] = costs[2] = costs[3] = 0.0;
+  BorderPlan bp;
+  FoldPlan fp;
+  if (p.kernel != CONV_M32 || !p.border || !plan_border(d, dtype, t.flags, p.main_rows, t.n_cu, &bp)) return 0;
+  if (!fold_eligible(d, dtype, t.flags, p)) return 0;
+  const bool taken = plan_fold(d, dtype, t.flags, p, bp, &fp);
+  const int steps = d.KT + fp.kr;
+  const int32_t h[RGBM_FOLD_HEAD_INTS] = {taken ? 1 : 0, (int32_t)fp.tiles.size(), fp.n_wg, fp.n_pix, fp.n_ch, steps, fp.kr, 1};
+  memcpy(head, h, sizeof(h));
+  if (costs) { costs[0] = fp.max_cost_folded; costs[1] = (double)fp.max_cost_main; costs[2] = fp.weight; costs[3] = fp.tail_launch; }
+  if (tiles || order) RGBM_REQUIRE((int)fp.tiles.size() <= cap_tiles, "conv_fold_plan: cap_tiles too small");
+  if (tiles)
+    for (size_t i = 0; i < fp.tiles.size(); ++i) {
+      const int32_t v[3] = {fp.tiles[i].pix, fp.tiles[i].ch, fp.tiles[i].steps};
+      memcpy(tiles + 3 * i, v, sizeof(v));
+    }
+  if (order) memcpy(order, fp.order.data(), fp.order.size() * sizeof(int32_t));
+  if (wg_off || barriers) RGBM_REQUIRE(fp.n_wg + 1 <= cap_wg, "conv_fold_plan: cap_wg too small");
+  if (wg_off) memcpy(wg_off, fp.wg_off.data(), fp.wg_off.size() * sizeof(int32_t));
+  if (barriers)
+    for (int b = 0; b < fp.n_wg; ++b) {
+      int32_t req1 = 0, mul1 = 0, mul2 = 0;
+      for (int i = bp.wg_off[b]; i < bp.wg_off[b + 1]; ++i) {
+        const int ent_steps = bp.tiles[bp.order[i]].steps - bp.kr;
+        req1 += ent_steps + bp.kr;
+        mul1 += (ent_steps - 1) + 1 + bp.kr + 1;
+      }
+      req1 += bp.wg_off[b + 1] - bp.wg_off[b];
+      for (int i = fp.wg_off[b]; i < fp.wg_off[b + 1]; ++i) mul2 += d.KT + fp.kr;
+      const int32_t req2 = (fp.wg_off[b + 1] - fp.wg_off[b]) * steps;
+      const int32_t v[5] = {req1, mul1, req2, mul2, req2};
+      memcpy(barriers + 5 * b, v, sizeof(v));
+    }
+  return 0;
+}
+
+int rgbm_conv_fold_launches(int64_t* count) {
+  RGBM_REQUIRE(count, "conv_fold_launches arguments");
+  *count = fold_launch_count();
+  return 0;
+}
+
 int rgbm_conv_border_launches(int64_t* count) {
   RGBM_REQUIRE(count, "conv_border_launches arguments");
   *count = border_launch_count();
diff --git a/rgbmanip_amd/csrc/common.h b/rgbmanip_amd/csrc/common.h
--- a/rgbmanip_amd/csrc/common.h
+++ b/rgbmanip_amd/csrc/common.h
@@ -239,6 +239,7 @@
   int out_f32;
   int ksplit; float* kscratch; unsigned* kcount;
   int w_finite; const int* btab; int b_nwg, b_ent, b_rows;
+  int b_fold; long long f_m0, f_M;
 };
 
 int launch_conv(const ConvDesc& d, int dtype, hipStream_t s);
diff --git a/rgbmanip_amd/csrc/conv_igemm_m32.inc b/rgbmanip_amd/csrc/conv_igemm_m32.inc
--- a/rgbmanip_amd/csrc/conv_igemm_m32.inc
+++ b/rgbmanip_amd/csrc/conv_igemm_m32.inc
@@ -81,7 +81,24 @@
     ch_tile = lid - pix_tile * d.n_ch_tiles;
   };
 
-  float* lbias = reinterpret_cast<float*>(lds3 + NST * STAGE);
+  constexpr bool FOLD = STAGED && !X3;
+  constexpr int BPIX2 = 128, XR2 = BPIX2 / 32, STAGE2 = (BCH + BPIX2) * 8, NP2 = XR2 + WL;
+  constexpr int RING = FOLD && 3 * STAGE2 > NST * STAGE ? 3 * STAGE2 : NST * STAGE;
+  bool fold = false;
+  int n2 = 0;
+  const int* __restrict__ fent = d.btab;
+  if constexpr (FOLD) {
+    if (bm && d.b_fold > 0) {
+      const int* ft = d.btab + d.b_fold;
+      const int f0 = ft[blockIdx.x];
+      fold = true;
+      n2 = __builtin_amdgcn_readfirstlane(ft[blockIdx.x + 1] - f0);
+      fent = ft + d.b_nwg + 1 + f0;
+    }
+  }
+  const int KR2 = res_in_acc ? BCH / BK : 0, KTT2 = d.KT + KR2, total2 = n2 * KTT2;
+
+  float* lbias = reinterpret_cast<float*>(lds3 + RING);
   const bool bias_lds = d.bias != nullptr && d.bias_stride == 0 && d.Cout <= 2560;
   if (bias_lds)
     for (int i = tid; i < d.Cout; i += NTH) lbias[i] = d.bias[i];
@@ -114,12 +131,12 @@
     int ikt = 0, itile = 0;
     int KTc = KT, KTTc = KTT, bkh0 = 0, bkh1 = 0, bkw0 = 0, bkw1 = 0, mym = -1;
     int* lrow = reinterpret_cast<int*>(lbias + 2560);
-    auto decode_my = [&](long long m) {
+    auto decode_my = [&](long long m, long long Mend, bool tab) {
       mybase = 0;
       mymask = 0;
       if (j < XR) {
         int xn = 0, xd0 = -(1 << 20), xh0 = 0, xw0 = 0;
-        if (m >= 0 && m < d.M) {
+        if (m >= 0 && m < Mend) {
           unsigned n, qd, qh, qw;
           decode_row(d, (unsigned)m, n, qd, qh, qw);
           xn = (int)n * d.Di;
@@ -130,7 +147,7 @@
         for (int kk = 0; kk < d.KD; ++kk) mymask |= (unsigned)((unsigned)(xd0 + kk * d.dild) < (unsigned)d.Di) << kk;
         for (int kk = 0; kk < d.KH; ++kk) mymask |= (unsigned)((unsigned)(xh0 + kk * d.dilh) < (unsigned)d.Hi) << (8 + kk);
         for (int kk = 0; kk < d.KW; ++kk) mymask |= (unsigned)((unsigned)(xw0 + kk * d.dilw) < (unsigned)d.Wi) << (16 + kk);
-        if (bm) mymask = m >= 0 ? 0x00ffffffu : 0u;
+        if (tab) mymask = m >= 0 ? 0x00ffffffu : 0u;
         const long long pix0 = ((long long)(xn + xd0) * d.Hi + xh0) * d.Wi + xw0;
         mybase = pix0 * d.Cin * (long long)sizeof(T);
       }
@@ -148,12 +165,12 @@
         mym = j < XR ? d.btab[d.b_rows + __builtin_amdgcn_readfirstlane(bent[4 * k]) + r0 + 32 * j] : -1;
         return;
       }
-      decode_my(d.m0 + (long long)pix_tile * BPIX + r0 + 32 * j);
+      decode_my(d.m0 + (long long)pix_tile * BPIX + r0 + 32 * j, d.M, bm);
     };
     auto enter_tile = [&]() {
       const int grp = (tp & 63) & 56;
       if (bm) {
-        decode_my(mym);
+        decode_my(mym, d.M, bm);
         if (j < XR) lrow[(itile & 1) * 256 + r0 + 32 * j] = mym;
         asm volatile("s_waitcnt lgkmcnt(0)" ::: "memory");
       }
@@ -252,6 +269,75 @@
       else { if (g + 1 < total) issue(st ^ 1); }
       st = st == NST - 1 ? 0 : st + 1;
       if (STAGED) { if (++gk == gKTT) { gk = 0; RGBM_BARRIER(); if (++gtile < n_my) gKTT = bsteps(gtile) + KR; } }
+    }
+    if constexpr (FOLD) {
+      if (fold) {
+        RGBM_BARRIER();
+        const __amdgpu_buffer_rsrc_t rsrc_r2 = __builtin_amdgcn_make_buffer_rsrc(
+            const_cast<char*>(reinterpret_cast<const char*>(d.res)), 0, (int)(unsigned)(d.f_M * d.ldo * (long long)sizeof(T)), 0x00020000);
+        int ikt2 = 0, it2 = 0;
+        auto prepare2 = [&](int k) {
+          const int e = __builtin_amdgcn_readfirstlane(fent[k]);
+          my_pix_tile = e & 0xffff;
+          my_ch_tile = e >> 16;
+          decode_my(d.f_m0 + (long long)my_pix_tile * BPIX2 + r0 + 32 * j, d.f_M, false);
+        };
+        auto enter2 = [&]() {
+          const int grp = (tp & 63) & 56;
+#pragma unroll
+          for (int i = 0; i < XR2; ++i) {
+            const long long b = __shfl(mybase, grp | i, 64);
+            rmask[i] = (unsigned)__shfl((int)mymask, grp | i, 64);
+            xoff[i] = (unsigned)(b + xbias + (long long)(js * E) * (long long)sizeof(T));
+            if (KR2) {
+              const long long m = d.f_m0 + (long long)my_pix_tile * BPIX2 + r0 + 32 * i;
+              roff[i] = m < d.f_M ? (unsigned)((m * d.ldo + my_ch_tile * BCH + js * E) * (long long)sizeof(T)) : 0xffffffffu;
+            }
+          }
+#pragma unroll
+          for (int i = 0; i < WL; ++i) {
+            const int row = r0 + 32 * i;
+            woff[i] = (unsigned)(((long long)(my_ch_tile * BCH + row) * d.Kpad + js * E) * (long long)sizeof(T));
+          }
+          tkd = tkh = tkw = tc = 0;
+          wko = 0;
+        };
+        auto issue2 = [&](int stage) {
+          if (ikt2 == 0) enter2();
+          const unsigned sbase = lds0 + (unsigned)stage * (STAGE2 * 16);
+          const unsigned sel = 1u | (256u << tkh) | (65536u << tkw);
+          const unsigned soff = (unsigned)(((long long)(tkh * d.dilh * d.Wi + tkw * d.dilw) * d.Cin + tc) * (long long)sizeof(T));
+          const bool cok = tc + js * E < d.Cin;
+          if (ikt2 >= d.KT) {
+            const unsigned ro = (unsigned)(ikt2 - d.KT) * (unsigned)(BK * sizeof(T));
+#pragma unroll
+            for (int i = 0; i < XR2; ++i) blds16(roff[i], rsrc_r2, ro, sbase + (BCH * 8 + i * 256) * 16);
+#pragma unroll
+            for (int i = 0; i < WL; ++i) blds16((unsigned)(((r0 + 32 * i) * 256 + js * E) * (int)sizeof(T)), rsrc_i, ro, sbase + (i * 256) * 16);
+          } else {
+#pragma unroll
+            for (int i = 0; i < XR2; ++i) {
+              const bool ok = cok && (rmask[i] & sel) == sel;
+              blds16(ok ? xoff[i] : 0xffffffffu, rsrc_x, soff, sbase + (BCH * 8 + i * 256) * 16);
+            }
+#pragma unroll
+            for (int i = 0; i < WL; ++i) blds16(woff[i], rsrc_w, wko, sbase + (i * 256) * 16);
+            wko += (unsigned)d.Cin * (unsigned)sizeof(T);
+            if (++tkw == d.KW) { tkw = 0; if (++tkh == d.KH) { tkh = 0; tc += BK; wko = (unsigned)tc * (unsigned)sizeof(T); } }
+          }
+          if (++ikt2 == KTT2) { ikt2 = 0; ++it2; if (it2 < n2) prepare2(it2); }
+        };
+        if (total2 > 0) { prepare2(0); issue2(0); }
+        if (total2 > 1) issue2(1);
+        int st2 = 0;
+        for (int g = 0; g < total2; ++g) {
+          if (g + 1 >= total2) asm volatile("s_waitcnt vmcnt(0)" ::: "memory");
+          else asm volatile("s_waitcnt vmcnt(%0)" :: "n"(NP2) : "memory");
+          RGBM_BARRIER();
+          if (g + 2 < total2) issue2(st2 == 0 ? 2 : st2 - 1);
+          st2 = st2 == 2 ? 0 : st2 + 1;
+        }
+      }
     }
     return;
   }
@@ -734,15 +820,146 @@
       }
     }
   }
+
+  if constexpr (FOLD) {
+    if (!fold) return;
+    asm volatile("s_waitcnt lgkmcnt(0)" ::: "memory");
+    RGBM_BARRIER();
+    if (wave >= 4) {
+      for (int g = 0; g < total2; ++g) RGBM_BARRIER();
+      return;
+    }
+    constexpr int CHK2 = 16 / (int)sizeof(T), NQ2 = 16 / CHK2;
+    const int wch2 = (wave >> 1) * WCHW, wpix2 = (wave & 1) * 64;
+    const int rowA2 = wch2 + m32_row_channel(li), rowB2 = wpix2 + li;
+    unsigned oA2 = (unsigned)(rowA2 * 8 + (lh ^ ((rowA2 >> 1) & 7))) * 16u;
+    unsigned oB2 = (unsigned)(BCH * 8 + rowB2 * 8 + (lh ^ ((rowB2 >> 1) & 7))) * 16u;
+    int st2 = 0;
+    for (int k = 0; k < n2; ++k) {
+      const int ent = __builtin_amdgcn_readfirstlane(fent[k]);
+      const int pt = ent & 0xffff, ct = ent >> 16;
+      const bool interior2 = (d.bias == nullptr || bias_lds) && d.f_m0 + (long long)(pt + 1) * BPIX2 <= d.f_M && d.act != ACT_TANH;
+      if (interior2 && d.bias) {
+        const float* bp = lbias + ct * BCH + wch2 + lh * 16;
+#pragma unroll
+        for (int a = 0; a < FA; ++a) {
+          f32x16 b16;
+#pragma unroll
+          for (int q = 0; q < 4; ++q) {
+            const f32x4 b4 = *reinterpret_cast<const f32x4*>(bp + a * 32 + q * 4);
+            b16[q * 4 + 0] = b4[0]; b16[q * 4 + 1] = b4[1]; b16[q * 4 + 2] = b4[2]; b16[q * 4 + 3] = b4[3];
+          }
+#pragma unroll
+          for (int b = 0; b < FB; ++b) acc[a][b] = b16;
+        }
+      } else {
+#pragma unroll
+        for (int a = 0; a < FA; ++a)
+#pragma unroll
+          for (int b = 0; b < FB; ++b)
+#pragma unroll
+            for (int e = 0; e < 16; ++e) acc[a][b][e] = 0.f;
+      }
+      uint4 A2[FA], B2[FB], Bn2[FB];
+      for (int kt = 0; kt < KTT2; ++kt) {
+        asm volatile("s_waitcnt lgkmcnt(0)" ::: "memory");
+        RGBM_BARRIER();
+        asm volatile("" : "+v"(oA2), "+v"(oB2));
+        const char* base = ldsc + st2 * (STAGE2 * 16);
+#pragma unroll
+        for (int b = 0; b < FB; ++b) B2[b] = *reinterpret_cast<const uint4*>(base + oB2 + b * 4096);
+#pragma unroll
+        for (int a = 0; a < FA; ++a) A2[a] = *reinterpret_cast<const uint4*>(base + oA2 + a * 4096);
+        __builtin_amdgcn_sched_barrier(0);
+#pragma unroll
+        for (int s = 0; s < 4; ++s) {
+          if (s < 3) {
+#pragma unroll
+            for (int b = 0; b < FB; ++b) Bn2[b] = *reinterpret_cast<const uint4*>(base + (oB2 ^ ((unsigned)(s + 1) << 5)) + b * 4096);
+          }
+          __builtin_amdgcn_sched_barrier(0);
+#pragma unroll
+          for (int a = 0; a < FA; ++a) {
+            Mma32<T>::run(A2[a], B2[0], acc[a][0]);
+            Mma32<T>::run(A2[a], B2[1], acc[a][1]);
+            __builtin_amdgcn_sched_barrier(0);
+            if (s < 3) A2[a] = *reinterpret_cast<const uint4*>(base + (oA2 ^ ((unsigned)(s + 1) << 5)) + a * 4096);
+            __builtin_amdgcn_sched_barrier(0);
+          }
+          if (s < 3) { B2[0] = Bn2[0]; B2[1] = Bn2[1]; }
+        }
+        st2 = st2 == 2 ? 0 : st2 + 1;
+      }
+      const long long mrow = d.f_m0 + (long long)pt * BPIX2 + wpix2;
+      const int ch0 = ct * BCH + wch2;
+      if (interior2) {
+        const float nslope = d.act == ACT_RELU ? 0.f : d.act == ACT_PRELU ? d.slope : 1.f;
+        unsigned lofs_c = (unsigned)((li * d.ldo + lh * 16) * (int)sizeof(T));
+        asm volatile("" : "+v"(lofs_c));
+        uint4 pk[FA][NQ2];
+#pragma unroll
+        for (int b = 0; b < FB; ++b) {
+#pragma unroll
+          for (int a = 0; a < FA; ++a) {
+#pragma unroll
+            for (int q = 0; q < NQ2; ++q) {
+              float v[CHK2];
+#pragma unroll
+              for (int e = 0; e < CHK2; ++e) v[e] = acc[a][b][q * CHK2 + e];
+#pragma unroll
+              for (int e = 0; e < CHK2; ++e) v[e] = v[e] < 0.f ? __builtin_fmaxf(v[e], -3.402823466e38f) * nslope : v[e];
+              pk[a][q] = pack_chunk(v, T());
+            }
+            __builtin_amdgcn_sched_barrier(0);
+          }
+#pragma unroll
+          for (int a = 0; a < FA; ++a)
+#pragma unroll
+            for (int q = 0; q < NQ2; ++q)
+              *reinterpret_cast<uint4*>(reinterpret_cast<char*>(out + (mrow + b * 32) * d.ldo + ch0 + a * 32) + lofs_c + q * 16) = pk[a][q];
+          __builtin_amdgcn_sched_barrier(0);
+        }
+        continue;
+      }
+#pragma unroll
+      for (int a = 0; a < FA; ++a) {
+        const int chL = ch0 + a * 32 + lh * 16;
+#pragma unroll
+        for (int b = 0; b < FB; ++b) {
+          const long long m = mrow + b * 32 + li;
+          if (m >= d.f_M) continue;
+#pragma unroll
+          for (int q = 0; q < NQ2; ++q) {
+            const int c = chL + q * CHK2;
+            float v[CHK2];
+#pragma unroll
+            for (int e = 0; e < CHK2; ++e) v[e] = acc[a][b][q * CHK2 + e];
+            if (d.bias) {
+#pragma unroll
+              for (int e = 0; e < CHK2; ++e) v[e] += d.bias[c + e];
+            }
+#pragma unroll
+            for (int e = 0; e < CHK2; ++e) v[e] = apply_act_g(v[e], d.act, d.slope);
+            *reinterpret_cast<uint4*>(out + m * d.ldo + c) = pack_chunk(v, T());
+          }
+        }
+      }
+    }
+  }
 }
 
+static std::atomic<long long> g_fold_launches{0};
+long long fold_launch_count() { return g_fold_launches.load(std::memory_order_relaxed); }
 static std::atomic<long long> g_border_launches{0};
 long long border_launch_count() { return g_border_launches.load(std::memory_order_relaxed); }
 
 template <typename T, int BPIX, int BCH = 256>
 static int launch_m32_range(ConvDesc d, hipStream_t s) {
   constexpr int NST = BPIX == 256 ? 2 : 3;
-  constexpr size_t LDS = ((size_t)NST * (BCH + BPIX) * 8) * sizeof(uint4) + 2560 * sizeof(float) + (BPIX == 256 && BCH == 256 ? 2 * 256 * sizeof(int) : 0);
+  constexpr bool FOLD = BPIX == 256 && BCH == 256 && !std::is_same<T, bx3_t>::value;
+  constexpr size_t RING = FOLD && 3 * (BCH + 128) * 8 > NST * (BCH + BPIX) * 8 ? 3 * (BCH + 128) * 8 : NST * (BCH + BPIX) * 8;
+  constexpr size_t LDS = RING * sizeof(uint4) + 2560 * sizeof(float) + (BPIX == 256 && BCH == 256 ? 2 * 256 * sizeof(int) : 0);
+  static_assert(LDS <= 160 * 1024, "a CU's LDS");
   d.n_pix_tiles = (int)((d.M - d.m0 + BPIX - 1) / BPIX);
   d.n_ch_tiles = (d.Cout + BCH - 1) / BCH;
   const long long ntiles = (long long)d.n_pix_tiles * d.n_ch_tiles;
@@ -758,6 +975,9 @@
   const int grid = d.ksplit > 1 ? (int)(ntiles * d.ksplit) : ntiles < n_cu ? (int)ntiles : n_cu;
   RGBM_REQUIRE(d.btab == nullptr || (BPIX == 256 && BCH == 256 && d.m0 == 0 && grid == d.b_nwg), "border-class table: made for another grid");
   if (d.btab) g_border_launches.fetch_add(1, std::memory_order_relaxed);
+  if (d.btab == nullptr || !(BPIX == 256 && BCH == 256) || std::is_same<T, bx3_t>::value) d.b_fold = 0;
+  RGBM_REQUIRE(d.b_fold == 0 || (d.f_m0 == d.M && d.f_M > d.M && d.f_M < (1ll << 31)), "folded tail: rows behind the main launch's");
+  if (d.b_fold) g_fold_launches.fetch_add(1, std::memory_order_relaxed);
   prof_begin_launch(s, BPIX == 256 && BCH == 256 ? (std::is_same<T, bx3_t>::value ? 33 : 31) : (std::is_same<T, bx3_t>::value ? 41 : 40), d.algo_flops, d.algo_bytes);
   hipLaunchKernelGGL((conv_igemm_m32_kernel<T, BPIX, BCH>), dim3((unsigned)grid), dim3(BPIX == 256 ? 768 : 512), LDS, s, d);
   prof_end_launch(s);
@@ -840,6 +1060,15 @@
 static int launch_m32(ConvDesc d, const ConvPlan& p, hipStream_t s) {
   if (int rc = m32_setup<T>(d, p, s)) return rc;
   if (!p.border) d.btab = nullptr;
+  const bool fold = p.border && d.btab && d.b_fold > 0 && fold_eligible(d, std::is_same<T, f16_t>::value ? F16 : std::is_same<T, bx3_t>::value ? BF16X3 : BF16, g_debug_flags, p);
+  if (fold) {
+    ConvDesc m = d;
+    m.M = p.main_rows;
+    m.f_m0 = p.main_rows;
+    m.f_M = d.M;
+    return launch_m32_range<T, 256, 256>(m, s);
+  }
+  d.b_fold = 0;
   if (p.main_rows > 0) {
     ConvDesc m = d;
     m.M = p.main_rows;
diff --git a/rgbmanip_amd/csrc/conv_plan.cpp b/rgbmanip_amd/csrc/conv_plan.cpp
--- a/rgbmanip_amd/csrc/conv_plan.cpp
+++ b/rgbmanip_amd/csrc/conv_plan.cpp
@@ -213,6 +213,60 @@
   return true;
 }
 
+constexpr double kFoldStepWeight = 0.5;
+constexpr double kFoldTailLaunchPerStep = 0.29;
+
+bool fold_eligible(const ConvDesc& d, int dtype, int flags, const ConvPlan& p) {
+  if (p.kernel != CONV_M32 || !p.border || p.tail_bch == 0 || p.main_rows <= 0 || p.main_rows >= d.M || p.korder != 1) return false;
+  if ((flags & (DBG_NO_FOLD_TAIL | DBG_NO_BORDER_TILES | DBG_KORDER_TAPS_OUTER)) || !(dtype == BF16 || dtype == F16)) return false;
+  if (d.KD != 1 || d.lcin < 0 || (d.M - p.main_rows + 127) / 128 >= 65536) return false;
+  return d.res_mode == RES_NONE || p.identity_residual;
+}
+
+bool plan_fold(const ConvDesc& d, int dtype, int flags, const ConvPlan& p, const BorderPlan& bp, FoldPlan* out) {
+  if (!fold_eligible(d, dtype, flags, p)) return false;
+  if (bp.n_wg <= 0 || (int)bp.wg_off.size() != bp.n_wg + 1 || bp.n_ch != d.Cout / 256) return false;
+  FoldPlan f;
+  f.n_wg = bp.n_wg;
+  f.n_ch = bp.n_ch;
+  f.n_pix = (int)((d.M - p.main_rows + 127) / 128);
+  f.kr = p.identity_residual ? 256 / conv_bk(dtype) : 0;
+  f.weight = kFoldStepWeight;
+  const int steps = d.KT + f.kr;
+  for (int t = 0; t < f.n_pix; ++t)
+    for (int ch = 0; ch < f.n_ch; ++ch) f.tiles.push_back(FoldTile{t, ch, steps});
+  const long long tail_tiles = (long long)f.n_pix * (d.Cout / p.tail_bch);
+  f.tail_launch = (double)((tail_tiles + f.n_wg - 1) / f.n_wg) * steps * kFoldTailLaunchPerStep;
+  typedef std::pair<double, std::pair<int, int>> Load;
+  std::priority_queue<Load, std::vector<Load>, std::greater<Load>> q;
+  const int per_xcd = (f.n_wg + 7) / 8;
+  f.max_cost_main = 0;
+  for (int b = 0; b < f.n_wg; ++b) {
+    long long s = 0;
+    for (int i = bp.wg_off[b]; i < bp.wg_off[b + 1]; ++i) s += bp.tiles[bp.order[i]].steps;
+    if (s > f.max_cost_main) f.max_cost_main = s;
+    q.push(Load((double)s, std::make_pair((b & 7) * per_xcd + (b >> 3), b)));
+  }
+  std::vector<std::vector<int>> mine(f.n_wg);
+  f.max_cost_folded = (double)f.max_cost_main;
+  for (size_t i = 0; i < f.tiles.size(); ++i) {
+    Load l = q.top();
+    q.pop();
+    mine[l.second.second].push_back((int)i);
+    l.first += f.tiles[i].steps * f.weight;
+    if (l.first > f.max_cost_folded) f.max_cost_folded = l.first;
+    q.push(l);
+  }
+  f.wg_off.assign(1, 0);
+  for (int b = 0; b < f.n_wg; ++b) {
+    for (int i : mine[b]) f.order.push_back(i);
+    f.wg_off.push_back((int)f.order.size());
+  }
+  const bool taken = f.max_cost_folded < (double)f.max_cost_main + f.tail_launch;
+  *out = std::move(f);
+  return taken;
+}
+
 int plan_conv(const ConvDesc& d, int dtype, const ConvTuning& t, ConvPlan* out) {
   RGBM_REQUIRE(d.M > 0 && d.M < (1ll << 31), "conv M out of range");
   RGBM_REQUIRE(d.Cout % 4 == 0 && d.ldo % 4 == 0, "conv Cout/ldo must be multiples of 4");
diff --git a/rgbmanip_amd/csrc/conv_plan.h b/rgbmanip_amd/csrc/conv_plan.h
--- a/rgbmanip_amd/csrc/conv_plan.h
+++ b/rgbmanip_amd/csrc/conv_plan.h
@@ -62,6 +62,22 @@
 bool border_applies(const ConvDesc& d, int dtype, int flags, long long main_rows);
 bool plan_border(const ConvDesc& d, int dtype, int flags, long long main_rows, int n_wg, BorderPlan* out);
 
+struct FoldTile {
+  int pix, ch;
+  int steps;
+};
+struct FoldPlan {
+  int n_wg, n_ch, n_pix, kr;
+  std::vector<FoldTile> tiles;
+  std::vector<int> order;
+  std::vector<int> wg_off;
+  double weight, tail_launch;
+  double max_cost_folded;
+  long long max_cost_main;
+};
+bool fold_eligible(const ConvDesc& d, int dtype, int flags, const ConvPlan& p);
+bool plan_fold(const ConvDesc& d, int dtype, int flags, const ConvPlan& p, const BorderPlan& bp, FoldPlan* out);
+
 constexpr size_t kM32SplitFloats = 8u << 20, kM32SplitCounters = 16384;
 
 int plan_conv(const ConvDesc& d, int dtype, const ConvTuning& t, ConvPlan* out);
diff --git a/rgbmanip_amd/csrc/kernels.h b/rgbmanip_amd/csrc/kernels.h
--- a/rgbmanip_amd/csrc/kernels.h
+++ b/rgbmanip_amd/csrc/kernels.h
@@ -136,8 +136,10 @@
   DBG_WS_128x256 = 65536, DBG_NO_SLIM64 = 262144, DBG_KORDER_TAPS_OUTER = 1 << 20, DBG_SWEEP_ALT_BLEND = 1 << 21, DBG_SWEEP_DOT2 = 1 << 22,
   DBG_PP_ONE_KERNEL = 1 << 23, DBG_NO_SLIM_SMALL = 1 << 24, DBG_PP_GENERIC_SELECT = 1 << 25, DBG_PP_GUARD = 1 << 26, DBG_GLOBAL_ADDR = 1 << 27,
   DBG_SWEEP_PER_TILE = 1 << 28, DBG_SPARSE_TAIL_R5 = 1 << 29, DBG_M32_TAILS_R5 = 1 << 30, DBG_POSE_MLP_R6 = 1 << 19, DBG_NO_BORDER_TILES = 32,
+  DBG_NO_FOLD_TAIL = 2,
 };
 extern int g_debug_flags;
+long long fold_launch_count();
 long long border_launch_count();
 extern long long g_ws_min_rows;
 extern int g_tuning_version;
diff --git a/rgbmanip_amd/csrc/layers.cpp b/rgbmanip_amd/csrc/layers.cpp
--- a/rgbmanip_amd/csrc/layers.cpp
+++ b/rgbmanip_amd/csrc/layers.cpp
@@ -127,7 +127,7 @@
 }
 
 struct BorderTables {
-  struct Entry { DevBuf buf; int n_wg = 0, b_ent = 0, b_rows = 0; };
+  struct Entry { DevBuf buf; int n_wg = 0, b_ent = 0, b_rows = 0, b_fold = 0; };
   std::mutex mu;
   std::map<std::array<long long, 7>, Entry> per_shape;
 };
@@ -283,12 +283,18 @@
     }
     e.b_rows = (int)tab.size();
     tab.insert(tab.end(), bp.rows.begin(), bp.rows.end());
+    FoldPlan fp;
+    if (plan_fold(d, dtype, t.flags & ~DBG_NO_FOLD_TAIL, p, bp, &fp)) {
+      e.b_fold = (int)tab.size();
+      tab.insert(tab.end(), fp.wg_off.begin(), fp.wg_off.end());
+      for (int i : fp.order) tab.push_back(fp.tiles[i].pix | fp.tiles[i].ch << 16);
+    }
     RGBM_CHECK_HIP(hipMalloc(e.buf.out(), tab.size() * sizeof(int)));
     RGBM_CHECK_HIP(hipMemcpy(e.buf.get(), tab.data(), tab.size() * sizeof(int), hipMemcpyHostToDevice));
     it = border->per_shape.emplace(key, std::move(e)).first;
   }
   d.btab = it->second.buf.get<int>();
-  d.b_nwg = it->second.n_wg; d.b_ent = it->second.b_ent; d.b_rows = it->second.b_rows;
+  d.b_nwg = it->second.n_wg; d.b_ent = it->second.b_ent; d.b_rows = it->second.b_rows; d.b_fold = it->second.b_fold;
   return 0;
 }
 
```

After: 6046 (median of 6 runs). About the same (+0.3%).
